# ashiq24/UNO

Hardware: AMD Instinct MI355X
Metric: UNO training samples/s (421^2 Darcy) (higher is better)
Workload: dtype f32; 1 GPU; Darcy 2D 421x421, UNO_9(3,64,pad=5) 64ch, batch 16/GPU, train step (fwd+loss+bwd+allreduce+Adam); global_batch=16, parallelism=dp1

## Files before the change

include/uno_spectral.h:

```cpp
#ifndef UNO_SPECTRAL_H
#define UNO_SPECTRAL_H

#ifdef __cplusplus
extern "C" {
#endif

#define UNO_SPECTRAL_ABI_VERSION 14

int uno_abi_version(void);
void* uno_upload_table(const void* host, long long bytes);

const char* uno_last_error(void);

long long uno_spectral_conv2d_fwd_ws_bytes(int B, int Ci, int Co, int m1, int m2);
long long uno_spectral_conv2d_bwd_ws_bytes(int B, int Ci, int Co, int m1, int m2);

int uno_spectral_conv2d_forward(const float* x, const float* w1, const float* w2, float* y,
                                float* xtrunc, void* ws, int B, int Ci, int Co, int H, int W,
                                int Ho, int Wo, int m1, int m2, void* stream);

int uno_spectral_conv2d_backward(const float* gy, const float* xtrunc, const float* w1,
                                 const float* w2, float* gx, float* gw1, float* gw2, void* ws,
                                 int B, int Ci, int Co, int H, int W, int Ho, int Wo, int m1,
                                 int m2, void* stream);
// ... 36 lines not shown
long long uno_spectral_conv3d_bwd_ws_bytes(int B, int Ci, int Co, int H, int Ho, int m1, int m2, int m3);
int uno_spectral_conv3d_forward(const float* x, const float* const* w, float* y, float* xtrunc, void* ws,
                                int B, int Ci, int Co, int H, int W, int T, int Ho, int Wo, int To,
                                int m1, int m2, int m3, void* stream);
int uno_spectral_conv3d_backward(const float* gy, const float* xtrunc, const float* const* w, float* gx,
                                 float* const* gw, void* ws, int B, int Ci, int Co, int H, int W, int T,
                                 int Ho, int Wo, int To, int m1, int m2, int m3, void* stream);

long long uno_dft3d_ws_bytes(int n_vol, int D1, int m2, int m3);
int uno_dft3d_forward_grouped(const float* x, float* spec, void* ws, int n_vol, int D1, int D2, int D3, int m1, int m2, int m3,
                              float scale, int adjoint, int group, int stride, int offset, void* stream);
int uno_dft3d_inverse_grouped(const float* spec, float* y, void* ws, int n_vol, int D1, int D2, int D3, int m1, int m2, int m3,
                              float scale, int weighted, int group, int stride, int offset, void* stream);

int uno_spectral_conv3d_forward2(const float* x1, const float* x2, int C1, const float* const* w, float* y, float* xtrunc, void* ws,
                                 int B, int Ci, int Co, int H, int W, int T, int Ho, int Wo, int To, int m1, int m2, int m3,
                                 void* stream);
int uno_spectral_conv3d_backward2(const float* gy, const float* xtrunc, const float* const* w, float* gx1, float* gx2, int C1,
                                  float* const* gw, void* ws, int B, int Ci, int Co, int H, int W, int T, int Ho, int Wo, int To,
                                  int m1, int m2, int m3, void* stream);

int uno_cdft_axis(const float* in, float* out, int inverse, int n_img, int H, int m1, int m2, int m3,
                  float scale, int mask_overlap, void* stream);


int uno_dft2d_forward(const float* images, float* spec, int n_img, int H, int W, int m1, int m2,
                      float scale, int hermitian_cols, int mask_overlap, void* stream);

int uno_dft2d_inverse(const float* spec, float* images, int n_img, int H, int W, int m1, int m2,
                      float scale, int hermitian_cols, int mask_overlap, void* stream);

int uno_reserve_cus(int n);

int uno_sweep_alternation(int enable);

int uno_dft2d_inverse_add_applies(int n_img, int H, int W, int m1, int m2, int Hs, int Ws);
int uno_dft2d_inverse_add(const float* spec, float* images, int n_img, int H, int W, int m1, int m2, float scale, int hermitian_cols,
                          int mask_overlap, const float* addend, int Hs, int Ws, const int* tile_p0, const float* row_op,
                          const int* col_v0, const float* col_op, void* stream);

int uno_dft2d_forward_resample_applies(int n_img, int H, int W, int m1, int m2, int Ho, int Wo, int KW);
int uno_dft2d_forward_resample(const float* images, float* spec, int n_img, int H, int W, int m1, int m2, float scale, int hermitian_cols,
                               int mask_overlap, int group, int stride, int offset, float* resampled, int Ho, int Wo, const int* col_start,
                               const float* col_wt, int KW, const int* row_tiles, const float* row_op, void* stream);

int uno_spectrum_crop(const float* src, float* dst, int n_img, int M1, int M2, int m1, int m2, int src_group, int src_stride, int src_offset,
                      int dst_group, int dst_stride, int dst_offset, void* stream);

int uno_dft2d_forward_bf16(const void* images, float* spec, int n_img, int H, int W, int m1, int m2,
                           float scale, int hermitian_cols, int mask_overlap, void* stream);
int uno_dft2d_inverse_bf16(const float* spec, void* images, int n_img, int H, int W, int m1, int m2,
                           float scale, int hermitian_cols, int mask_overlap, void* stream);

int uno_dft2d_forward_grouped(const float* images, float* spec, int n_img, int H, int W, int m1, int m2, float scale,
                              int hermitian_cols, int mask_overlap, int group, int stride, int offset, void* stream);
int uno_dft2d_inverse_grouped(const float* spec, float* images, int n_img, int H, int W, int m1, int m2, float scale,
                              int hermitian_cols, int mask_overlap, int group, int stride, int offset, void* stream);

int uno_mode_mix(const float* in, const float* const* w, float* out, int op, int B, int Ci, int Co,
                 int ncorner, int modes_per_corner, void* stream);

int uno_mode_wgrad(const float* xtrunc, const float* go, float* const* gw, int B, int Ci, int Co,
                   int ncorner, int modes_per_corner, void* stream);
int uno_mode_backward(const float* xtrunc, const float* go, const float* const* w, float* gx_spec, float* const* gw, int B, int Ci,
                      int Co, int ncorner, int modes_per_corner, int accumulate, void* stream);
int uno_mode_wgrad_acc(const float* xtrunc, const float* go, float* const* gw, int B, int Ci, int Co, int ncorner,
                       int modes_per_corner, int accumulate, void* stream);
int uno_spectral_conv2d_backward_acc(const void* gy, const float* xtrunc, const void* w1, const void* w2, void* gx,
                                     float* gw1, float* gw2, void* ws, int B, int Ci, int Co, int H, int W, int Ho, int Wo,
                                     int m1, int m2, int io_format, int accumulate_gw, void* stream);

int uno_resample2d(const float* in, float* out, float* tmp, int n_img, int H, int W, int Ho, int Wo,
                   const int* startH, const float* wtH, int KH, const int* startW, const float* wtW, int KW,
                   const int* tile_p0, const float* tile_w, int NP, int accumulate, void* stream);

int uno_channel_mix(const float* x, const float* w, const float* bias, float* y, int B, int Ci, int Co,
                    long long P, int transpose_w, int accumulate, int act_in, const float* dgelu_of, void* stream);

long long uno_channel_wgrad_ws_bytes(int B, int Ci, int Co, long long P);
int uno_channel_wgrad(const float* gy, const float* x, float* gw, float* gb, void* ws, int B, int Ci, int Co,
                      long long P, int act_x, void* stream);

int uno_channel_mix2(const float* x1, const float* x2, int C1, const float* w, const float* bias, float* y1, float* y2, int Co1,
                     float* y_act, int B, int Ci, int Co, long long P, int transpose_w, int accumulate, int act_in,
                     const float* dgelu_of, const float* proj_w, const float* proj_b, float* proj_out, void* stream);
int uno_channel_wgrad2(const float* gy, const float* x1, const float* x2, int C1, float* gw, float* gb, void* ws, int B, int Ci,
                       int Co, long long P, int act_x, int accumulate, void* stream);
int uno_channel_wgrad_finish(const void* parts, float* gw, float* gb, int Ci, int Co, long long nparts, int accumulate, void* stream);

int uno_gelu_project_forward(const float* pre, const float* w, const float* bias, float* out, int B, int C, long long P,
                             void* stream);
long long uno_gelu_project_bwd_ws_bytes(int B, int C, long long P);
int uno_gelu_project_backward(const float* pre, const float* w, const float* gout, float* gpre, float* gw, float* gb,
                              void* ws, int B, int C, long long P, void* stream);

int uno_gelu_project2_forward(const float* pre, const float* s, const float* w, const float* bias, float* out, int B, int C1, int C2,
                              long long P, int act2, void* stream);
long long uno_gelu_project2_bwd_ws_bytes(int B, int C1, int C2, long long P);
int uno_gelu_project2_backward(const float* pre, const float* s, const float* w, const float* gout, float* gpre, float* gs, float* gw,
                               float* gb, void* ws, int B, int C1, int C2, long long P, int act2, void* stream);

long long uno_rel_l2_steps_ws_bytes(int B, long long P, int T);
int uno_rel_l2_steps(const float* pred, const float* target, float* sums, float* rel, float* totals, void* ws, int B, long long P, int T,
                     void* stream);

long long uno_rel_l2_ws_bytes(int B, long long N);
int uno_rel_l2_forward(const float* x, long long x_row, long long x_elem, const float* y, long long y_row, long long y_elem, float* sums,
                       float* ratio, float* total, void* ws, int B, long long N, void* stream);
int uno_rel_l2_backward(const float* x, long long x_row, long long x_elem, const float* y, long long y_row, long long y_elem,
                        const float* sums, const float* g, int g_per_row, float scale, float* gx, int B, long long N, void* stream);

long long uno_rollout_ws_bytes(int B, long long P, int T);
int uno_rollout_advance(float* window, const float* frame, const float* target, float* pred, void* ws, int B, int C, int T_in, long long P,
                        int T, int t, int shift, void* stream);
int uno_rollout_finish(const void* ws, float* sums, float* rel, float* totals, int B, long long P, int T, void* stream);

int uno_rollout_lift(const float* given, const float* pred, const float* feat, const float* w, const float* bias, float* h, int B, int T_in,
                     int F, int Cm, long long P, int T, int t, void* stream);
long long uno_rollout_lift_bwd_ws_bytes(int B, int T_in, int F, int Cm, long long P, int T);
int uno_rollout_lift_backward(const float* gh, const float* given, const float* pred, const float* target, const float* feat, const float* w,
                              const float* sums, const float* gL, float* gpred, float* gframe, void* parts, int B, int T_in, int F, int Cm,
                              long long P, int T, int t, void* stream);
int uno_rollout_loss_seed(const float* pred, const float* target, const float* sums, const float* gL, float* gframe, int B, long long P, int T,
                          void* stream);

int uno_channel_mix2_win(const float* x1, const float* x2, int C1, const float* w, const float* bias, float* y1, float* y2, int Co1,
                         float* y_act, int B, int Ci, int Co, int rows, int cols, int pitch, long long plane, int transpose_w,
                         int accumulate, int act_in, const float* dgelu_of, const float* proj_w, const float* proj_b, float* proj_out,
                         void* stream);
int uno_channel_wgrad2_win(const float* gy, const float* x1, const float* x2, int C1, float* gw, float* gb, void* ws, int B, int Ci,
                           int Co, int rows, int cols, int pitch, long long plane, int act_x, int accumulate, void* stream);
int uno_gelu_project_backward_win(const float* pre, const float* w, const float* gout, float* gpre, float* gw, float* gb, void* ws,
                                  int B, int C, int rows, int cols, int pitch, long long plane, void* stream);
int uno_project_backward_applies(int B, int C1, int Ci, int Co, int rows, int cols, int pitch, long long plane);
long long uno_project_backward_ws_bytes(int B, int Ci, int Co, long long P);
int uno_project_backward(const float* x1, const float* x2, int C1, const float* w, const float* pre, const float* w2, const float* gout,
                         float* g1, float* g2, float* gw, float* gb, float* gw2, float* gb2, void* ws, int B, int Ci, int Co, int rows,
                         int cols, int pitch, long long plane, int act_in, int accumulate_w, void* stream);
int uno_clear_border(float* t, long long n_planes, int Hp, int Wp, int rows, int cols, void* stream);
int uno_channel_mix_act_padded(const float* x, const float* w, const float* bias, float* y, float* y_act, int B, int Ci, int Co, int H,
                               int W, int Hp, int Wp, int act_in, void* stream);
int uno_channel_mix_dgelu_padded(const float* x, const float* w, const float* bias, const float* g_padded, float* gz, int B, int Ci,
                                 int Co, int H, int W, int Hp, int Wp, int act_in, void* stream);
int uno_lift_forward(const float* x, const float* w1, const float* b1, const float* w0, const float* b0, float* act, int B, int Cin,
                     int Cm, int Co, int H, int W, int Hp, int Wp, void* stream);
long long uno_lift_bwd_ws_bytes(int B, int Cin, int Cm, int Co, int H, int W);
int uno_lift_backward(const float* x, const float* w1, const float* b1, const float* w0, const float* b0, const float* g_act, float* gw1,
                      float* gb1, float* gw0, float* gb0, void* ws, int B, int Cin, int Cm, int Co, int H, int W, int Hp, int Wp,
                      void* stream);
int uno_lift_backward_takes_second(int B, int Cin, int Cm, int Co, int H, int W, int Hp, int Wp);
int uno_lift_backward2(const float* x, const float* w1, const float* b1, const float* w0, const float* b0, const float* g_act,
                       const float* g_act2, float* gw1, float* gb1, float* gw0, float* gb0, void* ws, int B, int Cin, int Cm, int Co,
                       int H, int W, int Hp, int Wp, void* stream);

int uno_gelu_pad(const float* s, const float* gy, float* out, int n_img, int H, int W, int Hp, int Wp, int backward,
                 void* stream);

int uno_instnorm_forward(const float* x, const float* gamma, const float* beta, float* y, float* mean, float* rstd, long long rows,
                         int C, long long N, float eps, int gelu, void* stream);
int uno_instnorm_backward(const float* x, const float* gy, const float* gamma, const float* beta, const float* mean,
                          const float* rstd, float* gx, float* s1, float* s2, long long rows, int C, long long N, int gelu,
                          void* stream);

int uno_adam_step(float* p, const float* g, float* m, float* v, long long n, int is_complex, double lr, double beta1,
                  double beta2, double eps, double weight_decay, int step, void* stream);

int uno_adam_step_multi(int n_tensors, float* const* p, const float* const* g, float* const* m, float* const* v,
                        const long long* n, const int* is_complex, double lr, double beta1, double beta2, double eps,
                        double weight_decay, int step, void* stream);

int uno_adam_step_multi_dev(int n_tensors, float* const* p, const float* const* g, float* const* m, float* const* v,
                            const long long* n, const int* is_complex, double lr, double beta1, double beta2, double eps,
                            double weight_decay, int* step_counter, float* scalars, const double* hyper, void* stream);

int uno_spectral_conv2d_forward_mixed(const void* x_bf16, const void* w1_f16, const void* w2_f16, void* y_bf16,
                                      float* xtrunc, void* ws, int B, int Ci, int Co, int H, int W, int Ho, int Wo,
                                      int modes1, int modes2, void* stream);
int uno_spectral_conv2d_backward_mixed(const void* gy_bf16, const float* xtrunc, const void* w1_f16, const void* w2_f16,
                                       void* gx_bf16, float* gw1, float* gw2, void* ws, int B, int Ci, int Co, int H, int W,
                                       int Ho, int Wo, int modes1, int modes2, void* stream);
int uno_mode_mix_f16w(const float* in, const void* const* w_f16, float* out, int op, int B, int Ci, int Co, int ncorner,
                      int modes_per_corner, void* stream);
int uno_dft2d_forward_grouped_bf16(const void* images, float* spec, int n_img, int H, int W, int m1, int m2, float scale,
                                   int hermitian_cols, int mask_overlap, int group, int stride, int offset, void* stream);
int uno_dft2d_inverse_grouped_bf16(const float* spec, void* images, int n_img, int H, int W, int m1, int m2, float scale,
                                   int hermitian_cols, int mask_overlap, int group, int stride, int offset, void* stream);
int uno_resample2d_bf16(const void* in, void* out, float* tmp, int n_img, int H, int W, int Ho, int Wo, const int* startH,
                        const float* wtH, int KH, const int* startW, const float* wtW, int KW, const int* tile_p0,
                        const float* tile_w, int NP, int accumulate, void* stream);
int uno_channel_mix_bf16(const void* x, const float* w, const float* bias, void* y, int B, int Ci, int Co, long long P,
                         int transpose_w, int accumulate, int act_in, const void* dgelu_of, void* stream);
int uno_channel_wgrad_bf16(const void* gy, const void* x, float* gw, float* gb, void* ws, int B, int Ci, int Co, long long P,
                           int act_x, void* stream);
int uno_channel_mix2_bf16(const void* x1, const void* x2, int C1, const float* w, const float* bias, void* y1, void* y2, int Co1,
                          void* y_act, int B, int Ci, int Co, long long P, int transpose_w, int accumulate, int act_in,
                          const void* dgelu_of, const float* proj_w, const float* proj_b, void* proj_out, void* stream);
int uno_channel_wgrad2_bf16(const void* gy, const void* x1, const void* x2, int C1, float* gw, float* gb, void* ws, int B, int Ci,
                            int Co, long long P, int act_x, int accumulate, void* stream);
int uno_gelu_project_forward_bf16(const void* pre, const float* w, const float* bias, void* out, int B, int C, long long P,
                                  void* stream);
int uno_gelu_project_backward_bf16(const void* pre, const float* w, const void* gout, void* gpre, float* gw, float* gb,
                                   void* ws, int B, int C, long long P, void* stream);
int uno_gelu_pad_bf16(const void* s, const void* gy, void* out, int n_img, int H, int W, int Hp, int Wp, int backward,
                      void* stream);
int uno_instnorm_forward_bf16(const void* x, const float* gamma, const float* beta, void* y, float* mean, float* rstd,
                              long long rows, int C, long long N, float eps, int gelu, void* stream);
int uno_instnorm_backward_bf16(const void* x, const void* gy, const float* gamma, const float* beta, const float* mean,
                               const float* rstd, void* gx, float* s1, float* s2, long long rows, int C, long long N,
                               int gelu, void* stream);

long long uno_dft2d_any_ws_bytes(int n_img, int H, int W, int m1, int m2);
int uno_scratch_provide(void* ptr, long long bytes);
long long uno_channel_mix_ws_bytes(int Ci, int Co, long long P, int bf16);

int uno_transpose_batched(const float* in, float* out, int B, long long R, int C, long long ld_in, long long sb_in,
                          long long ld_out, long long sb_out, void* stream);

int uno_channel_mix2_rows(const float* x1, const float* x2, int C1, const float* w, const float* bias, float* y, int B, int Ci, int Co,
                          int rows, int cols, int pitch, int col0, long long plane, int act_in, void* stream);
int uno_channel_mix2_rows_grad(const float* gy, const float* w, int C1, const float* dgelu_of, float* g1, float* g2, int B, int Ci,
                               int Co, int rows, int cols, int pitch, int col0, long long plane, void* stream);
int uno_channel_wgrad2_rows(const float* gy, const float* x1, const float* x2, int C1, float* gw, float* gb, void* ws, int B, int Ci,
                            int Co, int rows, int cols, int pitch, int col0, long long plane, int act_x, int accumulate, void* stream);
int uno_channel_mix_act_padded_rows(const float* x, const float* w, const float* bias, float* y, float* y_act, int B, int Ci, int Co,
                                    int rows, int cols, int pitch, int col0, int act_in, void* stream);
int uno_dgelu_rows(const float* pre, const float* g_padded, float* gz, long long n_planes, int rows, int cols, int pitch, int col0,
                   long long plane, void* stream);

long long uno_ns2d_ws_bytes(int B, int N);
int uno_ns2d_forward(const float* w, float* w_h, void* ws, int B, int N, void* stream);
int uno_ns2d_inverse(const float* w_h, float* w, void* ws, int B, int N, void* stream);
int uno_ns2d_steps(float* w_h, const float* f_h, int f_batched, void* ws, int B, int N, long long n_steps, double visc, double delta_t,
                   void* stream);

int uno_profile_begin(int max_records);
int uno_profile_end(void);
int uno_profile_get(int index, char* name, int name_len, double* ms, double* bytes);

#ifdef __cplusplus
}
#endif
#endif
```

uno_amd/_native.py:

```python
from __future__ import annotations

import contextlib
import ctypes as C
import os
import threading

import torch

_HERE = os.path.dirname(os.path.abspath(__file__))
LIB_PATH = os.path.join(_HERE, "lib", "libuno_spectral.so")
ABI_VERSION = 14

_lib = None
_lock = threading.Lock()

_fp = C.c_void_p
_i = C.c_int
_SIGNATURES = {
    "uno_abi_version": (C.c_int, []),
    "uno_last_error": (C.c_char_p, []),
    "uno_dft2d_any_ws_bytes": (C.c_longlong, [_i] * 5),
    "uno_scratch_provide": (C.c_int, [_fp, C.c_longlong]),
    "uno_spectral_conv2d_fwd_ws_bytes": (C.c_longlong, [_i] * 5),
    "uno_spectral_conv2d_bwd_ws_bytes": (C.c_longlong, [_i] * 5),
    "uno_spectral_conv2d_forward": (C.c_int, [_fp] * 6 + [_i] * 9 + [_fp]),
    "uno_spectral_conv2d_backward": (C.c_int, [_fp] * 8 + [_i] * 9 + [_fp]),
    "uno_spectral_conv2d_forward_bf16": (C.c_int, [_fp] * 6 + [_i] * 9 + [_fp]),
    "uno_spectral_conv2d_backward_bf16": (C.c_int, [_fp] * 8 + [_i] * 9 + [_fp]),
    "uno_fft_resample3d_ws_bytes": (C.c_longlong, [_i] * 6),
    "uno_fft_resample3d": (C.c_int, [_fp] * 3 + [_i] * 8 + [_fp, _fp, _i, _fp, _fp, _i, C.c_float, _i, _i, _fp]),
    "uno_fft_resample3d_acc": (C.c_int, [_fp] * 4 + [_i] * 8 + [_fp, _fp, _i, _fp, _fp, _i, C.c_float, _i, _i, _fp]),
    "uno_fft_resample3d_any_ws_bytes": (C.c_longlong, [_i] * 6),
    "uno_fft_resample3d_any": (C.c_int, [_fp] * 3 + [_i] * 8 + [_fp, _fp, _i, _fp, _fp, _i, C.c_float, _i, _i, _fp]),
    "uno_fft_resample3d_any_acc": (C.c_int, [_fp] * 4 + [_i] * 8 + [_fp, _fp, _i, _fp, _fp, _i, C.c_float, _i, _i, _fp]),
    "uno_fft_resample3d_wide_ws_bytes": (C.c_longlong, [_i] * 6),
    "uno_fft_resample3d_wide": (C.c_int, [_fp] * 3 + [_i] * 8 + [_fp, _fp, _i, _fp, _fp, _i, C.c_float, _i, _i, _fp]),
    "uno_fft_resample3d_wide_acc": (C.c_int, [_fp] * 4 + [_i] * 8 + [_fp, _fp, _i, _fp, _fp, _i, C.c_float, _i, _i, _fp]),
    "uno_dft2d_forward": (C.c_int, [_fp, _fp] + [_i] * 5 + [C.c_float, _i, _i, _fp]),
    "uno_dft2d_forward_bf16": (C.c_int, [_fp, _fp] + [_i] * 5 + [C.c_float, _i, _i, _fp]),
    "uno_dft2d_inverse_bf16": (C.c_int, [_fp, _fp] + [_i] * 5 + [C.c_float, _i, _i, _fp]),
    "uno_dft2d_inverse": (C.c_int, [_fp, _fp] + [_i] * 5 + [C.c_float, _i, _i, _fp]),
    "uno_reserve_cus": (C.c_int, [_i]),
    "uno_sweep_alternation": (C.c_int, [_i]),
    "uno_dft2d_inverse_add_applies": (C.c_int, [_i] * 7),
    "uno_dft2d_forward_resample_applies": (C.c_int, [_i] * 8),
    "uno_dft2d_forward_resample": (C.c_int, [_fp, _fp] + [_i] * 5 + [C.c_float] + [_i] * 5 + [_fp, _i, _i, _fp, _fp, _i, _fp, _fp, _fp]),
    "uno_dft2d_inverse_add": (C.c_int, [_fp, _fp] + [_i] * 5 + [C.c_float, _i, _i, _fp, _i, _i, _fp, _fp, _fp, _fp, _fp]),
    "uno_dft2d_forward_grouped": (C.c_int, [_fp, _fp] + [_i] * 5 + [C.c_float] + [_i] * 5 + [_fp]),
    "uno_dft2d_inverse_grouped": (C.c_int, [_fp, _fp] + [_i] * 5 + [C.c_float] + [_i] * 5 + [_fp]),
    "uno_spectrum_crop": (C.c_int, [_fp, _fp] + [_i] * 11 + [_fp]),
    "uno_mode_mix": (C.c_int, [_fp, C.POINTER(_fp), _fp] + [_i] * 6 + [_fp]),
    "uno_mode_wgrad": (C.c_int, [_fp, _fp, C.POINTER(_fp)] + [_i] * 5 + [_fp]),
    "uno_mode_backward": (C.c_int, [_fp, _fp, C.POINTER(_fp), _fp, C.POINTER(_fp)] + [_i] * 6 + [_fp]),
    "uno_spectral_conv3d_fwd_ws_bytes": (C.c_longlong, [_i] * 8),
    "uno_spectral_conv3d_bwd_ws_bytes": (C.c_longlong, [_i] * 8),
    "uno_spectral_conv3d_forward": (C.c_int, [_fp, C.POINTER(_fp), _fp, _fp, _fp] + [_i] * 12 + [_fp]),
    "uno_spectral_conv3d_backward": (C.c_int, [_fp, _fp, C.POINTER(_fp), _fp, C.POINTER(_fp), _fp] + [_i] * 12 + [_fp]),
    "uno_cdft_axis": (C.c_int, [_fp, _fp] + [_i] * 6 + [C.c_float, _i, _fp]),
    "uno_dft3d_ws_bytes": (C.c_longlong, [_i] * 4),
    "uno_dft3d_forward_grouped": (C.c_int, [_fp, _fp, _fp] + [_i] * 7 + [C.c_float] + [_i] * 4 + [_fp]),
    "uno_dft3d_inverse_grouped": (C.c_int, [_fp, _fp, _fp] + [_i] * 7 + [C.c_float] + [_i] * 4 + [_fp]),
    "uno_spectral_conv3d_forward2": (C.c_int, [_fp, _fp, _i, C.POINTER(_fp), _fp, _fp, _fp] + [_i] * 12 + [_fp]),
    "uno_spectral_conv3d_backward2": (C.c_int, [_fp, _fp, C.POINTER(_fp), _fp, _fp, _i, C.POINTER(_fp), _fp] + [_i] * 12 + [_fp]),
    "uno_resample2d": (C.c_int, [_fp, _fp, _fp] + [_i] * 5 + [_fp, _fp, _i, _fp, _fp, _i, _fp, _fp, _i, _i, _fp]),
    "uno_channel_mix": (C.c_int, [_fp, _fp, _fp, _fp, _i, _i, _i, C.c_longlong, _i, _i, _i, _fp, _fp]),
    "uno_channel_wgrad_ws_bytes": (C.c_longlong, [_i, _i, _i, C.c_longlong]),
    "uno_channel_wgrad": (C.c_int, [_fp, _fp, _fp, _fp, _fp, _i, _i, _i, C.c_longlong, _i, _fp]),
    "uno_channel_mix2": (C.c_int, [_fp, _fp, _i, _fp, _fp, _fp, _fp, _i, _fp, _i, _i, _i, C.c_longlong, _i, _i, _i, _fp, _fp, _fp, _fp, _fp]),
    "uno_channel_wgrad2": (C.c_int, [_fp, _fp, _fp, _i, _fp, _fp, _fp, _i, _i, _i, C.c_longlong, _i, _i, _fp]),
    "uno_channel_mix2_win": (C.c_int, [_fp, _fp, _i, _fp, _fp, _fp, _fp, _i, _fp, _i, _i, _i, _i, _i, _i, C.c_longlong, _i, _i, _i, _fp, _fp, _fp, _fp, _fp]),
    "uno_channel_mix_ws_bytes": (C.c_longlong, [_i, _i, C.c_longlong, _i]),
    "uno_clear_border": (C.c_int, [_fp, C.c_longlong, _i, _i, _i, _i, _fp]),
    "uno_channel_mix_act_padded": (C.c_int, [_fp, _fp, _fp, _fp, _fp, _i, _i, _i, _i, _i, _i, _i, _i, _fp]),
    "uno_lift_forward": (C.c_int, [_fp] * 6 + [_i] * 8 + [_fp]),
    "uno_lift_bwd_ws_bytes": (C.c_longlong, [_i] * 6),
    "uno_lift_backward": (C.c_int, [_fp] * 11 + [_i] * 8 + [_fp]),
    "uno_lift_backward2": (C.c_int, [_fp] * 12 + [_i] * 8 + [_fp]),
    "uno_lift_backward_takes_second": (C.c_int, [_i] * 8),
    "uno_channel_mix_dgelu_padded": (C.c_int, [_fp, _fp, _fp, _fp, _fp, _i, _i, _i, _i, _i, _i, _i, _i, _fp]),
    "uno_channel_wgrad2_win": (C.c_int, [_fp, _fp, _fp, _i, _fp, _fp, _fp, _i, _i, _i, _i, _i, _i, C.c_longlong, _i, _i, _fp]),
    "uno_gelu_project_backward_win": (C.c_int, [_fp] * 7 + [_i, _i, _i, _i, _i, C.c_longlong, _fp]),
    "uno_channel_wgrad_finish": (C.c_int, [_fp, _fp, _fp, _i, _i, C.c_longlong, _i, _fp]),
    "uno_mode_wgrad_acc": (C.c_int, [_fp, _fp, C.POINTER(_fp)] + [_i] * 6 + [_fp]),
    "uno_spectral_conv2d_backward_acc": (C.c_int, [_fp] * 8 + [_i] * 11 + [_fp]),
    "uno_upload_table": (C.c_void_p, [_fp, C.c_longlong]),
    "uno_project_backward_applies": (C.c_int, [_i] * 7 + [C.c_longlong]),
    "uno_project_backward_ws_bytes": (C.c_longlong, [_i, _i, _i, C.c_longlong]),
    "uno_project_backward": (C.c_int, [_fp, _fp, _i] + [_fp] * 11 + [_i] * 6 + [C.c_longlong, _i, _i, _fp]),
    "uno_gelu_project_forward": (C.c_int, [_fp, _fp, _fp, _fp, _i, _i, C.c_longlong, _fp]),
    "uno_gelu_project_bwd_ws_bytes": (C.c_longlong, [_i, _i, C.c_longlong]),
    "uno_gelu_project_backward": (C.c_int, [_fp] * 7 + [_i, _i, C.c_longlong, _fp]),
    "uno_gelu_project2_forward": (C.c_int, [_fp] * 5 + [_i, _i, _i, C.c_longlong, _i, _fp]),
    "uno_gelu_project2_bwd_ws_bytes": (C.c_longlong, [_i, _i, _i, C.c_longlong]),
    "uno_gelu_project2_backward": (C.c_int, [_fp] * 9 + [_i, _i, _i, C.c_longlong, _i, _fp]),
    "uno_rel_l2_steps_ws_bytes": (C.c_longlong, [_i, C.c_longlong, _i]),
    "uno_rel_l2_steps": (C.c_int, [_fp] * 6 + [_i, C.c_longlong, _i, _fp]),
    "uno_rel_l2_ws_bytes": (C.c_longlong, [_i, C.c_longlong]),
    "uno_rel_l2_forward": (C.c_int, [_fp, C.c_longlong, C.c_longlong] * 2 + [_fp] * 4 + [_i, C.c_longlong, _fp]),
    "uno_rel_l2_backward": (C.c_int, [_fp, C.c_longlong, C.c_longlong] * 2 + [_fp, _fp, _i, C.c_float, _fp, _i, C.c_longlong, _fp]),
    "uno_rollout_ws_bytes": (C.c_longlong, [_i, C.c_longlong, _i]),
    "uno_rollout_advance": (C.c_int, [_fp] * 5 + [_i, _i, _i, C.c_longlong, _i, _i, _i, _fp]),
    "uno_rollout_finish": (C.c_int, [_fp] * 4 + [_i, C.c_longlong, _i, _fp]),
    "uno_rollout_lift": (C.c_int, [_fp] * 6 + [_i, _i, _i, _i, C.c_longlong, _i, _i, _fp]),
    "uno_rollout_lift_bwd_ws_bytes": (C.c_longlong, [_i, _i, _i, _i, C.c_longlong, _i]),
    "uno_rollout_lift_backward": (C.c_int, [_fp] * 11 + [_i, _i, _i, _i, C.c_longlong, _i, _i, _fp]),
    "uno_rollout_loss_seed": (C.c_int, [_fp] * 5 + [_i, C.c_longlong, _i, _fp]),
    "uno_gelu_pad": (C.c_int, [_fp, _fp, _fp] + [_i] * 6 + [_fp]),
    "uno_transpose_batched": (C.c_int, [_fp, _fp, _i, C.c_longlong, _i] + [C.c_longlong] * 4 + [_fp]),
    "uno_instnorm_forward": (C.c_int, [_fp] * 6 + [C.c_longlong, _i, C.c_longlong, C.c_float, _i, _fp]),
    "uno_instnorm_backward": (C.c_int, [_fp] * 9 + [C.c_longlong, _i, C.c_longlong, _i, _fp]),
    "uno_adam_step": (C.c_int, [_fp, _fp, _fp, _fp, C.c_longlong, _i] + [C.c_double] * 5 + [_i, _fp]),
    "uno_adam_step_multi": (C.c_int, [_i, C.POINTER(_fp), C.POINTER(_fp), C.POINTER(_fp), C.POINTER(_fp), C.POINTER(C.c_longlong),
                                      C.POINTER(_i)] + [C.c_double] * 5 + [_i, _fp]),
    "uno_adam_step_multi_dev": (C.c_int, [_i, C.POINTER(_fp), C.POINTER(_fp), C.POINTER(_fp), C.POINTER(_fp), C.POINTER(C.c_longlong),
                                          C.POINTER(_i)] + [C.c_double] * 5 + [_fp, _fp, _fp, _fp]),
    "uno_spectral_conv2d_forward_mixed": (C.c_int, [_fp] * 6 + [_i] * 9 + [_fp]),
    "uno_spectral_conv2d_backward_mixed": (C.c_int, [_fp] * 8 + [_i] * 9 + [_fp]),
    "uno_mode_mix_f16w": (C.c_int, [_fp, C.POINTER(_fp), _fp] + [_i] * 6 + [_fp]),
    "uno_dft2d_forward_grouped_bf16": (C.c_int, [_fp, _fp] + [_i] * 5 + [C.c_float] + [_i] * 5 + [_fp]),
    "uno_dft2d_inverse_grouped_bf16": (C.c_int, [_fp, _fp] + [_i] * 5 + [C.c_float] + [_i] * 5 + [_fp]),
    "uno_resample2d_bf16": (C.c_int, [_fp, _fp, _fp] + [_i] * 5 + [_fp, _fp, _i, _fp, _fp, _i, _fp, _fp, _i, _i, _fp]),
    "uno_channel_mix_bf16": (C.c_int, [_fp, _fp, _fp, _fp, _i, _i, _i, C.c_longlong, _i, _i, _i, _fp, _fp]),
    "uno_channel_wgrad_bf16": (C.c_int, [_fp, _fp, _fp, _fp, _fp, _i, _i, _i, C.c_longlong, _i, _fp]),
    "uno_channel_mix2_bf16": (C.c_int, [_fp, _fp, _i, _fp, _fp, _fp, _fp, _i, _fp, _i, _i, _i, C.c_longlong, _i, _i, _i, _fp, _fp, _fp, _fp, _fp]),
    "uno_channel_wgrad2_bf16": (C.c_int, [_fp, _fp, _fp, _i, _fp, _fp, _fp, _i, _i, _i, C.c_longlong, _i, _i, _fp]),
    "uno_gelu_project_forward_bf16": (C.c_int, [_fp, _fp, _fp, _fp, _i, _i, C.c_longlong, _fp]),
    "uno_gelu_project_backward_bf16": (C.c_int, [_fp] * 7 + [_i, _i, C.c_longlong, _fp]),
    "uno_gelu_pad_bf16": (C.c_int, [_fp, _fp, _fp] + [_i] * 6 + [_fp]),
    "uno_instnorm_forward_bf16": (C.c_int, [_fp] * 6 + [C.c_longlong, _i, C.c_longlong, C.c_float, _i, _fp]),
    "uno_instnorm_backward_bf16": (C.c_int, [_fp] * 9 + [C.c_longlong, _i, C.c_longlong, _i, _fp]),
    "uno_channel_mix2_rows": (C.c_int, [_fp, _fp, _i, _fp, _fp, _fp] + [_i] * 7 + [C.c_longlong, _i, _fp]),
    "uno_channel_mix2_rows_grad": (C.c_int, [_fp, _fp, _i, _fp, _fp, _fp] + [_i] * 7 + [C.c_longlong, _fp]),
    "uno_channel_wgrad2_rows": (C.c_int, [_fp, _fp, _fp, _i, _fp, _fp, _fp] + [_i] * 7 + [C.c_longlong, _i, _i, _fp]),
    "uno_channel_mix_act_padded_rows": (C.c_int, [_fp] * 5 + [_i] * 8 + [_fp]),
    "uno_dgelu_rows": (C.c_int, [_fp, _fp, _fp, C.c_longlong, _i, _i, _i, _i, C.c_longlong, _fp]),
    "uno_ns2d_ws_bytes": (C.c_longlong, [_i, _i]),
    "uno_ns2d_forward": (C.c_int, [_fp, _fp, _fp, _i, _i, _fp]),
    "uno_ns2d_inverse": (C.c_int, [_fp, _fp, _fp, _i, _i, _fp]),
    "uno_ns2d_steps": (C.c_int, [_fp, _fp, _i, _fp, _i, _i, C.c_longlong, C.c_double, C.c_double, _fp]),
    "uno_profile_begin": (C.c_int, [_i]),
    "uno_profile_end": (C.c_int, []),
    "uno_profile_get": (C.c_int, [_i, C.c_char_p, _i, C.POINTER(C.c_double), C.POINTER(C.c_double)]),
}
EXPORTED_SYMBOLS = tuple(_SIGNATURES)


def lib():
    global _lib
    if _lib is None:
        with _lock:
            if _lib is None:
                if not os.path.exists(LIB_PATH):
                    raise RuntimeError(
                        f"uno_amd: native library {LIB_PATH} is missing - build it with "
                        "`python -m uno_amd.build` (hipcc, gfx950); there is no CPU fallback")
                h = C.CDLL(LIB_PATH)
                for name, (res, args) in _SIGNATURES.items():
                    fn = getattr(h, name)
                    fn.restype = res
                    fn.argtypes = args
                if h.uno_abi_version() != ABI_VERSION:
                    raise RuntimeError(f"uno_amd: ABI mismatch, library {h.uno_abi_version()} != binding {ABI_VERSION}")
                _lib = h
    return _lib


def _check(rc: int, what: str):
    if rc != 0:
        msg = lib().uno_last_error().decode(errors="replace")
        raise RuntimeError(f"{what} failed (code {rc}): {msg}")


def _ptr(t: torch.Tensor):
    return C.c_void_p(t.data_ptr())


def _opt(t):
    return _ptr(t) if t is not None else C.c_void_p(0)


def _count(lead) -> int:
    n = 1
    for d in lead:
        n *= d
    return n


def _stream(t: torch.Tensor):
    return C.c_void_p(torch.cuda.current_stream(t.device).cuda_stream)


class _scratch:

    def __init__(self, device, nbytes):
        self.bytes, self.device, self.buf = nbytes, device, None

    def __enter__(self):
        if self.bytes > 0:
            self.buf = torch.empty(self.bytes, dtype=torch.uint8, device=self.device)
            _check(lib().uno_scratch_provide(_ptr(self.buf), self.bytes), "uno_scratch_provide")
        return self

    def __exit__(self, *exc):
        if self.bytes > 0:
            lib().uno_scratch_provide(None, 0)
        return False


class _any_mode_scratch(_scratch):

    def __init__(self, device, *needs):
        L = lib()
        _scratch.__init__(self, device, max((int(L.uno_dft2d_any_ws_bytes(*[int(v) for v in n])) for n in needs), default=0))


class _mix_scratch(_scratch):

    def __init__(self, device, Ci, Co, P, bf16):
        _scratch.__init__(self, device, int(lib().uno_channel_mix_ws_bytes(int(Ci), int(Co), int(P), 1 if bf16 else 0)))


def _require(t: torch.Tensor, dtype, name: str, dense: bool = True):
    if not t.is_cuda:
        raise RuntimeError(f"uno_amd: {name} must live on a HIP device (got {t.device})"
                           + ("; the spectral convolution runs only on the MI355X kernels" if dense else ""))
    if t.dtype != dtype:
        raise RuntimeError(f"uno_amd: {name} must be {dtype} (got {t.dtype})")
    if dense and not t.is_contiguous():
        raise RuntimeError(f"uno_amd: {name} must be contiguous")


# ... 497 lines not shown
    sW, wW = tabW
    accumulate = out is not None
    if accumulate:
        _require(out, x.dtype, "out")
        if tuple(out.shape) != (*lead, Ho, Wo):
            raise RuntimeError(f"uno_amd: out has shape {tuple(out.shape)}, expected {(*lead, Ho, Wo)}")
    else:
        out = torch.empty((*lead, Ho, Wo), dtype=x.dtype, device=x.device)
    with torch.cuda.device(x.device):
        tmp = torch.empty(max(1, n * min(Ho * W, H * Wo)), dtype=torch.float32, device=x.device)
        if tilesH is not None:
            tp0, tw = tilesH
            targs = (_ptr(tp0), _ptr(tw), tw.shape[1])
        else:
            targs = (C.c_void_p(0), C.c_void_p(0), 0)
        fn = _entry("uno_resample2d", bf16)
        rc = fn(_ptr(x), _ptr(out), _ptr(tmp), n, H, W, Ho, Wo, _ptr(sH), _ptr(wH), wH.shape[1],
                _ptr(sW), _ptr(wW), wW.shape[1], *targs, 1 if accumulate else 0, _stream(x))
    _check(rc, "uno_resample2d")
    return out


def _window_fits(rows: int, cols: int, pitch: int, plane: int) -> bool:
    return not (rows < 1 or cols % 4 or cols < 260 or pitch < cols or (rows - 1) * pitch + cols > plane or rows * cols >= 1 << 24)


def _window_args(window, plane: int, bf16: bool):
    rows, cols, pitch = (int(v) for v in window)
    if bf16:
        raise RuntimeError("uno_amd: pixel windows are float32 only")
    if not _window_fits(rows, cols, pitch, plane):
        raise RuntimeError(f"uno_amd: window rows={rows} cols={cols} pitch={pitch} does not fit a plane of {plane} elements "
                           "(cols: a multiple of 4, 260 <= cols <= pitch; rows * cols < 2^24)")
    return rows, cols, pitch


def channel_mix(x, w, bias=None, transpose_w: bool = False, out=None, act_in: bool = False, dgelu_of=None, dgelu_total: bool = False,
                window=None):
    if window is not None:
        return channel_mix2(x, None, w, bias, transpose_w=transpose_w, out=out, act_in=act_in, dgelu_of=dgelu_of,
                            accumulate=(2 if (dgelu_total and dgelu_of is not None) else 1) if out is not None else 0, window=window)
    bf16 = _act_dtype(x, "x")
    _require(w, torch.float32, "weight")
    if bias is not None:
        _require(bias, torch.float32, "bias")
    B, Ci, P = x.shape
    Co = w.shape[1] if transpose_w else w.shape[0]
    if (w.shape[0] if transpose_w else w.shape[1]) != Ci:
        raise RuntimeError(f"uno_amd: weight {tuple(w.shape)} does not match {Ci} input channels")
    accumulate = out is not None
    if accumulate:
        _require(out, x.dtype, "out")
        if tuple(out.shape) != (B, Co, P):
            raise RuntimeError(f"uno_amd: out has shape {tuple(out.shape)}, expected {(B, Co, P)}")
        y = out
    else:
        y = torch.empty((B, Co, P), dtype=x.dtype, device=x.device)
    with torch.cuda.device(x.device), _mix_scratch(x.device, Ci, Co, P, bf16):
        if dgelu_of is not None:
            _require(dgelu_of, x.dtype, "dgelu_of")
            if tuple(dgelu_of.shape) != (B, Co, P):
                raise RuntimeError(f"uno_amd: dgelu_of has shape {tuple(dgelu_of.shape)}, expected {(B, Co, P)}")
        rc = _entry("uno_channel_mix", bf16)(_ptr(x), _ptr(w), _opt(bias), _ptr(y), B, Ci, Co, P, 1 if transpose_w else 0,
                                             (2 if (dgelu_total and dgelu_of is not None) else 1) if accumulate else 0,
                                             1 if act_in else 0, _opt(dgelu_of), _stream(x))
    _check(rc, "uno_channel_mix")
    return y


def clear_border(t, rows: int, cols: int):
    _require(t, torch.float32, "tensor")
    Hp, Wp = t.shape[-2:]
    n = t.numel() // max(1, Hp * Wp)
    with torch.cuda.device(t.device):
        rc = lib().uno_clear_border(_ptr(t), n, Hp, Wp, int(rows), int(cols), _stream(t))
    _check(rc, "uno_clear_border")
    return t


def channel_mix_act_padded_ok(x, Hp: int, Wp: int) -> bool:
    H, W = x.shape[-2:]
    return x.dtype == torch.float32 and 260 <= W <= Wp and H <= Hp and H * W < (1 << 24)


def channel_mix_act_padded(x, w, bias, Hp: int, Wp: int, act_in: bool = False, keep_y: bool = True):
    _require(x, torch.float32, "x")
    _require(w, torch.float32, "weight")
    if bias is not None:
        _require(bias, torch.float32, "bias")
    B, Ci, H, W = x.shape
    Co = w.shape[0]
    if w.shape[1] != Ci:
        raise RuntimeError(f"uno_amd: weight {tuple(w.shape)} does not match {Ci} input channels")
    y = torch.empty((B, Co, H, W), dtype=x.dtype, device=x.device) if keep_y else None
    act = torch.empty((B, Co, Hp, Wp), dtype=x.dtype, device=x.device)
    with torch.cuda.device(x.device):
        rc = lib().uno_channel_mix_act_padded(_ptr(x), _ptr(w), _opt(bias), _opt(y), _ptr(act),
                                              B, Ci, Co, H, W, int(Hp), int(Wp), 1 if act_in else 0, _stream(x))
    _check(rc, "uno_channel_mix_act_padded")
    return y, act


def lift_ok(x, w1, w0, Hp: int, Wp: int) -> bool:
    if x.dim() != 4 or x.dtype != torch.float32:
        return False
    H, W = x.shape[-2:]
    return (1 <= x.shape[1] <= 3 and w1.shape[0] in (16, 32) and w1.shape[1] == x.shape[1] and w0.shape[1] == w1.shape[0]
            and 260 <= W <= Wp and H <= Hp and H * W < (1 << 24))


def lift_forward(x, w1, b1, w0, b0, Hp: int, Wp: int):
    for t, n in ((x, "x"), (w1, "weight 1"), (w0, "weight 0")) + tuple((t, "bias") for t in (b1, b0) if t is not None):
        _require(t, torch.float32, n)
    B, Cin, H, W = x.shape
    Cm, Co = w1.shape[0], w0.shape[0]
    act = torch.empty((B, Co, Hp, Wp), dtype=x.dtype, device=x.device)
    with torch.cuda.device(x.device):
        rc = lib().uno_lift_forward(_ptr(x), _ptr(w1), _opt(b1), _ptr(w0), _opt(b0),
                                    _ptr(act), B, Cin, Cm, Co, H, W, int(Hp), int(Wp), _stream(x))
    _check(rc, "uno_lift_forward")
    return act


def lift_backward_takes_second(x, w1, w0, Hp: int, Wp: int) -> bool:
    B, Cin, H, W = x.shape
    return bool(lib().uno_lift_backward_takes_second(B, Cin, w1.shape[0], w0.shape[0], H, W, int(Hp), int(Wp)))


def lift_backward(x, w1, b1, w0, b0, g_act, g_act2=None):
    _require(g_act, torch.float32, "grad_output")
    B, Cin, H, W = x.shape
    Cm, Co = w1.shape[0], w0.shape[0]
    Hp, Wp = g_act.shape[-2:]
    if tuple(g_act.shape[:2]) != (B, Co):
        raise RuntimeError("uno_amd: grad_output does not match the lift")
    if g_act2 is not None:
        _require(g_act2, torch.float32, "second grad_output")
        if tuple(g_act2.shape) != tuple(g_act.shape):
            raise RuntimeError("uno_amd: the two gradients of the lift's output disagree in shape")
    dev = x.device
    gw1 = torch.empty((Cm, Cin), dtype=torch.float32, device=dev)
    gw0 = torch.empty((Co, Cm), dtype=torch.float32, device=dev)
    gb1 = torch.empty((Cm,), dtype=torch.float32, device=dev) if b1 is not None else None
    gb0 = torch.empty((Co,), dtype=torch.float32, device=dev) if b0 is not None else None
    with torch.cuda.device(dev):
        ws = torch.empty(max(1, lib().uno_lift_bwd_ws_bytes(B, Cin, Cm, Co, H, W)), dtype=torch.uint8, device=dev)
        rc = lib().uno_lift_backward2(_ptr(x), _ptr(w1), _opt(b1), _ptr(w0), _opt(b0),
                                     _ptr(g_act), _opt(g_act2), _ptr(gw1), _opt(gb1), _ptr(gw0),
                                     _opt(gb0), _ptr(ws), B, Cin, Cm, Co, H, W, int(Hp), int(Wp), _stream(x))
    _check(rc, "uno_lift_backward")
    return gw1, gb1, gw0, gb0


def channel_mix_dgelu_padded(x, w, bias, g_padded, act_in: bool = False):
    _require(x, torch.float32, "x")
    _require(w, torch.float32, "weight")
    _require(g_padded, torch.float32, "grad_output")
    if bias is not None:
        _require(bias, torch.float32, "bias")
    B, Ci, H, W = x.shape
    Co = w.shape[0]
    if w.shape[1] != Ci or g_padded.dim() != 4 or g_padded.shape[:2] != (B, Co) or g_padded.shape[2] < H or g_padded.shape[3] < W:
        raise RuntimeError("uno_amd: weight / grad_output do not match the layer")
    Hp, Wp = g_padded.shape[2:]
    gz = torch.empty((B, Co, H, W), dtype=x.dtype, device=x.device)
    with torch.cuda.device(x.device):
        rc = lib().uno_channel_mix_dgelu_padded(_ptr(x), _ptr(w), _opt(bias), _ptr(g_padded), _ptr(gz),
                                                B, Ci, Co, H, W, int(Hp), int(Wp), 1 if act_in else 0, _stream(x))
    _check(rc, "uno_channel_mix_dgelu_padded")
    return gz


def channel_mix2_ok(C1: int, Co1, Co: int, P: int) -> bool:
    if C1 is not None and (C1 < 16 or C1 % 16):
        return False
    if Co1 is not None and (Co1 < 64 or Co1 % 64):
        return False
    return True


def channel_mix2(x1, x2, w, bias=None, transpose_w: bool = False, out=None, out2=None, split_out: int | None = None,
                 act_in: bool = False, dgelu_of=None, y_act: bool = False, accumulate: bool = False, project=None, window=None):
    bf16 = _act_dtype(x1, "x1")
    _require(w, torch.float32, "weight")
    if x2 is not None:
        _require(x2, x1.dtype, "x2")
        if x2.shape[0] != x1.shape[0] or x2.shape[2] != x1.shape[2]:
            raise RuntimeError("uno_amd: the two sources disagree in batch / pixel count")
    if bias is not None:
        _require(bias, torch.float32, "bias")
    B, C1, P = x1.shape
    Ci = C1 + (x2.shape[1] if x2 is not None else 0)
    Co = w.shape[1] if transpose_w else w.shape[0]
    if (w.shape[0] if transpose_w else w.shape[1]) != Ci:
        raise RuntimeError(f"uno_amd: weight {tuple(w.shape)} does not match {Ci} input channels")
    Co1 = Co if split_out is None else int(split_out)
    if out is None:
        y1 = torch.empty((B, Co1, P), dtype=x1.dtype, device=x1.device)
        y2 = torch.empty((B, Co - Co1, P), dtype=x1.dtype, device=x1.device) if split_out is not None else None
    else:
        y1, y2 = out, out2
        _require(y1, x1.dtype, "out")
        if tuple(y1.shape) != (B, Co1, P) or (split_out is not None and (y2 is None or tuple(y2.shape) != (B, Co - Co1, P))):
            raise RuntimeError("uno_amd: output tensors do not match (B, Co1, P) / (B, Co - Co1, P)")
        if y2 is not None:
            _require(y2, x1.dtype, "out2")
    act = torch.empty((B, Co, P), dtype=x1.dtype, device=x1.device) if y_act else None
    if dgelu_of is not None:
        _require(dgelu_of, x1.dtype, "dgelu_of")
        if tuple(dgelu_of.shape) != (B, Co1, P):
            raise RuntimeError(f"uno_amd: dgelu_of has shape {tuple(dgelu_of.shape)}, expected {(B, Co1, P)}")
    proj = pw = pb = None
    if project is not None:
        pw, pb = project
        _require(pw, torch.float32, "projection weight")
        if pw.numel() != Co:
            raise RuntimeError(f"uno_amd: projection weight has {pw.numel()} entries for {Co} channels")
        if pb is not None:
            _require(pb, torch.float32, "projection bias")
        proj = torch.empty((B, P), dtype=x1.dtype, device=x1.device)
    acc_flag = int(accumulate) if out is not None else 0
    if acc_flag == 2 and (dgelu_of is None or window is None):
        raise RuntimeError("uno_amd: accumulate = 2 goes with dgelu_of (windowed one-destination calls)")
    with torch.cuda.device(x1.device), _mix_scratch(x1.device, Ci, Co, P if window is None else window[0] * window[1], bf16):
        if window is not None:
            fn, size = lib().uno_channel_mix2_win, (*_window_args(window, P, bf16), P)
        else:
            fn, size = _entry("uno_channel_mix2", bf16), (P,)
        rc = fn(_ptr(x1), _opt(x2), C1, _ptr(w), _opt(bias), _ptr(y1), _opt(y2), Co1, _opt(act),
                B, Ci, Co, *size, 1 if transpose_w else 0, acc_flag, 1 if act_in else 0,
                _opt(dgelu_of), _opt(pw), _opt(pb), _opt(proj), _stream(x1))
    _check(rc, "uno_channel_mix2")
    if split_out is not None:
        return y1, y2
    if project is not None:
        return y1, proj
    return (y1, act) if y_act else y1


def channel_wgrad_partial_floats(B: int, Ci: int, Co: int, P: int) -> int:
    return int(lib().uno_channel_wgrad_ws_bytes(B, Ci, Co, P)) // 4


def channel_wgrad_finish(parts, Ci: int, Co: int, need_bias: bool, out_w=None, out_b=None, accumulate: bool = False):
    _require(parts, torch.float32, "partial sums")
    blk = Co * (Ci + 1)
    if parts.numel() == 0 or parts.numel() % blk:
        raise RuntimeError("uno_amd: the partial sums are not a whole number of (Co, Ci + 1) blocks")
    gw, gb, accumulate = _real_grad_buffers(out_w, out_b, Ci, Co, need_bias, parts.device, accumulate)
    with torch.cuda.device(parts.device):
        rc = lib().uno_channel_wgrad_finish(_ptr(parts), _ptr(gw), _opt(gb), Ci, Co,
                                            parts.numel() // blk, 1 if accumulate else 0, _stream(parts))
    _check(rc, "uno_channel_wgrad_finish")
    return gw, gb


def channel_wgrad2(gy, x1, x2, need_bias: bool = True, act_x: bool = False, out_w=None, out_b=None, accumulate: bool = False,
                   partials_out=None, window=None):
    bf16 = _act_dtype(gy, "grad_output")
    _require(x1, gy.dtype, "x1")
    B, Co, P = gy.shape
    if window is not None:
        if partials_out is not None:
            raise RuntimeError("uno_amd: windowed weight gradients run both stages")
        win = _window_args(window, P, bf16)
    C1 = x1.shape[1]
    C2 = 0
    if x2 is not None:
        _require(x2, gy.dtype, "x2")
        C2 = x2.shape[1]
        if x2.shape[0] != B or x2.shape[2] != P:
            raise RuntimeError("uno_amd: grad_output and the sources disagree in batch / pixel count")
    if x1.shape[0] != B or x1.shape[2] != P:
        raise RuntimeError("uno_amd: grad_output and the sources disagree in batch / pixel count")
    Ci = C1 + C2
    L = lib()
    if partials_out is not None:
        _require(partials_out, torch.float32, "partial-sum buffer")
        if partials_out.numel() != channel_wgrad_partial_floats(B, Ci, Co, P):
            raise RuntimeError("uno_amd: partial-sum buffer has the wrong size")
        with torch.cuda.device(gy.device):
            rc = _entry("uno_channel_wgrad2", bf16)(_ptr(gy), _ptr(x1), _opt(x2), C1, C.c_void_p(0), C.c_void_p(0),
                                                    _ptr(partials_out), B, Ci, Co, P, 1 if act_x else 0, 3, _stream(gy))
        _check(rc, "uno_channel_wgrad2")
        return None, None
    gw, gb, accumulate = _real_grad_buffers(out_w, out_b, Ci, Co, need_bias, gy.device, accumulate)
    with torch.cuda.device(gy.device):
        if window is not None:
            fn, size, Pl = L.uno_channel_wgrad2_win, (*win, P), win[0] * win[1]
        else:
            fn, size, Pl = _entry("uno_channel_wgrad2", bf16), (P,), P
        ws = torch.empty(max(1, L.uno_channel_wgrad_ws_bytes(B, Ci, Co, Pl)), dtype=torch.uint8, device=gy.device)
        rc = fn(_ptr(gy), _ptr(x1), _opt(x2), C1, _ptr(gw), _opt(gb),
                _ptr(ws), B, Ci, Co, *size, 1 if act_x else 0, 1 if accumulate else 0, _stream(gy))
    _check(rc, "uno_channel_wgrad2")
    return gw, gb


def rows_window_ok(rows: int, cols: int, pitch: int, col0: int, plane: int, Ci: int = 1, Co: int = 1) -> bool:
    return (rows >= 0 and cols >= 1 and col0 >= 0 and col0 + cols <= pitch <= 256 and rows * pitch < (1 << 24) and plane >= rows * pitch
            and 1 <= Ci <= 1024 and Co >= 1)


def _rows_args(window, plane: int):
    rows, cols, pitch, col0 = (int(v) for v in window)
    return rows, cols, pitch, col0, int(plane)
# ... 713 lines not shown
```

uno_amd/csrc/capi_pointwise.hip:

```cpp
#include "../../include/uno_spectral.h"
#include "uno_common.h"

using namespace uno;

extern "C" {

static int resample2d_impl(const void* in, void* out, float* tmp, int n_img, int H, int W, int Ho, int Wo, const int* startH,
                           const float* wtH, int KH, const int* startW, const float* wtW, int KW, const int* tile_p0,
                           const float* tile_w, int NP, int accumulate, int bf16, void* stream) {
    if (n_img < 0 || H < 1 || W < 1 || Ho < 1 || Wo < 1) { set_error("uno_resample2d: bad sizes"); return -1; }
    if (n_img == 0) return 0;
    if (!in || !out || !tmp || !startH || !wtH || !startW || !wtW) { set_error("uno_resample2d: null pointer"); return -1; }
    return launch_resample2d(in, out, tmp, n_img, H, W, Ho, Wo, startH, wtH, KH, startW, wtW, KW, tile_p0, tile_w, NP, accumulate, bf16, (hipStream_t)stream);
}

int uno_resample2d(const float* in, float* out, float* tmp, int n_img, int H, int W, int Ho, int Wo, const int* startH,
                   const float* wtH, int KH, const int* startW, const float* wtW, int KW, const int* tile_p0,
                   const float* tile_w, int NP, int accumulate, void* stream) {
    return resample2d_impl(in, out, tmp, n_img, H, W, Ho, Wo, startH, wtH, KH, startW, wtW, KW, tile_p0, tile_w, NP, accumulate, 0, stream);
}

int uno_resample2d_bf16(const void* in, void* out, float* tmp, int n_img, int H, int W, int Ho, int Wo, const int* startH,
                        const float* wtH, int KH, const int* startW, const float* wtW, int KW, const int* tile_p0,
                        const float* tile_w, int NP, int accumulate, void* stream) {
// ... 123 lines not shown
        ChannelMixArgs a{};
        a.x = pre; a.w = w; a.y = g1; a.y2 = x2 ? g2 : nullptr; a.dgelu_of = act_in ? x1 : nullptr;
        a.B = B; a.Ci = Co; a.Co = Ci; a.C1 = Co; a.Co1 = x2 ? C1 : Ci; a.P = P; a.transpose_w = 1;
        a.win = win; a.pb_w2 = w2; a.pb_g = gout;
        if (int rc = launch_channel_mix2(a, s)) return rc;
    }
    WgradProjectedBack pb;
    pb.w2 = w2; pb.g = gout; pb.gw2 = gw2; pb.gb2 = gb2;
    return launch_channel_wgrad2(pre, x1, x2, C1, gw, gb, (float*)ws, B, Ci, Co, P, act_in, accumulate_w, 0, s, win, pb);
}

int uno_clear_border(float* t, long long n_planes, int Hp, int Wp, int rows, int cols, void* stream) {
    if (n_planes < 0 || Hp < 1 || Wp < 1 || rows < 0 || rows > Hp || cols < 0 || cols > Wp) {
        set_error("uno_clear_border: bad sizes planes=%lld (%d, %d) keep (%d, %d)", n_planes, Hp, Wp, rows, cols);
        return -1;
    }
    if (n_planes == 0) return 0;
    if (!t) { set_error("uno_clear_border: null pointer"); return -1; }
    return launch_clear_border(t, n_planes, Hp, Wp, rows, cols, (hipStream_t)stream);
}

static int lift_padded(const char* who, const float* x, const float* w, const float* bias, float* y, float* y_act, const float* gmul, int B,
                       int Ci, int Co, int H, int W, int Hp, int Wp, int act_in, void* stream) {
    if (B < 0 || Ci < 1 || Co < 1 || H < 1 || W < 1 || Hp < H || Wp < W) {
        set_error("%s: bad sizes B=%d Ci=%d Co=%d (%d, %d) -> (%d, %d)", who, B, Ci, Co, H, W, Hp, Wp);
        return -1;
    }
    if (B == 0) return 0;
    if (!x || !w || (!y && !y_act) || (gmul && !y)) { set_error("%s: null pointer", who); return -1; }
    ChannelMixArgs a{};
    a.x = x; a.w = w; a.bias = bias; a.y = y; a.y_act = y_act; a.gmul = gmul;
    a.B = B; a.Ci = Ci; a.Co = Co; a.C1 = Ci; a.Co1 = Co; a.P = (long long)H * W; a.act_in = act_in;
    a.act_cols = W; a.act_pitch = Wp; a.act_plane = (long long)Hp * Wp;
    if (int rc = launch_channel_mix2(a, (hipStream_t)stream)) return rc;
    return y_act ? launch_clear_border(y_act, (long long)B * Co, Hp, Wp, H, W, (hipStream_t)stream) : 0;
}

int uno_channel_mix_act_padded(const float* x, const float* w, const float* bias, float* y, float* y_act, int B, int Ci, int Co, int H, int W,
                               int Hp, int Wp, int act_in, void* stream) {
    if (!y_act) { set_error("uno_channel_mix_act_padded: null pointer"); return -1; }
    return lift_padded("uno_channel_mix_act_padded", x, w, bias, y, y_act, nullptr, B, Ci, Co, H, W, Hp, Wp, act_in, stream);
}

int uno_channel_mix_dgelu_padded(const float* x, const float* w, const float* bias, const float* g_padded, float* gz, int B, int Ci, int Co,
                                 int H, int W, int Hp, int Wp, int act_in, void* stream) {
    if (!g_padded || !gz) { set_error("uno_channel_mix_dgelu_padded: null pointer"); return -1; }
    return lift_padded("uno_channel_mix_dgelu_padded", x, w, bias, gz, nullptr, g_padded, B, Ci, Co, H, W, Hp, Wp, act_in, stream);
}

static int lift_check(const char* who, int B, int Cin, int Cm, int Co, int H, int W, int Hp, int Wp) {
    if (B < 0 || Cin < 1 || Cin > 3 || Cm < 5 || Cm > 32 || Cm % 16 || Co < 1 || H < 1 || W < 260 || Hp < H || Wp < W || (long long)H * W >= (1LL << 24)) {
        set_error("%s: needs 1 .. 3 input channels, 16 or 32 middle channels, 260 <= W <= Wp, H <= Hp, H * W < 2^24 (got B=%d %d -> %d -> %d, (%d, %d) -> (%d, %d))",
                  who, B, Cin, Cm, Co, H, W, Hp, Wp);
        return -1;
    }
    return 0;
}

static bool lift_fused_fits(int B, int H, int Hp, int Wp, int Co) {
    return (long long)Hp * Wp * Co < (1LL << 31) && B <= 65535 && (long long)H * Wp < (1LL << 24);
}

int uno_lift_forward(const float* x, const float* w1, const float* b1, const float* w0, const float* b0, float* act, int B, int Cin, int Cm,
                     int Co, int H, int W, int Hp, int Wp, void* stream) {
    if (int rc = lift_check("uno_lift_forward", B, Cin, Cm, Co, H, W, Hp, Wp)) return rc;
    if (B == 0) return 0;
    if (!x || !w1 || !w0 || !act) { set_error("uno_lift_forward: null pointer"); return -1; }
    if (lift_bwd_fused_applies(Cin, Cm, Co, W, (long long)H * W) && lift_fused_fits(B, H, Hp, Wp, Co) && (Wp & ~3) >= 260 && (Wp & ~3) >= W) {
        if (int rc = launch_lift_forward_fused(x, w1, b1, w0, b0, act, B, Cin, H, W, Hp, Wp, (hipStream_t)stream)) return rc;
        return launch_clear_border(act, (long long)B * Co, Hp, Wp, H, Wp, (hipStream_t)stream);
    }
    ChannelMixArgs a{};
    a.x = x; a.w = w0; a.bias = b0; a.y = nullptr; a.y_act = act;
    a.B = B; a.Ci = Cm; a.Co = Co; a.C1 = Cm; a.Co1 = Co; a.P = (long long)H * W; a.act_in = 1;
    a.act_cols = W; a.act_pitch = Wp; a.act_plane = (long long)Hp * Wp;
    a.vh_x = x; a.vh_w = w1; a.vh_b = b1; a.vh_ci = Cin; a.vh_mode = 1;
    if (int rc = launch_channel_mix2(a, (hipStream_t)stream)) return rc;
    return launch_clear_border(act, (long long)B * Co, Hp, Wp, H, W, (hipStream_t)stream);
}

static long long lift_wgrad_ws(int B, int Cin, int Cm, int Co, long long P) {
    const long long a = 4LL * channel_wgrad_ws_floats(B, Cm, Co, P, nullptr), b = 4LL * channel_wgrad_ws_floats(B, Cin, Cm, P, nullptr);
    return a > b ? a : b;
}
long long uno_lift_bwd_ws_bytes(int B, int Cin, int Cm, int Co, int H, int W) {
    if (B < 1 || Cin < 1 || Cm < 1 || Co < 1 || H < 1 || W < 1) return 0;
    const long long P = (long long)H * W;
    return 4LL * B * P * (Co + Cm) + lift_wgrad_ws(B, Cin, Cm, Co, P);
}

int uno_lift_backward_takes_second(int B, int Cin, int Cm, int Co, int H, int W, int Hp, int Wp) {
    if (B < 1 || Cin < 1 || Cin > 3 || Cm < 5 || Cm > 32 || Cm % 16 || Co < 1 || H < 1 || W < 260 || Hp < H || Wp < W) return 0;
    return (lift_bwd_fused_applies(Cin, Cm, Co, W, (long long)H * W) && lift_fused_fits(B, H, Hp, Wp, Co)) ? 1 : 0;
}

int uno_lift_backward2(const float* x, const float* w1, const float* b1, const float* w0, const float* b0_, const float* g_act, const float* g_act2,
                       float* gw1, float* gb1, float* gw0, float* gb0, void* ws, int B, int Cin, int Cm, int Co, int H, int W, int Hp, int Wp,
                       void* stream);

int uno_lift_backward(const float* x, const float* w1, const float* b1, const float* w0, const float* b0_, const float* g_act, float* gw1,
                      float* gb1, float* gw0, float* gb0, void* ws, int B, int Cin, int Cm, int Co, int H, int W, int Hp, int Wp, void* stream) {
    return uno_lift_backward2(x, w1, b1, w0, b0_, g_act, nullptr, gw1, gb1, gw0, gb0, ws, B, Cin, Cm, Co, H, W, Hp, Wp, stream);
}

int uno_lift_backward2(const float* x, const float* w1, const float* b1, const float* w0, const float* b0_, const float* g_act, const float* g_act2,
                       float* gw1, float* gb1, float* gw0, float* gb0, void* ws, int B, int Cin, int Cm, int Co, int H, int W, int Hp, int Wp,
                       void* stream) {
    if (int rc = lift_check("uno_lift_backward", B, Cin, Cm, Co, H, W, Hp, Wp)) return rc;
    if (g_act2 && !uno_lift_backward_takes_second(B, Cin, Cm, Co, H, W, Hp, Wp) && B > 0) {
        set_error("uno_lift_backward2: a second gradient tensor goes with the fused kernel only (query uno_lift_backward_takes_second)");
        return -3;
    }
    if (!gw1 || !gw0) { set_error("uno_lift_backward: null pointer"); return -1; }
    hipStream_t s = (hipStream_t)stream;
    if (B == 0) {
        if (hipMemsetAsync(gw1, 0, sizeof(float) * Cm * Cin, s) != hipSuccess || hipMemsetAsync(gw0, 0, sizeof(float) * Co * Cm, s) != hipSuccess ||
            (gb1 && hipMemsetAsync(gb1, 0, sizeof(float) * Cm, s) != hipSuccess) || (gb0 && hipMemsetAsync(gb0, 0, sizeof(float) * Co, s) != hipSuccess)) {
            set_error("uno_lift_backward: memset failed");
            return -5;
        }
        return 0;
    }
    if (!x || !w1 || !w0 || !g_act || !ws) { set_error("uno_lift_backward: null pointer"); return -1; }
    const long long P = (long long)H * W;
    if (lift_bwd_fused_applies(Cin, Cm, Co, W, P) && lift_fused_fits(B, H, Hp, Wp, Co)) {
        float* part = static_cast<float*>(ws);
        const long long nparts = lift_bwd_fused_parts(B, H, W);
        float* part1 = part + (size_t)nparts * Co * (Cm + 1);
        if (int rc = launch_lift_backward_fused(x, w1, b1, w0, b0_, g_act, part, part1, B, Cin, H, W, Hp, Wp, s, g_act2)) return rc;
        if (int rc = launch_channel_wgrad_finish(part, gw0, gb0, Cm, Co, nparts, 0, s)) return rc;
        return launch_channel_wgrad_finish(part1, gw1, gb1, Cin, Cm, nparts, 0, s);
    }
    float* gz = static_cast<float*>(ws);
    float* gh = gz + (size_t)B * Co * P;
    float* wws = gh + (size_t)B * Cm * P;
    {
        ChannelMixArgs a{};
        a.x = x; a.w = w0; a.bias = b0_; a.y = gz; a.gmul = g_act;
        a.B = B; a.Ci = Cm; a.Co = Co; a.C1 = Cm; a.Co1 = Co; a.P = P; a.act_in = 1;
        a.act_cols = W; a.act_pitch = Wp; a.act_plane = (long long)Hp * Wp;
        a.vh_x = x; a.vh_w = w1; a.vh_b = b1; a.vh_ci = Cin; a.vh_mode = 1;
        if (int rc = launch_channel_mix2(a, s)) return rc;
    }
    {
        ChannelMixArgs a{};
        a.x = gz; a.w = w0; a.y = gh; a.B = B; a.Ci = Co; a.Co = Cm; a.C1 = Co; a.Co1 = Cm; a.P = P; a.transpose_w = 1;
        a.vh_x = x; a.vh_w = w1; a.vh_b = b1; a.vh_ci = Cin; a.vh_mode = 2;
        if (int rc = launch_channel_mix2(a, s)) return rc;
    }
    if (int rc = launch_channel_wgrad_vh(gz, x, w1, b1, Cin, gw0, gb0, wws, B, Cm, Co, P, 1, s, 0)) return rc;
    return launch_channel_wgrad2(gh, x, nullptr, Cin, gw1, gb1, wws, B, Cin, Cm, P, 0, 0, 0, s);
}

long long uno_channel_wgrad_ws_bytes(int B, int Ci, int Co, long long P) {
    if (B < 1 || Ci < 1 || Co < 1 || P < 1) return 0;
    return 4LL * channel_wgrad_ws_floats(B, Ci, Co, P, nullptr);
}

static int channel_wgrad_impl(const void* gy, const void* x, float* gw, float* gb, void* ws, int B, int Ci, int Co, long long P,
                              int act_x, int bf16, void* stream) {
    if (B < 0 || Ci < 1 || Co < 1 || P < 0) { set_error("uno_channel_wgrad: bad sizes B=%d Ci=%d Co=%d P=%lld", B, Ci, Co, P); return -1; }
    if (!gw) { set_error("uno_channel_wgrad: null pointer"); return -1; }
    if (B == 0 || P == 0) {
        if (hipMemsetAsync(gw, 0, sizeof(float) * Co * Ci, (hipStream_t)stream) != hipSuccess ||
            (gb && hipMemsetAsync(gb, 0, sizeof(float) * Co, (hipStream_t)stream) != hipSuccess)) { set_error("uno_channel_wgrad: memset failed"); return -5; }
        return 0;
    }
    if (!gy || !x || !ws) { set_error("uno_channel_wgrad: null pointer"); return -1; }
    return launch_channel_wgrad(gy, x, gw, gb, (float*)ws, B, Ci, Co, P, act_x, bf16, (hipStream_t)stream);
}

int uno_channel_wgrad(const float* gy, const float* x, float* gw, float* gb, void* ws, int B, int Ci, int Co, long long P,
                      int act_x, void* stream) {
    return channel_wgrad_impl(gy, x, gw, gb, ws, B, Ci, Co, P, act_x, 0, stream);
}

int uno_channel_wgrad_bf16(const void* gy, const void* x, float* gw, float* gb, void* ws, int B, int Ci, int Co, long long P,
                           int act_x, void* stream) {
    return channel_wgrad_impl(gy, x, gw, gb, ws, B, Ci, Co, P, act_x, 1, stream);
}

static int channel_wgrad2_impl(const void* gy, const void* x1, const void* x2, int C1, float* gw, float* gb, void* ws, int B, int Ci,
                               int Co, long long P, int act_x, int accumulate, int bf16, void* stream, const PixelWindow& win = PixelWindow()) {
    if (B < 0 || Ci < 1 || Co < 1 || P < 0) { set_error("uno_channel_wgrad2: bad sizes B=%d Ci=%d Co=%d P=%lld", B, Ci, Co, P); return -1; }
    if (accumulate < 0 || accumulate > 3 || accumulate == 2) { set_error("uno_channel_wgrad2: accumulate is 0, 1 or 3 (got %d)", accumulate); return -1; }
    if (!gw && accumulate != 3) { set_error("uno_channel_wgrad2: null pointer"); return -1; }
    if (B == 0 || P == 0) {
        if (accumulate == 3) {
            if (!ws) { set_error("uno_channel_wgrad2: null pointer"); return -1; }
            if (hipMemsetAsync(ws, 0, uno_channel_wgrad_ws_bytes(B, Ci, Co, P), (hipStream_t)stream) != hipSuccess) { set_error("uno_channel_wgrad2: memset failed"); return -5; }
            return 0;
        }
        if (accumulate) return 0;
        if (hipMemsetAsync(gw, 0, sizeof(float) * Co * Ci, (hipStream_t)stream) != hipSuccess ||
            (gb && hipMemsetAsync(gb, 0, sizeof(float) * Co, (hipStream_t)stream) != hipSuccess)) { set_error("uno_channel_wgrad2: memset failed"); return -5; }
        return 0;
    }
    if (!gy || !x1 || !ws) { set_error("uno_channel_wgrad2: null pointer"); return -1; }
    return launch_channel_wgrad2(gy, x1, x2, x2 ? C1 : Ci, gw, gb, (float*)ws, B, Ci, Co, P, act_x, accumulate, bf16, (hipStream_t)stream, win);
}

int uno_channel_wgrad2_win(const float* gy, const float* x1, const float* x2, int C1, float* gw, float* gb, void* ws, int B, int Ci, int Co,
                           int rows, int cols, int pitch, long long plane, int act_x, int accumulate, void* stream) {
    PixelWindow win; long long P;
    if (!make_window("uno_channel_wgrad2_win", rows, cols, pitch, plane, &win, &P)) return -1;
    return channel_wgrad2_impl(gy, x1, x2, C1, gw, gb, ws, B, Ci, Co, P, act_x, accumulate, 0, stream, win);
}

int uno_channel_wgrad2(const float* gy, const float* x1, const float* x2, int C1, float* gw, float* gb, void* ws, int B, int Ci, int Co,
                       long long P, int act_x, int accumulate, void* stream) {
    return channel_wgrad2_impl(gy, x1, x2, C1, gw, gb, ws, B, Ci, Co, P, act_x, accumulate, 0, stream);
}

int uno_channel_wgrad2_bf16(const void* gy, const void* x1, const void* x2, int C1, float* gw, float* gb, void* ws, int B, int Ci, int Co,
                            long long P, int act_x, int accumulate, void* stream) {
    return channel_wgrad2_impl(gy, x1, x2, C1, gw, gb, ws, B, Ci, Co, P, act_x, accumulate, 1, stream);
}

int uno_channel_wgrad_finish(const void* parts, float* gw, float* gb, int Ci, int Co, long long nparts, int accumulate, void* stream) {
    if (Ci < 1 || Co < 1 || nparts < 1) { set_error("uno_channel_wgrad_finish: bad sizes Ci=%d Co=%d blocks=%lld", Ci, Co, nparts); return -1; }
    if (!parts || !gw) { set_error("uno_channel_wgrad_finish: null pointer"); return -1; }
    return launch_channel_wgrad_finish((const float*)parts, gw, gb, Ci, Co, nparts, accumulate, (hipStream_t)stream);
}

int uno_adam_step(float* p, const float* g, float* m, float* v, long long n, int is_complex, double lr, double beta1, double beta2,
                  double eps, double weight_decay, int step, void* stream) {
    if (n < 0 || step < 1 || !(beta1 >= 0.f && beta1 < 1.f) || !(beta2 >= 0.f && beta2 < 1.f)) {
        set_error("uno_adam_step: bad arguments n=%lld step=%d betas=(%g, %g)", n, step, beta1, beta2);
        return -1;
    }
    if (n == 0) return 0;
    if (!p || !g || !m || !v) { set_error("uno_adam_step: null pointer"); return -1; }
    return launch_adam(p, g, m, v, n, is_complex, lr, beta1, beta2, eps, weight_decay, step, (hipStream_t)stream);
}

int uno_adam_step_multi(int n_tensors, float* const* p, const float* const* g, float* const* m, float* const* v,
                        const long long* n, const int* is_complex, double lr, double beta1, double beta2, double eps,
                        double weight_decay, int step, void* stream) {
    if (n_tensors < 0 || (n_tensors > 0 && (!p || !g || !m || !v || !n || !is_complex))) {
        set_error("uno_adam_step_multi: bad arguments");
        return -1;
    }
    if (step < 1 || !(beta1 >= 0.f && beta1 < 1.f) || !(beta2 >= 0.f && beta2 < 1.f)) {
        set_error("uno_adam_step_multi: bad arguments step=%d betas=(%g, %g)", step, beta1, beta2);
        return -1;
    }
    for (int t = 0; t < n_tensors; ++t) {
        if (n[t] < 0) { set_error("uno_adam_step_multi: tensor %d has n=%lld", t, n[t]); return -1; }
        if (n[t] > 0 && (!p[t] || !g[t] || !m[t] || !v[t])) { set_error("uno_adam_step_multi: null pointer (tensor %d)", t); return -1; }
    }
    return launch_adam_multi(n_tensors, p, g, m, v, n, is_complex, lr, beta1, beta2, eps, weight_decay, step, (hipStream_t)stream);
}

int uno_adam_step_multi_dev(int n_tensors, float* const* p, const float* const* g, float* const* m, float* const* v,
                            const long long* n, const int* is_complex, double lr, double beta1, double beta2, double eps,
                            double weight_decay, int* step_counter, float* scalars, const double* hyper, void* stream) {
    if (n_tensors < 0 || (n_tensors > 0 && (!p || !g || !m || !v || !n || !is_complex)) || !step_counter || !scalars) {
        set_error("uno_adam_step_multi_dev: bad arguments");
        return -1;
    }
    if (!(beta1 >= 0.f && beta1 < 1.f) || !(beta2 >= 0.f && beta2 < 1.f)) { set_error("uno_adam_step_multi_dev: bad betas (%g, %g)", beta1, beta2); return -1; }
    for (int t = 0; t < n_tensors; ++t) {
        if (n[t] < 0) { set_error("uno_adam_step_multi_dev: tensor %d has n=%lld", t, n[t]); return -1; }
        if (n[t] > 0 && (!p[t] || !g[t] || !m[t] || !v[t])) { set_error("uno_adam_step_multi_dev: null pointer (tensor %d)", t); return -1; }
    }
    if (int rc = launch_adam_advance(step_counter, scalars, hyper, lr, eps, weight_decay, beta1, beta2, (hipStream_t)stream)) return rc;
    return launch_adam_multi(n_tensors, p, g, m, v, n, is_complex, lr, beta1, beta2, eps, weight_decay, 1, (hipStream_t)stream, scalars);
}

static int gelu_project_forward_impl(const void* pre, const float* w, const float* bias, void* out, int B, int C, long long P, int bf16, void* stream) {
    if (B < 0 || C < 1 || P < 0) { set_error("uno_gelu_project_forward: bad sizes B=%d C=%d P=%lld", B, C, P); return -1; }
    if (B == 0 || P == 0) return 0;
    if (!pre || !w || !out) { set_error("uno_gelu_project_forward: null pointer"); return -1; }
    return launch_gelu_project_fwd(pre, w, bias, out, B, C, P, bf16, (hipStream_t)stream);
}

int uno_gelu_project_forward(const float* pre, const float* w, const float* bias, float* out, int B, int C, long long P, void* stream) {
    return gelu_project_forward_impl(pre, w, bias, out, B, C, P, 0, stream);
}

int uno_gelu_project_forward_bf16(const void* pre, const float* w, const float* bias, void* out, int B, int C, long long P, void* stream) {
    return gelu_project_forward_impl(pre, w, bias, out, B, C, P, 1, stream);
}

long long uno_gelu_project_bwd_ws_bytes(int B, int C, long long P) {
    if (B < 1 || C < 1 || P < 1) return 0;
    return 4LL * gelu_project_ws_floats(B, C, P);
}

static int gelu_project_backward_impl(const void* pre, const float* w, const void* gout, void* gpre, float* gw, float* gb, void* ws, int B,
                                      int C, long long P, int bf16, void* stream, const PixelWindow& win = PixelWindow()) {
    if (B < 0 || C < 1 || P < 0) { set_error("uno_gelu_project_backward: bad sizes B=%d C=%d P=%lld", B, C, P); return -1; }
    if (!gw) { set_error("uno_gelu_project_backward: null pointer"); return -1; }
    if (B == 0 || P == 0) {
        if (hipMemsetAsync(gw, 0, sizeof(float) * C, (hipStream_t)stream) != hipSuccess ||
            (gb && hipMemsetAsync(gb, 0, sizeof(float), (hipStream_t)stream) != hipSuccess)) { set_error("uno_gelu_project_backward: memset failed"); return -5; }
        return 0;
    }
    if (!pre || !w || !gout || !gpre || !ws) { set_error("uno_gelu_project_backward: null pointer"); return -1; }
    return launch_gelu_project_bwd(pre, w, gout, gpre, gw, gb, (float*)ws, B, C, P, bf16, (hipStream_t)stream, win);
}

int uno_gelu_project_backward_win(const float* pre, const float* w, const float* gout, float* gpre, float* gw, float* gb, void* ws, int B,
                                  int C, int rows, int cols, int pitch, long long plane, void* stream) {
    PixelWindow win; long long P;
    if (!make_window("uno_gelu_project_backward_win", rows, cols, pitch, plane, &win, &P)) return -1;
// ... 240 lines not shown
```

uno_amd/csrc/lift_bwd.hip:

```cpp
#include "uno_common.h"
#include <cstdlib>

namespace uno {

constexpr int LB_PT = 128;
constexpr int LB_TS = 148;
constexpr int LB_CM = 32, LB_CO = 64;
constexpr int LB_WS = 80, LB_WTS = 48;
#ifndef UNO_LB_TPW
#define UNO_LB_TPW 8
#endif
constexpr int LB_TPW = UNO_LB_TPW;

struct LiftGeom {
    int H, W, W4, nslot, npt;
    int skip_d, skip_p;
    int Pd, Pp;
    unsigned magic;
};
static LiftGeom lift_geom(int H, int W, int Hp, int Wp, int slots_per_row = 0) {
    LiftGeom g;
    g.H = H; g.W = W; g.W4 = slots_per_row ? slots_per_row : ((W + 3) & ~3); g.nslot = H * g.W4; g.npt = (g.nslot + 127) / 128;
    g.skip_d = W - g.W4; g.skip_p = Wp - g.W4; g.Pd = H * W; g.Pp = Hp * Wp;
    g.magic = (unsigned)(((1ULL << 40) + g.W4 - 1) / (unsigned long long)g.W4);
    return g;
}
__device__ __forceinline__ int lift_clamped(int off, int plane_len) { return max(min(off, plane_len - 4), 0); }
struct LiftQuad { int nv, od, op, row_ok, last, shd, shp; };
__device__ __forceinline__ LiftQuad lift_quad(const LiftGeom& g, int s0, int s) {
    const int r0 = (int)(((unsigned long long)(unsigned)s0 * g.magic) >> 40);
    const int r = r0 + (s >= (r0 + 1) * g.W4 ? 1 : 0);
    const int col = s - r * g.W4;
    const int od = s + r * g.skip_d, op = s + r * g.skip_p, odc = lift_clamped(od, g.Pd), opc = lift_clamped(op, g.Pp);
    return LiftQuad{r < g.H ? min(max(g.W - col, 0), 4) : 0, odc, opc, r < g.H ? 1 : 0, col == g.W4 - 4 ? 1 : 0, od - odc, op - opc};
}
__device__ __forceinline__ float4 lift_fix(const float4& v, int sh) {
    float t0 = v.x, t1 = v.y, t2 = v.z, t3 = v.w;
    if (sh & 1) { t0 = t1; t1 = t2; t2 = t3; }
    if (sh & 2) { t0 = t2; t1 = t3; }
    return make_float4(t0, t1, t2, t3);
}
__device__ __forceinline__ float4 lift_mask(const float4& v, int nv) {
    return make_float4(nv > 0 ? v.x : 0.f, nv > 1 ? v.y : 0.f, nv > 2 ? v.z : 0.f, nv > 3 ? v.w : 0.f);
}

struct LiftBwdParams {
    const float* x;
    const float* w1;
    const float* b1;
    const float* w0;
    const float* b0;
    const float* g;
    const float* g2;
    float* part;
    float* part1;
    int B, Cin;
    LiftGeom geo;
    unsigned long long* stamps;
    int rev;
};

__device__ __forceinline__ float4 lb_vh(const float4& t, const float4* q) {
    return make_float4(fmaf(t.z, q[2].x, fmaf(t.y, q[1].x, fmaf(t.x, q[0].x, t.w))), fmaf(t.z, q[2].y, fmaf(t.y, q[1].y, fmaf(t.x, q[0].y, t.w))),
                       fmaf(t.z, q[2].z, fmaf(t.y, q[1].z, fmaf(t.x, q[0].z, t.w))), fmaf(t.z, q[2].w, fmaf(t.y, q[1].w, fmaf(t.x, q[0].w, t.w))));
}

__device__ __forceinline__ void lb_gelu_both(float x, float& g, float& d) {
    const float cdf = 0.5f * (1.f + uno_erf(x * 0.70710678118654752440f));
    g = x * cdf;
    d = fmaf(x, 0.39894228040143267794f * __expf(-0.5f * x * x), cdf);
}

__global__ __launch_bounds__(256, 2) void lift_backward_kernel(LiftBwdParams p) {
    extern __shared__ __attribute__((aligned(16))) float lb_smem[];
    float* sA = lb_smem;
    float* sZ = sA + LB_CM * LB_TS;
    float* sW = sZ + LB_CO * LB_TS;
    float* sWT = sW + LB_CM * LB_WS;
    float4* sVH = reinterpret_cast<float4*>(sWT + LB_CO * LB_WTS);
    const int tid = threadIdx.x, lane = tid & 63, r16 = lane & 15, kk = lane >> 4;
    const int wave = __builtin_amdgcn_readfirstlane(tid >> 6);
    const int b = sweep_y(p.rev), bxs = sweep_x(p.rev);
    const LiftGeom& G = p.geo;

#pragma unroll
    for (int u = 0; u < 8; ++u) {
        const int e = tid + 256 * u, o = e >> 5, m = e & 31;
        const float v = p.w0[e];
        sW[m * LB_WS + o] = v;
        sWT[o * LB_WTS + m] = v;
    }
    if (tid < LB_CM) {
        const float* wr = p.w1 + tid * p.Cin;
        sVH[tid] = make_float4(wr[0], p.Cin > 1 ? wr[1] : 0.f, p.Cin > 2 ? wr[2] : 0.f, p.b1 ? p.b1[tid] : 0.f);
    }
    const float b0v = p.b0 ? p.b0[16 * wave + r16] : 0.f;
    const float* xb = p.x + (size_t)b * p.Cin * G.Pd;
    const float* gb = p.g + (size_t)b * LB_CO * G.Pp;
    const float* gb2 = p.g2 ? p.g2 + (size_t)b * LB_CO * G.Pp : nullptr;

    f32x4 acc3[2] = {f32x4{0, 0, 0, 0}, f32x4{0, 0, 0, 0}};
    float bsum = 0.f;

#ifdef UNO_LB_DEV
    unsigned long long tph[8] = {0, 0, 0, 0, 0, 0, 0, 0}, t_prev = __builtin_readcyclecounter();
#define LB_STAMP(i) do { asm volatile("s_waitcnt lgkmcnt(0)" ::: "memory"); const unsigned long long t_ = __builtin_readcyclecounter(); tph[i] += t_ - t_prev; t_prev = t_; } while (0)
#else
#define LB_STAMP(i) do { } while (0)
#endif
    const int t_begin = bxs * LB_TPW, t_end = min(t_begin + LB_TPW, G.npt);
    float4 xq[3], gq[8];
    float4 xc[3];
    float g1[4][4];
#pragma unroll
    for (int u = 0; u < 4; ++u)
#pragma unroll
        for (int k = 0; k < 4; ++k) g1[u][k] = 0.f;
    LiftQuad cur = {0, 0, 0, 0, 0, 0, 0}, nxt = {0, 0, 0, 0, 0, 0, 0};
    auto load_tile = [&](int tile) {
        const int s0 = tile * LB_PT;
        nxt = lift_quad(G, s0, s0 + (tid & 31) * 4);
#pragma unroll
        for (int k = 0; k < 3; ++k) xq[k] = io_ld4(xb + (size_t)min(k, p.Cin - 1) * G.Pd + nxt.od);
#pragma unroll
        for (int u = 0; u < 8; ++u) gq[u] = io_ld4(gb + (size_t)((tid >> 5) + 8 * u) * G.Pp + nxt.op);
    };
    if (t_begin < t_end) load_tile(t_begin);
    __syncthreads();
    for (int tile = t_begin; tile < t_end; ++tile) {
        cur = nxt;
#pragma unroll
        for (int k = 0; k < 3; ++k) { xq[k] = lift_fix(xq[k], cur.shd); xc[k] = lift_mask(xq[k], cur.nv); }
        float4 dh[4];
        {
            const int q4 = (tid & 31) * 4;
            const float vm0 = cur.nv > 0 ? 1.f : 0.f, vm1 = cur.nv > 1 ? 1.f : 0.f, vm2 = cur.nv > 2 ? 1.f : 0.f, vm3 = cur.nv > 3 ? 1.f : 0.f;
#pragma unroll
            for (int u = 0; u < 4; ++u) {
                const int m = (tid >> 5) + 8 * u;
                const float4 h = lb_vh(sVH[m], xq);
                float4 a4;
                lb_gelu_both(h.x, a4.x, dh[u].x); lb_gelu_both(h.y, a4.y, dh[u].y); lb_gelu_both(h.z, a4.z, dh[u].z); lb_gelu_both(h.w, a4.w, dh[u].w);
                *reinterpret_cast<float4*>(sA + m * LB_TS + q4) = make_float4(a4.x * vm0, a4.y * vm1, a4.z * vm2, a4.w * vm3);
            }
#pragma unroll
            for (int u = 0; u < 8; ++u) *reinterpret_cast<float4*>(sZ + ((tid >> 5) + 8 * u) * LB_TS + q4) = lift_mask(lift_fix(gq[u], cur.shp), cur.nv);
        }
        if (gb2) {
#pragma unroll
            for (int u = 0; u < 8; ++u) gq[u] = io_ld4(gb2 + (size_t)((tid >> 5) + 8 * u) * G.Pp + cur.op);
        } else if (tile + 1 < t_end) load_tile(tile + 1);
        LB_STAMP(0);
        __syncthreads();
        LB_STAMP(1);
        f32x4 acc1[8];
#pragma unroll
        for (int mt = 0; mt < 8; ++mt) acc1[mt] = f32x4{0, 0, 0, 0};
        float wv[LB_CM / 4];
#pragma unroll
        for (int ks = 0; ks < LB_CM / 4; ++ks) wv[ks] = sW[(4 * ks + kk) * LB_WS + 16 * wave + r16];
#pragma unroll
        for (int ks = 0; ks < LB_CM / 4; ++ks) {
            const float* arow = sA + (4 * ks + kk) * LB_TS + r16;
#pragma unroll
            for (int mt = 0; mt < 4; ++mt) acc1[mt] = mfma16(arow[16 * mt], wv[ks], acc1[mt]);
        }
        LB_STAMP(2);
        if (gb2) {
            const int q4 = (tid & 31) * 4;
#pragma unroll
            for (int u = 0; u < 8; ++u) {
                float4* dst = reinterpret_cast<float4*>(sZ + ((tid >> 5) + 8 * u) * LB_TS + q4);
                const float4 a = *dst, b2 = lift_mask(lift_fix(gq[u], cur.shp), cur.nv);
                *dst = make_float4(a.x + b2.x, a.y + b2.y, a.z + b2.z, a.w + b2.w);
            }
            if (tile + 1 < t_end) load_tile(tile + 1);
            __syncthreads();
        }
        float* const zrow = sZ + (16 * wave + r16) * LB_TS + 4 * kk;
        auto gz_tile = [&](int mt) {
            const float4 g4 = *reinterpret_cast<const float4*>(zrow + 16 * mt);
            const float4 gz = make_float4(uno_dgelu(acc1[mt][0] + b0v) * g4.x, uno_dgelu(acc1[mt][1] + b0v) * g4.y,
                                          uno_dgelu(acc1[mt][2] + b0v) * g4.z, uno_dgelu(acc1[mt][3] + b0v) * g4.w);
            *reinterpret_cast<float4*>(zrow + 16 * mt) = gz;
            bsum += (gz.x + gz.y) + (gz.z + gz.w);
        };
        __builtin_amdgcn_sched_barrier(0);
#pragma unroll
        for (int ks = 0; ks < LB_CM / 4; ++ks) {
            const float* arow = sA + (4 * ks + kk) * LB_TS + r16;
#pragma unroll
            for (int mt = 4; mt < 8; ++mt) acc1[mt] = mfma16(arow[16 * mt], wv[ks], acc1[mt]);
        }
#pragma unroll
        for (int mt = 0; mt < 4; ++mt) gz_tile(mt);
        __builtin_amdgcn_sched_group_barrier(0x100, 36, 0);
#pragma unroll
        for (int i = 0; i < 32; ++i) {
            __builtin_amdgcn_sched_group_barrier(0x008, 1, 0);
            __builtin_amdgcn_sched_group_barrier(0x002, 11, 0);
        }
        __builtin_amdgcn_sched_barrier(0);
#pragma unroll
        for (int mt = 4; mt < 8; ++mt) gz_tile(mt);
        LB_STAMP(3);
        __syncthreads();
        LB_STAMP(1);
        const int wp = wave >> 1, wm = wave & 1;
        f32x4 acc2[4];
#pragma unroll
        for (int mt = 0; mt < 4; ++mt) acc2[mt] = f32x4{0, 0, 0, 0};
#pragma unroll 4
        for (int ks = 0; ks < LB_CO / 4; ++ks) {
            const float wv = sWT[(4 * ks + kk) * LB_WTS + 16 * wm + r16];
            const float* zrow = sZ + (4 * ks + kk) * LB_TS + 64 * wp + r16;
#pragma unroll
            for (int mt = 0; mt < 4; ++mt) acc2[mt] = mfma16(zrow[16 * mt], wv, acc2[mt]);
        }
        LB_STAMP(4);
        {
            const float* zr = sZ + (16 * wave + r16) * LB_TS + kk;
            const float* a0 = sA + r16 * LB_TS + kk;
            const float* a1 = sA + (16 + r16) * LB_TS + kk;
#pragma unroll 8
            for (int ks = 0; ks < LB_PT / 4; ++ks) {
                const float zv = zr[4 * ks];
                acc3[0] = mfma16(zv, a0[4 * ks], acc3[0]);
                acc3[1] = mfma16(zv, a1[4 * ks], acc3[1]);
            }
        }
        LB_STAMP(5);
        __syncthreads();
        LB_STAMP(1);
#pragma unroll
        for (int mt = 0; mt < 4; ++mt)
            *reinterpret_cast<float4*>(sA + (16 * wm + r16) * LB_TS + 64 * wp + 16 * mt + 4 * kk) = make_float4(acc2[mt][0], acc2[mt][1], acc2[mt][2], acc2[mt][3]);
        LB_STAMP(6);
        __syncthreads();
        LB_STAMP(1);
        {
            const int q4 = (tid & 31) * 4;
#pragma unroll
            for (int u = 0; u < 4; ++u) {
                const int m = (tid >> 5) + 8 * u;
                float4 v = *reinterpret_cast<const float4*>(sA + m * LB_TS + q4);
                v = lift_mask(make_float4(v.x * dh[u].x, v.y * dh[u].y, v.z * dh[u].z, v.w * dh[u].w), cur.nv);
#pragma unroll
                for (int k = 0; k < 3; ++k) g1[u][k] = fmaf(v.x, xc[k].x, fmaf(v.y, xc[k].y, fmaf(v.z, xc[k].z, fmaf(v.w, xc[k].w, g1[u][k]))));
                g1[u][3] += (v.x + v.y) + (v.z + v.w);
            }
        }
        LB_STAMP(7);
        __syncthreads();
        LB_STAMP(1);
    }
#ifdef UNO_LB_DEV
    if (p.stamps && lane == 0) {
        unsigned long long* o_ = p.stamps + (((size_t)b * gridDim.x + blockIdx.x) * 4 + wave) * 8;
        for (int i = 0; i < 8; ++i) o_[i] = tph[i];
    }
#endif
    float* part = p.part + ((size_t)b * gridDim.x + bxs) * (LB_CO * (LB_CM + 1));
#pragma unroll
    for (int t = 0; t < 2; ++t)
#pragma unroll
        for (int r = 0; r < 4; ++r) part[(16 * wave + 4 * kk + r) * (LB_CM + 1) + 16 * t + r16] = acc3[t][r];
    bsum += __shfl_xor(bsum, 16);
    bsum += __shfl_xor(bsum, 32);
    if (kk == 0) part[(16 * wave + r16) * (LB_CM + 1) + LB_CM] = bsum;
    float* part1 = p.part1 + ((size_t)b * gridDim.x + bxs) * (LB_CM * (p.Cin + 1));
#pragma unroll
    for (int u = 0; u < 4; ++u)
#pragma unroll
        for (int k = 0; k < 4; ++k) {
            float v = g1[u][k];
            v += __shfl_xor(v, 1); v += __shfl_xor(v, 2); v += __shfl_xor(v, 4); v += __shfl_xor(v, 8); v += __shfl_xor(v, 16);
            if ((tid & 31) == 0) {
                const int m = (tid >> 5) + 8 * u;
                if (k < p.Cin) part1[m * (p.Cin + 1) + k] = v;
                else if (k == 3) part1[m * (p.Cin + 1) + p.Cin] = v;
            }
        }
}

struct LiftFwdParams {
    const float* x; const float* w1; const float* b1; const float* w0; const float* b0;
    float* act;
    int B, Cin, tail;
    LiftGeom geo;
    unsigned long long* stamps;
    int rev;
};

__global__ __launch_bounds__(256, 2) void lift_forward_kernel(LiftFwdParams p) {
    extern __shared__ __attribute__((aligned(16))) float lb_smem[];
    float* sA = lb_smem;
    float* sO = sA + LB_CM * LB_TS;
    float* sW = sO + LB_CO * LB_TS;
    float4* sVH = reinterpret_cast<float4*>(sW + LB_CM * LB_WS);
    const int tid = threadIdx.x, lane = tid & 63, r16 = lane & 15, kk = lane >> 4;
    const int wave = __builtin_amdgcn_readfirstlane(tid >> 6);
    const int b = sweep_y(p.rev), bxs = sweep_x(p.rev);
    const LiftGeom& G = p.geo;
#pragma unroll
    for (int u = 0; u < 8; ++u) {
        const int e = tid + 256 * u;
        sW[(e & 31) * LB_WS + (e >> 5)] = p.w0[e];
    }
    if (tid < LB_CM) {
        const float* wr = p.w1 + tid * p.Cin;
        sVH[tid] = make_float4(wr[0], p.Cin > 1 ? wr[1] : 0.f, p.Cin > 2 ? wr[2] : 0.f, p.b1 ? p.b1[tid] : 0.f);
    }
    const float b0v = p.b0 ? p.b0[16 * wave + r16] : 0.f;
    const float* xb = p.x + (size_t)b * p.Cin * G.Pd;
    float* ab = p.act + (size_t)b * LB_CO * G.Pp;
    float4 xqA[3], xqB[3];
    LiftQuad qdA = {0, 0, 0, 0, 0, 0, 0}, qdB = {0, 0, 0, 0, 0, 0, 0};
    auto load_x = [&](int tile, float4* xq, LiftQuad& qd) {
        const int s0 = tile * LB_PT;
        qd = lift_quad(G, s0, s0 + (tid & 31) * 4);
#pragma unroll
        for (int k = 0; k < 3; ++k) xq[k] = io_ld4(xb + (size_t)min(k, p.Cin - 1) * G.Pd + qd.od);
    };
#ifdef UNO_LB_DEV
    unsigned long long tph[8] = {0, 0, 0, 0, 0, 0, 0, 0}, t_prev = __builtin_readcyclecounter();
#endif
    const int t_begin = bxs * LB_TPW, t_end = min(t_begin + LB_TPW, G.npt);
    if (t_begin < t_end) load_x(t_begin, xqA, qdA);
    if (t_begin + 1 < t_end) load_x(t_begin + 1, xqB, qdB);
    __syncthreads();
    auto do_tile = [&](int tile, float4* xq, LiftQuad& qd) {
        const LiftQuad cur = qd;
        {
            const int q4 = (tid & 31) * 4;
            const float4 q[3] = {lift_mask(lift_fix(xq[0], cur.shd), cur.nv), lift_mask(lift_fix(xq[1], cur.shd), cur.nv), lift_mask(lift_fix(xq[2], cur.shd), cur.nv)};
#pragma unroll
            for (int u = 0; u < 4; ++u) {
                const int m = (tid >> 5) + 8 * u;
                const float4 h = lb_vh(sVH[m], q);
                *reinterpret_cast<float4*>(sA + m * LB_TS + q4) = make_float4(uno_gelu(h.x), uno_gelu(h.y), uno_gelu(h.z), uno_gelu(h.w));
            }
        }
        if (tile + 2 < t_end) load_x(tile + 2, xq, qd);
        LB_STAMP(0);
        __syncthreads();
        LB_STAMP(1);
        f32x4 acc1[8];
#pragma unroll
        for (int mt = 0; mt < 8; ++mt) acc1[mt] = f32x4{0, 0, 0, 0};
        float wv[LB_CM / 4];
#pragma unroll
        for (int ks = 0; ks < LB_CM / 4; ++ks) wv[ks] = sW[(4 * ks + kk) * LB_WS + 16 * wave + r16];
#pragma unroll
        for (int ks = 0; ks < LB_CM / 4; ++ks) {
            const float* arow = sA + (4 * ks + kk) * LB_TS + r16;
#pragma unroll
            for (int mt = 0; mt < 4; ++mt) acc1[mt] = mfma16(arow[16 * mt], wv[ks], acc1[mt]);
        }
        LB_STAMP(2);
        float* const orow = sO + (16 * wave + r16) * LB_TS + 4 * kk;
        auto out_tile = [&](int mt) {
            *reinterpret_cast<float4*>(orow + 16 * mt) = make_float4(uno_gelu(acc1[mt][0] + b0v), uno_gelu(acc1[mt][1] + b0v),
                                                                     uno_gelu(acc1[mt][2] + b0v), uno_gelu(acc1[mt][3] + b0v));
        };
        __builtin_amdgcn_sched_barrier(0);
#pragma unroll
        for (int ks = 0; ks < LB_CM / 4; ++ks) {
            const float* arow = sA + (4 * ks + kk) * LB_TS + r16;
#pragma unroll
            for (int mt = 4; mt < 8; ++mt) acc1[mt] = mfma16(arow[16 * mt], wv[ks], acc1[mt]);
        }
#pragma unroll
        for (int mt = 0; mt < 4; ++mt) out_tile(mt);
        __builtin_amdgcn_sched_group_barrier(0x100, 32, 0);
#pragma unroll
        for (int i = 0; i < 32; ++i) {
            __builtin_amdgcn_sched_group_barrier(0x008, 1, 0);
            __builtin_amdgcn_sched_group_barrier(0x002, 7, 0);
        }
        __builtin_amdgcn_sched_barrier(0);
#pragma unroll
        for (int mt = 4; mt < 8; ++mt) out_tile(mt);
        LB_STAMP(3);
        __syncthreads();
        LB_STAMP(1);
        if (cur.row_ok) {
            const int q4 = (tid & 31) * 4;
#pragma unroll
            for (int u = 0; u < 8; ++u) {
                const int o = (tid >> 5) + 8 * u;
                const float4 v = lift_mask(*reinterpret_cast<const float4*>(sO + o * LB_TS + q4), cur.nv);
                float* dst = ab + (size_t)o * G.Pp + cur.op;
                io_store4(dst, v.x, v.y, v.z, v.w);
                if (cur.last) {
                    if (p.tail > 0) dst[4] = 0.f;
                    if (p.tail > 1) dst[5] = 0.f;
                    if (p.tail > 2) dst[6] = 0.f;
                }
            }
        }
        LB_STAMP(7);
        __syncthreads();
        LB_STAMP(1);
    };
    for (int tile = t_begin; tile < t_end; tile += 2) {
        do_tile(tile, xqA, qdA);
        if (tile + 1 < t_end) do_tile(tile + 1, xqB, qdB);
    }
#ifdef UNO_LB_DEV
    if (p.stamps && lane == 0) {
        unsigned long long* o_ = p.stamps + (((size_t)b * gridDim.x + blockIdx.x) * 4 + wave) * 8;
        for (int i = 0; i < 8; ++i) o_[i] = tph[i];
    }
#endif
}

int launch_lift_forward_fused(const float* x, const float* w1, const float* b1, const float* w0, const float* b0, float* act, int B, int Cin,
                              int H, int W, int Hp, int Wp, hipStream_t s) {
    LiftFwdParams p;
    p.x = x; p.w1 = w1; p.b1 = b1; p.w0 = w0; p.b0 = b0; p.act = act;
    p.B = B; p.Cin = Cin; p.geo = lift_geom(H, W, Hp, Wp, Wp & ~3); p.tail = Wp & 3;
    p.stamps = nullptr;
    p.rev = next_sweep_reversed(SWEEP_LIFT);
#ifdef UNO_LB_DEV
    if (getenv("UNO_LF_STAMPS")) p.stamps = reinterpret_cast<unsigned long long*>((uintptr_t)strtoull(getenv("UNO_LF_STAMPS"), nullptr, 0));
#endif
    if ((long long)Hp * Wp * LB_CO >= (1LL << 31) || B > 65535 || (long long)H * Wp >= (1LL << 24)) { set_error("lift_forward: tensor too large"); return -2; }
    static int lds_slot[64];
    const size_t lds = sizeof(float) * (LB_CM * LB_TS + LB_CO * LB_TS + LB_CM * LB_WS) + sizeof(float4) * LB_CM;
    if (!ensure_dynamic_lds(reinterpret_cast<const void*>(lift_forward_kernel), lds, lds_slot)) { set_error("lift_forward: cannot raise dynamic LDS to %zu", lds); return -4; }
    {
        ProfScope prof("uno::lift_forward_kernel", 4.0 * B * ((double)H * W * Cin + (double)H * Wp * LB_CO), s);
        hipLaunchKernelGGL(lift_forward_kernel, dim3((unsigned)((p.geo.npt + LB_TPW - 1) / LB_TPW), (unsigned)B), dim3(256), lds, s, p);
    }
    const hipError_t e = hipGetLastError();
    if (e != hipSuccess) { set_error("lift_forward launch: %s", hipGetErrorString(e)); return -5; }
    return 0;
}

static size_t lift_bwd_lds() { return sizeof(float) * (LB_CM * LB_TS + LB_CO * LB_TS + LB_CM * LB_WS + LB_CO * LB_WTS) + sizeof(float4) * LB_CM; }

bool lift_bwd_fused_applies(int Cin, int Cm, int Co, int W, long long P) {
    return Cin >= 1 && Cin <= 3 && Cm == LB_CM && Co == LB_CO && W >= 260 && P >= LB_PT && P < (1LL << 24) - (1 << 16);
}

long long lift_bwd_fused_parts(int B, int H, int W) {
    const long long npt = ((long long)H * ((W + 3) & ~3) + LB_PT - 1) / LB_PT;
    return (long long)B * ((npt + LB_TPW - 1) / LB_TPW);
}

int launch_lift_backward_fused(const float* x, const float* w1, const float* b1, const float* w0, const float* b0, const float* g, float* part,
                               float* part1, int B, int Cin, int H, int W, int Hp, int Wp, hipStream_t s, const float* g2) {
    LiftBwdParams p;
    p.x = x; p.w1 = w1; p.b1 = b1; p.w0 = w0; p.b0 = b0; p.g = g; p.g2 = g2; p.part = part; p.part1 = part1;
    p.B = B; p.Cin = Cin; p.geo = lift_geom(H, W, Hp, Wp);
    p.stamps = nullptr;
    p.rev = next_sweep_reversed(SWEEP_LIFT);
#ifdef UNO_LB_DEV
    if (getenv("UNO_LB_STAMPS")) p.stamps = reinterpret_cast<unsigned long long*>((uintptr_t)strtoull(getenv("UNO_LB_STAMPS"), nullptr, 0));
#endif
    if ((long long)Hp * Wp * LB_CO >= (1LL << 31) || B > 65535) { set_error("lift_backward: tensor too large"); return -2; }
    static int lds_slot[64];
    const size_t lds = lift_bwd_lds();
    if (!ensure_dynamic_lds(reinterpret_cast<const void*>(lift_backward_kernel), lds, lds_slot)) { set_error("lift_backward: cannot raise dynamic LDS to %zu", lds); return -4; }
    {
        ProfScope prof("uno::lift_backward_kernel", 4.0 * B * (double)H * W * (Cin + LB_CO * (g2 ? 2 : 1)), s);
        hipLaunchKernelGGL(lift_backward_kernel, dim3((unsigned)((p.geo.npt + LB_TPW - 1) / LB_TPW), (unsigned)B), dim3(256), lds, s, p);
    }
    const hipError_t e = hipGetLastError();
    if (e != hipSuccess) { set_error("lift_backward launch: %s", hipGetErrorString(e)); return -5; }
    return 0;
}

}
```

uno_amd/csrc/uno_common.h:

```cpp
#pragma once
#include <hip/hip_runtime.h>
#include <stdint.h>

namespace uno {

typedef float f32x4 __attribute__((ext_vector_type(4)));

__device__ __forceinline__ f32x4 mfma16(float a, float b, f32x4 c) {
    return __builtin_amdgcn_mfma_f32_16x16x4f32(a, b, c, 0, 0, 0);
}

__device__ __forceinline__ float uno_erf(float x) {
    x = __builtin_fminf(__builtin_fmaxf(x, -4.f), 4.f);
    const float t = x * x;
    float p = -2.72614225801306e-10f;
    p = fmaf(p, t, 2.77068142495902e-08f);
    p = fmaf(p, t, -2.10102402082508e-06f);
    p = fmaf(p, t, -5.69250639462346e-05f);
    p = fmaf(p, t, -7.34990630326855e-04f);
    p = fmaf(p, t, -2.95459980854025e-03f);
    p = fmaf(p, t, -1.60960333262415e-02f);
    p *= x;
    float q = -1.45660718464996e-05f;
    q = fmaf(q, t, -2.13374055278905e-04f);
// ... 159 lines not shown
    int accumulate;
};

struct CdftParams {
    const float* in = nullptr;
    float* out = nullptr;
    const float2* tw = nullptr;
    int n_img = 0, H = 0, C = 0, m1 = 0, m2 = 0, m3 = 0;
    float scale = 1.f;
    int mask = 0;
    const int* rowfreq = nullptr;
    int sp_group = 0, sp_stride = 0, sp_offset = 0;
};

__host__ __device__ __forceinline__ size_t grouped_volume(int vol, int group, int stride, int offset) {
    if (group <= 0) return (size_t)vol;
    return (size_t)(vol / group) * (size_t)stride + (size_t)offset + (size_t)(vol % group);
}

struct Vol3dParams {
    const float* in = nullptr;
    float* out = nullptr;
    const float2* tw1 = nullptr;
    const float2* tw2 = nullptr;
    const float2* tw3 = nullptr;
    int n_vol = 0, D1 = 0, D2 = 0, D3 = 0, m1 = 0, m2 = 0, m3 = 0;
    float scale = 1.f;
    int herm = 0;
    const float* ctab = nullptr;
    int sp_group = 0, sp_stride = 0, sp_offset = 0;
};

const float2* twiddle_table(int N);
void* upload_table(const void* host, size_t bytes);
float2 twiddle_value(long long n, int N);

inline bool ensure_dynamic_lds(const void* kernel, size_t bytes, int* slot) {
    if (bytes <= 64 * 1024) return true;
    int dev = 0;
    if (hipGetDevice(&dev) != hipSuccess || dev < 0 || dev >= 64) dev = 0;
    if ((size_t)__atomic_load_n(&slot[dev], __ATOMIC_RELAXED) >= bytes) return true;
    const int want = 160 * 1024;
    if (hipFuncSetAttribute(kernel, hipFuncAttributeMaxDynamicSharedMemorySize, want) != hipSuccess) return false;
    __atomic_store_n(&slot[dev], want, __ATOMIC_RELAXED);
    return true;
}
void set_error(const char* fmt, ...);
struct Scratch { void* ptr; size_t bytes; };
const Scratch& thread_scratch();
int reserved_cus();
int next_sweep_reversed(int family);
enum { SWEEP_K1 = 1, SWEEP_K3 = 2, SWEEP_K7 = 4, SWEEP_K8 = 8, SWEEP_K9 = 16, SWEEP_NORM = 32, SWEEP_PROJ = 64, SWEEP_LIFT = 128 };
inline int usable_cus(int device_cus) { const int r = reserved_cus(); return device_cus - r >= 8 ? device_cus - r : (device_cus < 8 ? device_cus : 8); }

struct ProfScope {
    int slot;
    hipStream_t stream;
    ProfScope(const char* name, double bytes, hipStream_t s);
    ~ProfScope();
};

int launch_dft2d_fwd(const Dft2dParams& p, hipStream_t s);
int launch_dft2d_inv(const Dft2dParams& p, hipStream_t s);
bool dft2d_inv_add_applies(const Dft2dParams& p);
int launch_dft2d_inv_add(const Dft2dParams& p, hipStream_t s);
bool dft2d_fwd_fd_applies(const Dft2dParams& p);
int launch_dft2d_fwd_fd(const Dft2dParams& p, hipStream_t s);
int launch_spectrum_crop(const float* src, float* dst, int n_img, int M1, int M2, int m1, int m2, int s_group, int s_stride, int s_offset,
                         int d_group, int d_stride, int d_offset, hipStream_t s);
bool dft2d_fwd_plane_applies(const Dft2dParams& p);
bool dft2d_inv_plane_applies(const Dft2dParams& p);
bool dft2d_b16_applies(const Dft2dParams& p);
int launch_dft2d_fwd_b16(const Dft2dParams& p, hipStream_t s);
int launch_dft2d_inv_b16(const Dft2dParams& p, hipStream_t s);
int launch_dft2d_fwd_plane(const Dft2dParams& p, hipStream_t s);
int launch_dft2d_inv_plane(const Dft2dParams& p, hipStream_t s);
bool vol3d_fwd_applies(int n_vol, int D1, int D2, int D3, int m1, int m2, int m3);
bool vol3d_inv_applies(int n_vol, int D1, int D2, int D3, int m1, int m2, int m3);
int launch_dft3d_fwd_volume(const Vol3dParams& p, hipStream_t s);
int launch_dft3d_inv_volume(const Vol3dParams& p, hipStream_t s);
int launch_mode_gemm(const ModeGemmParams& p, hipStream_t s);
int launch_mode_gemm_pair(const ModeGemmParams& input_grad, const ModeGemmParams& weight_grad, hipStream_t s);
int launch_cdft(const CdftParams& p, bool inverse, hipStream_t s);
int launch_dft2d_generic(const Dft2dParams& p, bool inverse, void* ws, size_t ws_bytes, hipStream_t s);
int launch_cdft_generic(const CdftParams& p, bool inverse, hipStream_t s);
void resample3d_any_lds_bytes(int D1, int D2, int D3, int M1, int M2, int M3, int J1, int J2, int m3, size_t out[3]);
void resample3d_wide_lds_bytes(int D1, int D2, int D3, int M1, int M2, int M3, int J1, int J2, int m3, size_t out[3]);
int launch_resample3d_any(const float* x, float* y, float* y_act, int accumulate, void* ws, int n_vol, int D1, int D2, int D3, int M1, int M2, int M3, int J1,
                          const int* f1_in, const int* f1_out, int J2, const int* f2_in, const int* f2_out, int m3, float scale,
                          int herm_in, int herm_out, hipStream_t s);
int launch_resample3d_wide(const float* x, float* y, float* y_act, int accumulate, void* ws, int n_vol, int D1, int D2, int D3, int M1, int M2, int M3,
                           int J1, const int* f1_in, const int* f1_out, int J2, const int* f2_in, const int* f2_out, int m3, float scale,
                           int herm_in, int herm_out, hipStream_t s);
long long ns2d_ws_bytes(int B, int N);
int launch_ns2d_forward(const float* w, float* w_h, void* ws, int B, int N, hipStream_t s);
int launch_ns2d_inverse(const float* w_h, float* w, void* ws, int B, int N, hipStream_t s);
int launch_ns2d_steps(float* w_h, const float* f_h, int f_batched, void* ws, int B, int N, long long n_steps, double visc, double delta_t,
                      hipStream_t s);
int launch_resample2d(const void* in, void* out, float* tmp, int n_img, int H, int W, int Ho, int Wo, const int* startH,
                      const float* wtH, int KH, const int* startW, const float* wtW, int KW, const int* tile_p0,
                      const float* tile_w, int NP, int accumulate, int bf16, hipStream_t s);
struct ChannelMixArgs {
    const void* x; const void* x2; const float* w; const float* bias; void* y; void* y2; void* y_act; const void* dgelu_of;
    const float* proj_w; const float* proj_b; void* proj_out;
    int B, Ci, Co, C1, Co1; long long P; int transpose_w, accumulate, act_in, bf16;
    PixelWindow win;
    void* ws = nullptr; size_t ws_bytes = 0;
    const float* vh_x = nullptr; const float* vh_w = nullptr; const float* vh_b = nullptr; int vh_ci = 0, vh_mode = 0;
    const void* gmul = nullptr;
    const float* pb_w2 = nullptr; const float* pb_g = nullptr;
    int act_cols = 0, act_pitch = 0; long long act_plane = 0;
};
int launch_clear_border(float* t, long long n_planes, int Hp, int Wp, int rows, int cols, hipStream_t s);
int launch_channel_mix2(const ChannelMixArgs& a, hipStream_t s);
int launch_channel_mix(const void* x, const float* w, const float* bias, void* y, int B, int Ci, int Co, long long P,
                       int transpose_w, int accumulate, int act_in, const void* dgelu_of, int bf16, hipStream_t s, void* ws = nullptr,
                       size_t ws_bytes = 0);
long long channel_mix_ws_bytes(int Ci, int Co, long long P, int bf16);
int launch_adam_multi(int n_tensors, float* const* p, const float* const* g, float* const* m, float* const* v, const long long* n,
                      const int* is_complex, double lr, double beta1, double beta2, double eps, double wd, int step, hipStream_t s,
                      const float* dev_scalars = nullptr);
int launch_adam_advance(int* step, float* scalars, const double* hyper, double lr, double eps, double wd, double beta1, double beta2,
                        hipStream_t s);
int launch_adam(float* p, const float* g, float* m, float* v, long long n, int is_complex, double lr, double beta1, double beta2,
                double eps, double wd, int step, hipStream_t s);
struct GeluProjectSecond { const void* s = nullptr; void* gs = nullptr; int C1 = 0, act = 0; };
int launch_gelu_project_fwd(const void* pre, const float* w, const float* bias, void* out, int B, int C, long long P, int bf16, hipStream_t s,
                            const GeluProjectSecond* two = nullptr);
long long gelu_project_ws_floats(int B, int C, long long P);
int launch_gelu_project_bwd(const void* pre, const float* w, const void* gout, void* gpre, float* gw, float* gb, float* ws, int B,
                            int C, long long P, int bf16, hipStream_t s, const PixelWindow& win = PixelWindow(),
                            const GeluProjectSecond* two = nullptr);
int launch_gelu_pad(const void* s, const void* gy, void* out, int n_img, int H, int W, int Hp, int Wp, int backward, int bf16, hipStream_t st);
int launch_transpose_batched(const float* in, float* out, int B, long long R, int C, long long ld_in, long long sb_in, long long ld_out,
                             long long sb_out, hipStream_t st);
int launch_instnorm_fwd(const void* x, const float* gamma, const float* beta, void* y, float* mean, float* rstd, long long rows, int C,
                        long long N, float eps, int gelu, int bf16, hipStream_t s);
int launch_instnorm_bwd(const void* x, const void* gy, const float* gamma, const float* beta, const float* mean, const float* rstd,
                        void* gx, float* s1, float* s2, long long rows, int C, long long N, int gelu, int bf16, hipStream_t s);
long long channel_wgrad_ws_floats(int B, int Ci, int Co, long long P, int* nsplit_out);
int launch_channel_wgrad(const void* gy, const void* x, float* gw, float* gb, float* ws, int B, int Ci, int Co, long long P,
                         int act_x, int bf16, hipStream_t s);
struct WgradProjectedBack { const float* w2 = nullptr; const float* g = nullptr; float* gw2 = nullptr; float* gb2 = nullptr; };
bool channel_wgrad_pb_applies(int B, int Ci, int Co, int C1, long long P);
long long channel_wgrad_pb_ws_floats(int B, int Ci, int Co, long long P);
int launch_channel_wgrad2(const void* gy, const void* x, const void* x2, int C1, float* gw, float* gb, float* ws, int B, int Ci, int Co,
                          long long P, int act_x, int accumulate, int bf16, hipStream_t s, const PixelWindow& win = PixelWindow(),
                          const WgradProjectedBack& pb = WgradProjectedBack());
int launch_channel_wgrad_vh(const void* gy, const float* vh_x, const float* vh_w, const float* vh_b, int vh_ci, float* gw, float* gb, float* ws,
                            int B, int Ci, int Co, long long P, int act_x, hipStream_t s, int accumulate = 0);
bool lift_bwd_fused_applies(int Cin, int Cm, int Co, int W, long long P);
long long lift_bwd_fused_parts(int B, int H, int W);
int launch_lift_forward_fused(const float* x, const float* w1, const float* b1, const float* w0, const float* b0, float* act, int B, int Cin,
                              int H, int W, int Hp, int Wp, hipStream_t s);
int launch_lift_backward_fused(const float* x, const float* w1, const float* b1, const float* w0, const float* b0, const float* g, float* part,
                               float* part1, int B, int Cin, int H, int W, int Hp, int Wp, hipStream_t s, const float* g2 = nullptr);
int launch_channel_wgrad_finish(const float* parts, float* gw, float* gb, int Ci, int Co, long long nparts, int accumulate, hipStream_t s);
long long rel_l2_steps_chunks(long long P, int T, long long* chunk_pixels);
long long rel_l2_steps_ws_floats(int B, long long P, int T);
int launch_rel_l2_steps(const float* pred, const float* target, float* sums, float* rel, float* totals, float* ws, int B, long long P, int T,
                        hipStream_t s);
int launch_rel_l2_steps_finish(const float* ws, float* sums, float* rel, float* totals, int B, int T, long long nc, hipStream_t s);
long long rollout_chunks(long long P, long long* chunk_pixels);
long long rollout_ws_floats(int B, long long P, int T);
int launch_rollout_advance(float* window, const float* frame, const float* target, float* pred, float* ws, int B, int C, int T_in, long long P,
                           int T, int t, int shift, hipStream_t s);
long long rollout_lift_bwd_ws_floats(int B, int C, int Cm, long long P, int T);
int launch_rollout_lift(const float* given, const float* pred, const float* feat, const float* w, const float* bias, float* h, int B, int T_in,
                        int F, int Cm, long long P, int T, int t, hipStream_t s);
int launch_rollout_lift_backward(const float* gh, const float* given, const float* pred, const float* target, const float* feat, const float* w,
                                 const float* sums, const float* gL, float* gpred, float* gframe, float* parts, int B, int T_in, int F, int Cm,
                                 long long P, int T, int t, hipStream_t s);
int launch_rollout_loss_seed(const float* pred, const float* target, const float* sums, const float* gL, float* gframe, int B, long long P, int T,
                             hipStream_t s);
long long rel_l2_chunks(long long N, long long* chunk_elems);
long long rel_l2_ws_floats(int B, long long N);
int launch_rel_l2_forward(const float* x, long long xrs, long long xes, const float* y, long long yrs, long long yes, float* sums, float* ratio,
                          float* total, float* ws, int B, long long N, hipStream_t s);
int launch_rel_l2_backward(const float* x, long long xrs, long long xes, const float* y, long long yrs, long long yes, const float* sums,
                           const float* g, int per_row, float scale, float* gx, int B, long long N, hipStream_t s);

}
```

uno_amd/harness/__init__.py:

```python
from .models import UNO, UNO_9, UNO_P, UNO_S256, Uno3D_T9, Uno3D_T10, Uno3D_T20, Uno3D_T40
from .optim import ComplexAdam
from .losses import LpLoss, RolloutErrors, StepErrors, lp_loss_rel_sum, rel_l2, step_errors
from .mixed import MixedDarcyTrainer
from .train import DarcyTrainer, GraphedRollout, GraphedStep, ns2d_evaluate, ns2d_rollout_errors, ns2d_rollout_loss, ns3d_evaluate, ns3d_loss, ns3d_step_error, synthetic_darcy_batch
from .datagen import GaussianRF, generate_ns_dataset, navier_stokes_2d
from . import workloads
```

uno_amd/harness/losses.py:

```python
from typing import NamedTuple, Optional

import torch


def lp_loss_rel_sum(pred: torch.Tensor, target: torch.Tensor) -> torch.Tensor:
    n = pred.shape[0]
    diff = torch.linalg.vector_norm(pred.reshape(n, -1) - target.reshape(n, -1), ord=2, dim=1)
    return (diff / torch.linalg.vector_norm(target.reshape(n, -1), ord=2, dim=1)).sum()


def _rows(t: torch.Tensor) -> Optional[torch.Tensor]:
    if t.dim() < 1 or t.shape[0] == 0 or t.numel() == 0:
        return None
    try:
        return t.view(t.shape[0], -1)
    except RuntimeError:
        return None


def _native_rows(x: torch.Tensor, y: torch.Tensor):
    if not (x.is_cuda and y.is_cuda and x.device == y.device and x.dtype == torch.float32 and y.dtype == torch.float32
            and x.shape == y.shape and not (y.requires_grad and torch.is_grad_enabled())):
        return None
    xr, yr = _rows(x), _rows(y)
    return None if xr is None or yr is None else (xr, yr)


class _RelL2Fn(torch.autograd.Function):

    @staticmethod
    def forward(ctx, x, y, reduce):
        from .. import _native
        record = _native.rel_l2_forward(x, y)
        ctx.save_for_backward(x, y, record)
        ctx.reduce = reduce
        B = x.shape[0]
        if reduce == 0:
            return record[2 * B:3 * B]
        return record[3 * B] if reduce == 1 else record[3 * B] / B

    @staticmethod
    @torch.autograd.function.once_differentiable
    def backward(ctx, g):
        from .. import _native
        if not ctx.needs_input_grad[0]:
            return None, None, None
        x, y, record = ctx.saved_tensors
        if g.dtype != torch.float32:
            g = g.to(torch.float32)
        if g.dim() == 1 and g.shape[0] > 1 and g.stride(0) == 0:
            g = g[:1]
        elif not g.is_contiguous():
            g = g.contiguous()
        return _native.rel_l2_backward(x, y, record, g, 1.0 / x.shape[0] if ctx.reduce == 2 else 1.0), None, None


def rel_l2(x: torch.Tensor, y: torch.Tensor) -> torch.Tensor:
    rows = _native_rows(x, y)
    if rows is None:
        n = x.shape[0]
        diff = torch.linalg.vector_norm(x.reshape(n, -1) - y.reshape(n, -1), ord=2, dim=1)
        return diff / torch.linalg.vector_norm(y.reshape(n, -1), ord=2, dim=1)
    return _RelL2Fn.apply(rows[0], rows[1], 0)


class LpLoss(object):

    def __init__(self, d=2, p=2, size_average=True, reduction=True):
        super(LpLoss, self).__init__()
        assert d > 0 and p > 0
        self.d = d
        self.p = p
        self.reduction = reduction
        self.size_average = size_average

    def rel(self, x, y):
        rows = _native_rows(x, y) if self.p == 2 else None
        if rows is not None:
            return _RelL2Fn.apply(rows[0], rows[1], 0 if not self.reduction else (2 if self.size_average else 1))
        n = x.size()[0]
        ratio = torch.linalg.vector_norm(x.reshape(n, -1) - y.reshape(n, -1), ord=self.p, dim=1) \
            / torch.linalg.vector_norm(y.reshape(n, -1), ord=self.p, dim=1)
        if self.reduction:
            return torch.mean(ratio) if self.size_average else torch.sum(ratio)
        return ratio

    def __call__(self, x, y):
        return self.rel(x, y)


class StepErrors(NamedTuple):
    sums: torch.Tensor
    per_step: torch.Tensor
    full: torch.Tensor
    step_sum: torch.Tensor
    full_sum: torch.Tensor


class RolloutErrors(NamedTuple):
    errors: StepErrors
    pred: Optional[torch.Tensor]


NATIVE_STEP_ERRORS_MAX_T = 256


def _step_errors_stock(pred: torch.Tensor, target: torch.Tensor) -> StepErrors:
    B, T = pred.shape[0], pred.shape[-1]
    sums = torch.empty((B, T, 2), dtype=pred.dtype, device=pred.device)
    per_step = torch.empty((B, T), dtype=pred.dtype, device=pred.device)
    step_sum = torch.zeros((), dtype=pred.dtype, device=pred.device)
    for t in range(T):
        k, l = pred[..., t].reshape(B, -1), target[..., t].reshape(B, -1)
        d = k - l
        sums[:, t, 0], sums[:, t, 1] = (d * d).sum(dim=1), (l * l).sum(dim=1)
        per_step[:, t] = torch.linalg.vector_norm(d, ord=2, dim=1) / torch.linalg.vector_norm(l, ord=2, dim=1)
        step_sum = step_sum + per_step[:, t].sum()
    p, y = pred.reshape(B, -1), target.reshape(B, -1)
    full = torch.linalg.vector_norm(p - y, ord=2, dim=1) / torch.linalg.vector_norm(y, ord=2, dim=1)
    return StepErrors(sums, per_step, full, step_sum, full.sum())


def step_errors(pred: torch.Tensor, target: torch.Tensor) -> StepErrors:
    if pred.shape != target.shape or pred.dim() < 2:
        raise RuntimeError(f"step_errors: pred {tuple(pred.shape)} and target {tuple(target.shape)} must be equal (B, ..., T) shapes")
    pred, target = pred.detach(), target.detach()
    if not (pred.is_cuda and target.is_cuda and pred.dtype == torch.float32 and target.dtype == torch.float32
            and 1 <= pred.shape[-1] <= NATIVE_STEP_ERRORS_MAX_T and pred.shape[0] > 0 and pred[0].numel() > 0):
        return _step_errors_stock(pred, target)
    from .. import _native
    sums, rel, totals = _native.rel_l2_steps(pred.contiguous(), target.contiguous())
    T = pred.shape[-1]
    return StepErrors(sums, rel[:, :T], rel[:, T], totals[0], totals[1])
```

uno_amd/harness/mixed.py:

```python
from __future__ import annotations

import time

import torch

from ..integral_operators import enable_mixed_precision
from .losses import lp_loss_rel_sum
from .models import UNO_9
from .train import DarcyTrainer, synthetic_darcy_batch


class MixedDarcyTrainer(DarcyTrainer):

    def __init__(self, model, **kw):
        enable_mixed_precision(model)
        super().__init__(model, **kw)

    def step(self, a, u):
        B = a.shape[0]
        ab = a.to(torch.bfloat16)
        return self.step_with(lambda: lp_loss_rel_sum(self.model(ab).reshape(B, -1).float(), u.reshape(B, -1)))


def c5_mixed_model_bench(dev, B: int = 4, S: int = 1024, steps: int = 4, warmup: int = 2):
    torch.manual_seed(0)
    torch.cuda.synchronize(dev)
    torch.cuda.empty_cache()
    torch.cuda.reset_peak_memory_stats(dev)
    model = UNO_9(3, 64, pad=5).to(dev)
    tr = MixedDarcyTrainer(model, lr=1e-3, weight_decay=1e-3)
    a, u = synthetic_darcy_batch(B, S, 1234, dev)
    for _ in range(warmup):
        tr.step(a, u)
    torch.cuda.synchronize(dev)
    t0 = time.perf_counter()
    for _ in range(steps):
        loss = tr.step(a, u)
    torch.cuda.synchronize(dev)
    ms = (time.perf_counter() - t0) / steps * 1e3
    lv = float(loss)
    assert lv == lv, "mixed-precision training produced NaN"
    return {"config": f"C5 model: UNO_9(3,64,pad=5) at {S}^2, batch {B}, bf16 activations + fp16 spectral weights, f32 accumulation "
                      "and f32 master weights / Adam", "ms_per_step": ms, "samples_per_s": B / ms * 1e3,
            "peak_mem_GiB": torch.cuda.max_memory_allocated(dev) / 2 ** 30, "final_loss": lv}
```

uno_amd/harness/models.py:

```python
from __future__ import annotations

import math

import torch
import torch.nn as nn
import torch.nn.functional as F

from ..integral_operators import (GradJoin, SpectrumShare, OperatorBlock_2D, OperatorBlock_3D, channel_mix, channel_mix_cat, channel_mix_cat_project,
                                  enable_native_resample3d_any, enable_native_resample3d_wide, enable_one_buffer_any_grid, gelu_channel_mix, gelu_channel_mix_pad, gelu_pad2d, gelu_project, gelu_project2,
                                  lift_gelu_pad)
from ..pointwise import gelu_channel_mix_pad_last

NATIVE_ENDS_3D = False


def enable_native_ends_3d(model: nn.Module, enabled: bool = True) -> nn.Module:
    for m in model.modules():
        if isinstance(m, Uno3D_T20):
            m.native_ends = bool(enabled)
    return model


CAT_FREE_SKIPS_3D = False


def enable_cat_free_skips_3d(model: nn.Module, enabled: bool = True) -> nn.Module:
    for m in model.modules():
        if isinstance(m, Uno3D_T20):
            m.cat_free_skips = bool(enabled)
    return model


def _block_cat(block, xs, *dims):
    if hasattr(block, "forward_cat"):
        return block.forward_cat(xs, *dims)
    return block(torch.cat(list(xs), dim=1), *dims)


def _cached(cache: dict, key, build):
    grid = cache.get(key)
    if grid is None:
        grid = build()
        cache.clear()
        cache[key] = grid
    return grid


class UNO_9(nn.Module):

    def __init__(self, in_width, width, pad=5, factor=1, block_cls=OperatorBlock_2D):
        super().__init__()
        self.in_width = in_width
        self.width = width
        self.padding = pad
        w, f = width, factor
        self.fc_n1 = nn.Linear(in_width, w // 2)
        self.fc0 = nn.Linear(w // 2, w)
        self.conv0 = block_cls(w, 2 * f * w, 40, 40, 18, 18)
        self.conv1 = block_cls(2 * f * w, 4 * f * w, 20, 20, 8, 8, Normalize=True)
        self.conv2 = block_cls(4 * f * w, 4 * f * w, 20, 20, 8, 8)
        self.conv4 = block_cls(4 * f * w, 2 * f * w, 40, 40, 8, 8, Normalize=True)
        self.conv5 = block_cls(4 * f * w, w, 85, 85, 18, 18)
        self.fc1 = nn.Linear(2 * w, w)
        self.fc2 = nn.Linear(w, 1)
        self._grid_cache = {}

    def get_grid(self, shape, device):
        def build():
            b, sx, sy = shape[0], shape[1], shape[2]
            gx = torch.linspace(0, 1, sx, dtype=torch.float64).to(torch.float32).reshape(1, sx, 1, 1).expand(b, sx, sy, 1)
            gy = torch.linspace(0, 1, sy, dtype=torch.float64).to(torch.float32).reshape(1, 1, sy, 1).expand(b, sx, sy, 1)
            return torch.cat((gx, gy), dim=-1).contiguous().to(device)
        return _cached(self._grid_cache, (tuple(shape[:3]), str(device)), build)

    def forward(self, x):
        S1, S2 = x.shape[1], x.shape[2]
        x = torch.cat((x, self.get_grid(x.shape, x.device).to(x.dtype)), dim=-1).permute(0, 3, 1, 2).contiguous()
        scale = math.ceil(S2 / 85)
        margin = scale * self.padding
        product = hasattr(self.conv5, "forward_cat")
        fused = product and self.conv5.non_lin and not self.conv5.normalize
        jl = GradJoin() if fused else None
        lifted = lift_gelu_pad(x, self.fc_n1, self.fc0, margin, margin, grad_join=jl)
        d1, d2 = lifted.shape[-2], lifted.shape[-1]

        if fused:
            jc, j2 = GradJoin(), GradJoin()
            c0 = self.conv0(lifted, d1 // 2, d2 // 2, join=jl, out_join=jc)
            sc = SpectrumShare.for_block(self.conv5, self.conv4.conv.out_channels)
            c1 = self.conv1(c0, d1 // 4, d2 // 4, join=jc, share=sc)
            c2 = self.conv2(c1, d1 // 4, d2 // 4, out_join=j2)
            skip5 = [self.conv4(c2, d1 // 2, d2 // 2, join=j2), c0]
            out = channel_mix_cat_project([self.conv5.forward_cat(skip5, d1, d2, defer_gelu=True, defer_grad=jc, share=sc), lifted], self.fc1.weight,
                                          self.fc1.bias, self.fc2.weight, self.fc2.bias, gelu_first=True, defer_grad=jl, crop=(S1, S2))
            return out[:, :, :S1, :S2].permute(0, 2, 3, 1).contiguous()
        else:
            c0 = self.conv0(lifted, d1 // 2, d2 // 2)
            c1 = self.conv1(c0, d1 // 4, d2 // 4)
            c2 = self.conv2(c1, d1 // 4, d2 // 4)
            skip5 = [self.conv4(c2, d1 // 2, d2 // 2), c0]
            c5 = channel_mix_cat([_block_cat(self.conv5, skip5, d1, d2), lifted], self.fc1.weight, self.fc1.bias)
        out = gelu_project(c5, self.fc2.weight, self.fc2.bias)
        return out[:, :, :S1, :S2].permute(0, 2, 3, 1).contiguous()


class UNO(nn.Module):

    _BLOCKS = ((48, 48, 22, 22), (32, 32, 14, 14), (16, 16, 6, 6), (16, 16, 6, 6), (32, 32, 6, 6), (48, 48, 14, 14), (64, 64, 22, 22))
    _LIFT = None
    _FC1 = 4
    _TWO_SOURCE = False

    def __init__(self, in_width, width, pad=0, factor=3 / 4, block_cls=OperatorBlock_2D):
        super().__init__()
        self.in_width, self.width, self.factor, self.padding = in_width, width, factor, pad
        w, f = width, factor
        lift = w // 2 if self._LIFT is None else self._LIFT
        self.fc = nn.Linear(in_width, lift)
        self.fc0 = nn.Linear(lift, w)
        cin = (w, 2 * f * w, 4 * f * w, 8 * f * w, 8 * f * w, 8 * f * w, 4 * f * w)
        cout = (2 * f * w, 4 * f * w, 8 * f * w, 8 * f * w, 4 * f * w, 2 * f * w, w)
        for i, row in enumerate(self._BLOCKS):
            setattr(self, f"L{i}", block_cls(cin[i], cout[i], *row))
        self.fc1 = nn.Linear(2 * w, self._FC1 * w)
        self.fc2 = nn.Linear(self._FC1 * w + (lift if self._TWO_SOURCE else 0), 1)
        self._grid_cache = {}

    def get_grid(self, shape, device):
        def build():
            b, sx, sy = shape[0], shape[1], shape[2]
            gx = torch.linspace(0, 2 * math.pi, sx, dtype=torch.float64).to(torch.float32).reshape(1, sx, 1, 1).expand(b, sx, sy, 1)
            gy = torch.linspace(0, 2 * math.pi, sy, dtype=torch.float64).to(torch.float32).reshape(1, 1, sy, 1).expand(b, sx, sy, 1)
            return torch.cat((torch.sin(gx), torch.sin(gy), torch.cos(gx), torch.cos(gy)), dim=-1).contiguous().to(device)
        return _cached(self._grid_cache, (tuple(shape[:3]), str(device)), build)

    def _grids(self, d1, d2):
        a, b, c = (int(d1 * self.factor), int(d2 * self.factor)), (d1 // 2, d2 // 2), (d1 // 4, d2 // 4)
        return a, b, c, c, b, a, (d1, d2)

    def forward(self, x):
        z = torch.cat((x.permute(0, 3, 1, 2), self.get_grid(x.shape, x.device).permute(0, 3, 1, 2)), dim=1)
        return self.forward_cf(z).permute(0, 2, 3, 1).contiguous()

    def forward_cf(self, x):
        return self.body_cf(channel_mix(x, self.fc.weight, self.fc.bias))

    def body_cf(self, h):
        lifted = F.gelu(gelu_channel_mix(h, self.fc0.weight, self.fc0.bias))
        p = self.padding
        if p != 0:
            lifted = F.pad(lifted, [p, p, p, p])
        g = self._grids(lifted.shape[-2], lifted.shape[-1])
        c0 = self.L0(lifted, *g[0])
        c1 = self.L1(c0, *g[1])
        if hasattr(self.L6, "forward_cat") and all(b.non_lin and not b.normalize for b in (self.L2, self.L3)):
            j2, j3 = GradJoin(), GradJoin()
            c2 = self.L2(c1, *g[2], out_join=j2)
            c3 = self.L3(c2, *g[3], join=j2, out_join=j3)
            c4 = self.L4(c3, *g[4], join=j3)
        else:
            c4 = self.L4(self.L3(self.L2(c1, *g[2]), *g[3]), *g[4])
        c4 = torch.cat([c4, c1], dim=1)
        c5 = torch.cat([self.L5(c4, *g[5]), c0], dim=1)
        c6 = torch.cat([self.L6(c5, *g[6]), lifted], dim=1)
        if p != 0:
            c6 = c6[..., p:-p, p:-p] if self._TWO_SOURCE else c6[..., :-p, :-p]
        out = channel_mix(c6.contiguous(), self.fc1.weight, self.fc1.bias)
        if self._TWO_SOURCE:
            return gelu_project2(out, h, self.fc2.weight, self.fc2.bias, act2=True)
        return gelu_project(out, self.fc2.weight, self.fc2.bias)


class UNO_P(UNO):

    _BLOCKS = ((32, 32, 14, 14), (16, 16, 6, 6), (8, 8, 3, 3), (8, 8, 3, 3), (16, 16, 3, 3), (32, 32, 6, 6), (64, 64, 14, 14))
    _FC1, _TWO_SOURCE = 3, True
    _DIV = (2, 4, 8, 8, 4, 2, 1)

    def __init__(self, in_width, width, pad=0, factor=1, block_cls=OperatorBlock_2D):
        super().__init__(in_width, width, pad, factor, block_cls)

    def _grids(self, d1, d2):
        return [(d1 // k, d2 // k) for k in self._DIV]


class UNO_S256(UNO_P):

    _BLOCKS = ((64, 64, 32, 33), (16, 16, 8, 9), (8, 8, 4, 5), (8, 8, 4, 5), (16, 16, 4, 5), (64, 64, 8, 9), (256, 256, 32, 32))
    _LIFT = 16
    _DIV = (4, 16, 32, 32, 16, 4, 1)


def _grids3d(d1, d2, bottom, times):
    a, b, c = (int(3 * d1 / 4), int(3 * d2 / 4)), (d1 // 2, d2 // 2), (d1 // 4, d2 // 4)
    return [(*s, t) for s, t in zip((a, b, c, bottom, b, a, (d1, d2)), times)]


class Uno3D_T20(nn.Module):

    _NAMES = ("conv0", "conv1", "conv2", "conv3", "conv6", "conv7", "conv8")
    _NORMALIZED = ("conv0", "conv3", "conv7")
    _WIDTHS = (2, 4, 8, 16, 4, 2)
    _SKIPS = {"conv6": "conv1", "conv7": "conv0", "conv8": None}
    _BLOCKS = ((48, 48, 10, 22, 22, 5), (32, 32, 10, 14, 14, 5), (16, 16, 12, 6, 6, 5), (16, 16, 12, 6, 6, 6), (32, 32, 18, 6, 6, 6),
               (48, 48, 20, 14, 14, 8), (64, 64, 20, 22, 22, 8))

    @staticmethod
    def _lift_width(in_width, width):
        return in_width * 2

    @staticmethod
    def _plan(d1, d2, d3, padding):
        return _grids3d(d1, d2, (d1 // 4, d2 // 4), (d3, d3, int(d3 * 1.2), int(d3 * 1.2), int(d3 * 1.8), int(2.0 * d3), 2 * d3)), 2 * padding

    def __init__(self, in_width, width, pad=2, factor=1, pad_both=False, block_cls=OperatorBlock_3D):
        super().__init__()
        self.in_width, self.width, self.pad, self.pad_both = in_width, width, pad, pad_both
        w, f = width, factor
        lift = self._lift_width(in_width, w)
        self.fc = nn.Linear(in_width, lift)
        self.fc0 = nn.Linear(lift, w)
        cout = dict(zip(self._NAMES, [m * f * w for m in self._WIDTHS] + [2 * w]))
        cin = w
        for name, row in zip(self._NAMES, self._BLOCKS):
            setattr(self, name, block_cls(cin, cout[name], *row, Normalize=name in self._NORMALIZED))
            cin = cout[name] + (cout.get(self._SKIPS[name], w) if name in self._SKIPS else 0)
        self.fc1 = nn.Linear(3 * w, 4 * w)
        self.fc2 = nn.Linear(4 * w, 1)
        self._grid_cache = {}

    def get_grid(self, shape, device):
        def build():
            b, sx, sy, sz = shape[0], shape[1], shape[2], shape[3]
            lin = lambda hi, n: torch.linspace(0, hi, n, dtype=torch.float64).to(torch.float32)
            gx = lin(2 * math.pi, sx).reshape(1, sx, 1, 1, 1).expand(b, sx, sy, sz, 1)
            gy = lin(2 * math.pi, sy).reshape(1, 1, sy, 1, 1).expand(b, sx, sy, sz, 1)
# ... 135 lines not shown
```

uno_amd/harness/train.py:

```python
from __future__ import annotations

import time

import torch
import torch.distributed as dist
from torch.autograd.function import once_differentiable

from .losses import NATIVE_STEP_ERRORS_MAX_T, RolloutErrors, StepErrors, _step_errors_stock, lp_loss_rel_sum, step_errors
from .optim import ComplexAdam


def synthetic_darcy_batch(batch, S, seed, device, dtype=torch.float32):
    g = torch.Generator(device="cpu").manual_seed(seed)
    a = torch.rand(batch, S, S, 1, generator=g, dtype=dtype)
    u = torch.rand(batch, S, S, generator=g, dtype=dtype)
    return a.to(device), u.to(device)


class FlatGradients:

    def __init__(self, params, bucket_mb: float = 32.0, comm_dtype=None):
        self.comm_dtype = comm_dtype
        self.params = [p for p in params if p.requires_grad]
        sizes = [p.numel() * (2 if p.is_complex() else 1) for p in self.params]
        dev = self.params[0].device
        n_cplx = sum(1 for p in self.params if p.is_complex())
        self.flat = torch.zeros(sum(sizes) + n_cplx, dtype=torch.float32, device=dev)
        offsets = []
        self.views = []
        off = 0
        for p, n in zip(self.params, sizes):
            if p.is_complex() and off % 2:
                off += 1
            seg = self.flat[off:off + n]
            if p.is_complex():
                view = torch.view_as_complex(seg.view(*p.shape, 2))
            else:
                assert p.dtype == torch.float32
                view = seg.view(p.shape)
            p.grad = None
            p._uno_grad_buffer = view
            self.views.append(view)
            offsets.append(off)
            off += n
        limit = int(bucket_mb * (1 << 20) / 4)
        self.buckets = []
        self._bucket_of = {}
        end = off
        count = 0
        members = []
        for i in range(len(self.params) - 1, -1, -1):
            members.append(i)
            count += sizes[i]
            if count >= limit or i == 0:
                for j in members:
                    self._bucket_of[j] = len(self.buckets)
                self.buckets.append((offsets[i], end))
                end = offsets[i]
                count = 0
                members = []
        self._bucket_params = [sum(1 for b in self._bucket_of.values() if b == k) for k in range(len(self.buckets))]
        self._pending = list(self._bucket_params)
        self._next = 0
        self._works = []
        self._group = None
        self._armed = False
        self._hooks = []
        self.trace = None
        self._t_arm = 0.0

    def zero_(self):
        for p in self.params:
            p.grad = None

    def collect(self, only=None):
        pairs = zip(self.params, self.views) if only is None else ((self.params[only], self.views[only]),)
        for p, view in pairs:
            g = p.grad
            if g is None:
                if only is None:
                    view.zero_()
            elif g.data_ptr() != view.data_ptr():
                view.copy_(g)
                p.grad = view.view(view.shape)

    def arm(self, group=None, force=False):
        if self._works:
            self.abort()
        self._armed = bool(dist.is_available() and dist.is_initialized() and (force or dist.get_world_size(group) > 1))
        if not self._armed:
            return
        self._group = group
        self._t_arm = time.perf_counter()
        self._pending = list(self._bucket_params)
        self._next = 0
        self._works = []
        if not self._hooks:
            for i, p in enumerate(self.params):
                self._hooks.append(p.register_post_accumulate_grad_hook(self._make_hook(i)))

    def _make_hook(self, i):
        k = self._bucket_of[i]

        def hook(_param):
            if self._armed:
                self.collect(i)
                self._pending[k] -= 1
                self._issue_ready()
        return hook

    def _issue(self, k):
        a, b = self.buckets[k]
        if self.trace is not None:
            self.trace.append(time.perf_counter() - self._t_arm)
        if self.comm_dtype is None:
            self._works.append((dist.all_reduce(self.flat[a:b], op=dist.ReduceOp.SUM, group=self._group, async_op=True), None, a, b))
        else:
            low = self.flat[a:b].to(self.comm_dtype)
            self._works.append((dist.all_reduce(low, op=dist.ReduceOp.SUM, group=self._group, async_op=True), low, a, b))

    def _issue_ready(self):
        while self._next < len(self.buckets) and self._pending[self._next] <= 0:
            self._issue(self._next)
            self._next += 1

    def finish(self):
        self.collect()
        if not self._armed:
            return
        while self._next < len(self.buckets):
            self._issue(self._next)
            self._next += 1
        for w, low, a, b in self._works:
            w.wait()
            if low is not None:
                self.flat[a:b].copy_(low)
        self._works = []
        self._armed = False

    def abort(self):
        for w, low, a, b in self._works:
            try:
                w.wait()
            except Exception:
                pass
        self._works = []
        self._armed = False
        self._next = 0
        self._pending = list(self._bucket_params)

    def all_reduce_sum(self, group=None, force=False):
        self.collect()
        if dist.is_available() and dist.is_initialized() and (force or dist.get_world_size(group) > 1):
            dist.all_reduce(self.flat, op=dist.ReduceOp.SUM, group=group)


def ns2d_rollout_loss(model, xx, yy, T_f, step=1, native=False):
    if native:
        return _rollout_loss_native(model, xx, yy, T_f, step)
    loss = 0
    B = yy.shape[0]
# ... 242 lines not shown


def ns3d_step_error(out, y):
    return step_errors(out, y).step_sum


def ns3d_loss(model, x, y, with_step_error=False):
    B, S, T_f = x.shape[0], x.shape[1], y.shape[-1]
    out = model(x).view(B, S, S, T_f)
    loss = lp_loss_rel_sum(out.reshape(B, -1), y.reshape(B, -1))
    if not with_step_error:
        return loss
    with torch.no_grad():
        return loss, ns3d_step_error(out.detach(), y.reshape(B, S, S, T_f))


def ns3d_evaluate(model, batches):
    was_training = model.training
    model.eval()
    total = None
    try:
        with torch.no_grad():
            for x, y in batches:
                B, S, T_f = x.shape[0], x.shape[1], y.shape[-1]
                err = ns3d_step_error(model(x).view(B, S, S, T_f), y.reshape(B, S, S, T_f))
                total = err if total is None else total + err
    finally:
        model.train(was_training)
    return total


class GraphedStep:

    def __init__(self, model, opt, loss_fn, example_inputs, warmup: int = 2):
        if not torch.cuda.is_available():
            raise RuntimeError("GraphedStep needs the GPU (HIP graph capture)")
        self.model, self.opt, self.loss_fn = model, opt, loss_fn
        self.opt_in_graph = bool(getattr(opt, "capturable", False))
        if self.opt_in_graph:
            opt.init_state()
        self.static_in = tuple(t.clone() for t in example_inputs)
        side = torch.cuda.Stream()
        side.wait_stream(torch.cuda.current_stream())
        with torch.cuda.stream(side):
            for _ in range(warmup):
                opt.zero_grad(set_to_none=True)
                loss_fn(*self.static_in).backward()
        torch.cuda.current_stream().wait_stream(side)
        torch.cuda.synchronize()
        opt.zero_grad(set_to_none=True)
        self.graph = torch.cuda.CUDAGraph()
        with torch.cuda.graph(self.graph):
            self.static_loss = loss_fn(*self.static_in)
            self.static_loss.backward()
            if self.opt_in_graph:
                self.opt.step()
        self._params = [p for g in opt.param_groups for p in g["params"] if p.requires_grad]

    def step(self, *inputs):
        for dst, src in zip(self.static_in, inputs):
            dst.copy_(src, non_blocking=True)
        if self.opt_in_graph:
            self.opt.sync_hyper()
        self.graph.replay()
        if self.opt_in_graph:
            torch.autograd.graph.increment_version(self._params)
        else:
            self.opt.step()
        return self.static_loss.detach().clone()


class GraphedRollout:

    def __init__(self, model, T_f, example_inputs, return_pred=False, warmup: int = 1):
        if not torch.cuda.is_available():
            raise RuntimeError("GraphedRollout needs the GPU (HIP graph capture)")
        xx, yy = example_inputs
        if not _rollout_native_applies(model, xx, yy, T_f, 1):
            raise RuntimeError("GraphedRollout captures the native roll-out only: float32 device tensors (B, S, S, T), a model with "
                               f"forward_cf / get_grid, 1 <= T_f <= {NATIVE_STEP_ERRORS_MAX_T}, a non-empty batch")
        self.model, self.T_f, self.return_pred = model, T_f, return_pred
        self.static_in = (xx.clone(), yy.clone())
        side = torch.cuda.Stream()
        side.wait_stream(torch.cuda.current_stream())
        with torch.cuda.stream(side):
            for _ in range(max(1, warmup)):
                ns2d_rollout_errors(model, *self.static_in, T_f, return_pred=return_pred)
        torch.cuda.current_stream().wait_stream(side)
        torch.cuda.synchronize()
        self.graph = torch.cuda.CUDAGraph()
        with torch.cuda.graph(self.graph), torch.no_grad():
            self._record, self._pred = _rollout_native(model, *self.static_in, T_f, return_pred)

    def _replay(self, xx, yy):
        for dst, src in zip(self.static_in, (xx, yy)):
            if dst.shape != src.shape:
                raise RuntimeError(f"GraphedRollout: captured for {tuple(dst.shape)}, got {tuple(src.shape)}")
            if src.data_ptr() != dst.data_ptr():
                dst.copy_(src, non_blocking=True)
        self.graph.replay()

    def errors(self, xx, yy) -> RolloutErrors:
        self._replay(xx, yy)
        return _rollout_result(self._record.clone(), self._pred.clone() if self._pred is not None else None, xx.shape[0], self.T_f)

    def evaluate(self, batches):
        total = None
        for xx, yy in batches:
            self._replay(xx, yy)
            totals = self._record[-2:]
            total = totals.clone() if total is None else total + totals
        return total[0], total[1]


class DarcyTrainer:

    def __init__(self, model, lr=1e-3, weight_decay=1e-3, group=None, force_collectives=False, bucket_mb=32.0, comm_dtype=None,
                 comm_cus=None):
        self.model = model
        self.group = group
        self.force_collectives = force_collectives
        self.grads = FlatGradients(model.parameters(), bucket_mb=bucket_mb, comm_dtype=comm_dtype)
        self.comm_cus = 0
        if dist.is_available() and dist.is_initialized() and dist.get_world_size(group) > 1 and next(model.parameters()).is_cuda:
            import os
            from .. import _native
            self.comm_cus = int(os.environ.get("UNO_COMM_CUS", 16 if comm_cus is None else comm_cus))
            _native.reserve_cus(self.comm_cus)
        self.opt = ComplexAdam(model.parameters(), lr=lr, weight_decay=weight_decay)
        self.broadcast_parameters()

    def broadcast_parameters(self):
        if dist.is_available() and dist.is_initialized() and (self.force_collectives or dist.get_world_size(self.group) > 1):
            for t in list(self.model.parameters()) + list(self.model.buffers()):
                dist.broadcast(torch.view_as_real(t.data) if t.is_complex() else t.data, src=0, group=self.group)

    def step_with(self, loss_closure):
        self.grads.zero_()
        loss = loss_closure()
        self.grads.arm(self.group, self.force_collectives)
        try:
            loss.backward()
        except BaseException:
            self.grads.abort()
            from ..integral_operators import release_pass_state
            release_pass_state()
            raise
        self.grads.finish()
        self.opt.step()
        return loss.detach()

    def step(self, a, u):
        B, S = a.shape[0], a.shape[1]
        return self.step_with(lambda: lp_loss_rel_sum(self.model(a).reshape(B, -1), u.reshape(B, -1)))

    def step_blocking(self, a, u):
        B = a.shape[0]
        self.grads.zero_()
        loss = lp_loss_rel_sum(self.model(a).reshape(B, -1), u.reshape(B, -1))
        loss.backward()
        self.grads.all_reduce_sum(self.group, self.force_collectives)
        self.opt.step()
        return loss.detach()
```

uno_amd/pointwise.py:

```python
from __future__ import annotations

import torch
import torch.nn as nn
import torch.nn.functional as F
from torch.autograd.function import once_differentiable

from . import _native
from ._param_grads import _layer_grad_targets, _stack_pointwise


_ACT = (torch.float32, torch.bfloat16)


def _dev_act(x: torch.Tensor) -> bool:
    return x.is_cuda and x.dtype in _ACT


def _plain(t: torch.Tensor) -> torch.Tensor:
    if t.is_complex() and t.is_conj():
        t = t.resolve_conj()
    if t.is_neg():
        t = t.resolve_neg()
    if t.is_contiguous():
        return t
# ... 411 lines not shown
        return y.view(B, w.shape[0], *x1.shape[2:])
    xs = list(xs)
    if defer_grad is not None:
        defer_grad.void()
    if gelu_first:
        xs[0] = F.gelu(xs[0])
    return channel_mix(torch.cat(xs, dim=1), weight, bias)


class _GeluChannelMixFn(torch.autograd.Function):

    @staticmethod
    def forward(ctx, pre, w, bias, leaves=None):
        pre, w = _plain(pre), _plain(w)
        y = _native.channel_mix(pre, w, None if bias is None else _plain(bias), act_in=True)
        ctx.save_for_backward(pre, w)
        ctx.has_bias = bias is not None
        ctx.leaves = leaves
        return y

    @staticmethod
    @once_differentiable
    def backward(ctx, gy):
        pre, w = ctx.saved_tensors
        gy = _plain(gy)
        g_pre = _native.channel_mix(gy, w, None, transpose_w=True, dgelu_of=pre) if ctx.needs_input_grad[0] else None
        gw, gb = _wgrad_into(ctx.leaves, gy, pre, None, ctx.needs_input_grad[1], ctx.has_bias and ctx.needs_input_grad[2], act_x=True)
        return g_pre, gw, gb, None


def gelu_channel_mix(pre: torch.Tensor, weight: torch.Tensor, bias: torch.Tensor | None) -> torch.Tensor:
    B, Ci = pre.shape[0], pre.shape[1]
    w = weight.reshape(weight.shape[0], Ci)
    if _dev_act(pre) and w.dtype == torch.float32:
        y = _GeluChannelMixFn.apply(pre.reshape(B, Ci, -1), w, bias, (weight, bias))
        return y.view(B, w.shape[0], *pre.shape[2:])
    return channel_mix(F.gelu(pre), weight, bias)


class _GeluChannelMixPadFn(torch.autograd.Function):

    @staticmethod
    def forward(ctx, pre, w, bias, Hp, Wp, leaves=None):
        pre, w = _plain(pre), _plain(w)
        bias = None if bias is None else _plain(bias)
        _, act = _native.channel_mix_act_padded(pre, w, bias, Hp, Wp, act_in=True, keep_y=False)
        ctx.save_for_backward(pre, w, bias)
        ctx.has_bias = bias is not None
        ctx.leaves = leaves
        return act

    @staticmethod
    @once_differentiable
    def backward(ctx, gact):
        pre, w, bias = ctx.saved_tensors
        B, Ci, Co = pre.shape[0], pre.shape[1], w.shape[0]
        gz = _native.channel_mix_dgelu_padded(pre, w, bias, _plain(gact), act_in=True).view(B, Co, -1)
        pre3 = pre.view(B, Ci, -1)
        g_pre = _native.channel_mix(gz, w, None, transpose_w=True, dgelu_of=pre3).view(pre.shape) if ctx.needs_input_grad[0] else None
        gw, gb = _wgrad_into(ctx.leaves, gz, pre3, None, ctx.needs_input_grad[1], ctx.has_bias and ctx.needs_input_grad[2], act_x=True)
        return g_pre, gw, gb, None, None, None


def gelu_channel_mix_pad(pre: torch.Tensor, weight: torch.Tensor, bias: torch.Tensor | None, pad_h: int, pad_w: int) -> torch.Tensor:
    if pre.dim() == 4 and _dev_act(pre) and weight.dtype == torch.float32 and pad_h >= 0 and pad_w >= 0:
        Hp, Wp = pre.shape[2] + int(pad_h), pre.shape[3] + int(pad_w)
        if _native.channel_mix_act_padded_ok(pre, Hp, Wp):
            return _GeluChannelMixPadFn.apply(pre, weight.reshape(weight.shape[0], pre.shape[1]), bias, Hp, Wp, (weight, bias))
    return gelu_pad2d(gelu_channel_mix(pre, weight, bias), pad_h, pad_w)


class _GeluChannelMixPadLastFn(torch.autograd.Function):

    @staticmethod
    def forward(ctx, pre, w, bias, window, leaves=None):
        pre, w = _plain(pre), _plain(w)
        y, act = _native.channel_mix_act_padded_rows(pre, w, None if bias is None else _plain(bias), window, act_in=True, keep_y=True)
        ctx.save_for_backward(pre, w, y)
        ctx.has_bias, ctx.window, ctx.leaves = bias is not None, window, leaves
        return act

    @staticmethod
    @once_differentiable
    def backward(ctx, gact):
        pre, w, y = ctx.saved_tensors
        gz = _native.dgelu_rows(y, _plain(gact), ctx.window)
        g_pre = _native.channel_mix(gz, w, None, transpose_w=True, dgelu_of=pre) if ctx.needs_input_grad[0] else None
        gw, gb = _wgrad_into(ctx.leaves, gz, pre, None, ctx.needs_input_grad[1], ctx.has_bias and ctx.needs_input_grad[2], act_x=True)
        return g_pre, gw, gb, None, None


def gelu_channel_mix_pad_last(pre: torch.Tensor, weight: torch.Tensor, bias: torch.Tensor | None, pad_left: int, pad_right: int) -> torch.Tensor:
    pl, pr = int(pad_left), int(pad_right)
    if pre.dim() >= 3 and pre.is_cuda and pre.dtype == torch.float32 and weight.dtype == torch.float32 and pl >= 0 and pr >= 0 and pre.numel() > 0:
        B, Ci, T = pre.shape[0], pre.shape[1], pre.shape[-1]
        rows = pre.numel() // (B * Ci * T)
        pitch = T + pl + pr
        Co = weight.shape[0]
        if _native.rows_window_ok(rows, T, pitch, pl, rows * pitch, Ci, Co):
            act = _GeluChannelMixPadLastFn.apply(pre.reshape(B, Ci, -1), weight.reshape(Co, Ci), bias, (rows, T, pitch, pl), (weight, bias))
            return act.view(B, Co, *pre.shape[2:-1], pitch)
    return F.pad(F.gelu(gelu_channel_mix(pre, weight, bias)), [pl, pr] + [0, 0] * (pre.dim() - 3))


class _LiftFn(torch.autograd.Function):

    @staticmethod
    def forward(ctx, x, w1, b1, w0, b0, Hp, Wp, grad_join=None):
        x, w1, w0 = _plain(x), _plain(w1), _plain(w0)
        b1 = None if b1 is None else _plain(b1)
        b0 = None if b0 is None else _plain(b0)
        ctx.save_for_backward(x, w1, w0, *[t for t in (b1, b0) if t is not None])
        ctx.has = (b1 is not None, b0 is not None)
        ctx.join = None
        if grad_join is not None:
            grad_join.accepts_extra = bool(_native.lift_backward_takes_second(x, w1, w0, Hp, Wp))
            grad_join.extra = []
            ctx.join = grad_join
        return _native.lift_forward(x, w1, b1, w0, b0, Hp, Wp)

    @staticmethod
    @once_differentiable
    def backward(ctx, gact):
        x, w1, w0, *bs = ctx.saved_tensors
        b1 = bs.pop(0) if ctx.has[0] else None
        b0 = bs.pop(0) if ctx.has[1] else None
        gact = _plain(gact)
        g2 = None
        if ctx.join is not None:
            ctx.join.accepts_extra = False
            H, W = x.shape[-2:]
            for t, (rows, cols, pitch) in ctx.join.take_extra():
                t = t.view(gact.shape)
                if g2 is None and rows >= H and cols >= W and pitch == gact.shape[-1]:
                    g2 = t
                else:
                    gact = gact.clone()
                    gact[..., :rows, :cols] += t[..., :rows, :cols]
        gw1, gb1, gw0, gb0 = _native.lift_backward(x, w1, b1, w0, b0, gact, g2)
        return None, gw1, gb1, gw0, gb0, None, None, None


def lift_gelu_pad(x: torch.Tensor, fc_n1: nn.Module, fc0: nn.Module, pad_h: int, pad_w: int, grad_join=None) -> torch.Tensor:
    w1, w0 = fc_n1.weight, fc0.weight
    if x.dim() == 4 and _dev_act(x) and not x.requires_grad and w1.dtype == torch.float32 and w0.dtype == torch.float32 and pad_h >= 0 and pad_w >= 0:
        Hp, Wp = x.shape[2] + int(pad_h), x.shape[3] + int(pad_w)
        if _native.lift_ok(x, w1, w0, Hp, Wp):
            return _LiftFn.apply(x, w1, fc_n1.bias, w0, fc0.bias, Hp, Wp, grad_join)
    if grad_join is not None:
        grad_join.accepts_extra = False
    return gelu_channel_mix_pad(channel_mix(x, w1, fc_n1.bias), w0, fc0.bias, pad_h, pad_w)


class _GeluProjectFn(torch.autograd.Function):

    @staticmethod
    def forward(ctx, pre, w, bias):
        pre, w = _plain(pre), _plain(w)
        out = _native.gelu_project_forward(pre, w, None if bias is None else _plain(bias))
        ctx.save_for_backward(pre, w)
        ctx.has_bias = bias is not None
        return out

    @staticmethod
    @once_differentiable
    def backward(ctx, gout):
        pre, w = ctx.saved_tensors
        gpre, gw, gb = _native.gelu_project_backward(pre, w, _plain(gout), need_bias=ctx.has_bias)
        return gpre, gw, gb


def gelu_project(pre: torch.Tensor, weight: torch.Tensor, bias: torch.Tensor | None) -> torch.Tensor:
    if weight.shape[0] == 1 and _dev_act(pre) and weight.dtype == torch.float32 and pre.shape[1] <= 1024:
        B, C = pre.shape[0], pre.shape[1]
        out = _GeluProjectFn.apply(pre.reshape(B, C, -1), weight.reshape(C), bias)
        return out.view(B, 1, *pre.shape[2:])
    return channel_mix(F.gelu(pre), weight, bias)


class _GeluProject2Fn(torch.autograd.Function):

    @staticmethod
    def forward(ctx, pre, s, w, bias, act2):
        pre, s, w = _plain(pre), _plain(s), _plain(w)
        out = _native.gelu_project2_forward(pre, s, w, None if bias is None else _plain(bias), act2)
        ctx.save_for_backward(pre, s, w)
        ctx.has_bias, ctx.act2 = bias is not None, act2
        return out

    @staticmethod
    @once_differentiable
    def backward(ctx, gout):
        pre, s, w = ctx.saved_tensors
        gpre, gs, gw, gb = _native.gelu_project2_backward(pre, s, w, _plain(gout), ctx.act2, need_gs=ctx.needs_input_grad[1],
                                                          need_bias=ctx.has_bias)
        return gpre, gs, gw, gb, None


def gelu_project2(pre: torch.Tensor, s: torch.Tensor, weight: torch.Tensor, bias: torch.Tensor | None, act2: bool = False) -> torch.Tensor:
    C1, C2 = pre.shape[1], s.shape[1]
    if (weight.shape[0] == 1 and pre.is_cuda and s.is_cuda and pre.dtype == torch.float32 and s.dtype == torch.float32
            and weight.dtype == torch.float32 and C1 >= 1 and C2 >= 1 and C1 + C2 <= 1024):
        B = pre.shape[0]
        out = _GeluProject2Fn.apply(pre.reshape(B, C1, -1), s.reshape(B, C2, -1), weight.reshape(C1 + C2), bias, bool(act2))
        return out.view(B, 1, *pre.shape[2:])
    return channel_mix(torch.cat([F.gelu(pre), F.gelu(s) if act2 else s], 1), weight, bias)


class _GeluPadFn(torch.autograd.Function):

    @staticmethod
    def forward(ctx, s, Hp, Wp):
        s = _plain(s)
        ctx.save_for_backward(s)
        return _native.gelu_pad(s, Hp, Wp)

    @staticmethod
    @once_differentiable
    def backward(ctx, gy):
        (s,) = ctx.saved_tensors
        return _native.gelu_pad_backward(s, _plain(gy)), None, None


def gelu_pad2d(s: torch.Tensor, pad_h: int, pad_w: int) -> torch.Tensor:
    if _dev_act(s) and s.dim() >= 2 and pad_h >= 0 and pad_w >= 0:
        return _GeluPadFn.apply(s, s.shape[-2] + int(pad_h), s.shape[-1] + int(pad_w))
    return F.pad(F.gelu(s), [0, pad_w, 0, pad_h])


class _InstanceNormGeluFn(torch.autograd.Function):

    @staticmethod
    def forward(ctx, x, weight, bias, eps, gelu):
        x = _plain(x)
        w = None if weight is None else _plain(weight)
        b = None if bias is None else _plain(bias)
        y, mean, rstd = _native.instnorm_forward(x, w, b, eps, gelu)
        ctx.save_for_backward(x, w, b, mean, rstd)
        ctx.gelu = gelu
        return y

    @staticmethod
    @once_differentiable
    def backward(ctx, gy):
        x, w, b, mean, rstd = ctx.saved_tensors
        gx, s1, s2 = _native.instnorm_backward(x, _plain(gy), w, b, mean, rstd, ctx.gelu)
        gw = s2.sum(0) if w is not None and ctx.needs_input_grad[1] else None
        gb = s1.sum(0) if b is not None and ctx.needs_input_grad[2] else None
        return gx, gw, gb, None, None


def instance_norm_gelu(x: torch.Tensor, norm: nn.Module, gelu: bool) -> torch.Tensor:
    if (_dev_act(x) and isinstance(norm, (nn.InstanceNorm1d, nn.InstanceNorm2d, nn.InstanceNorm3d))
            and not norm.track_running_stats and x.dim() >= 3 and x.shape[1] == norm.num_features):
        if x.numel() // max(x.shape[0] * x.shape[1], 1) <= 1:
            raise ValueError(f"Expected more than 1 spatial element when training, got input size {x.size()}")
        return _InstanceNormGeluFn.apply(x, norm.weight, norm.bias, norm.eps, bool(gelu))
    out = norm(x)
    return F.gelu(out) if gelu else out
```

Measured before the change: 1515 samples/s.

## Generate grid coordinates inside lift kernels instead of concatenating grid input

The model's lift no longer concatenates the coordinate grid onto the input and permutes it to channels-first. The fused lift forward and backward kernels now read the single-channel input directly and look up x/y coordinates from small cached row and column tables. This removes the cat+permute+contiguous copy and cuts input reads from three planes to one. The training loss also switches from the stock relative-L2 to a native rel_l2_sum path.

```diff
diff --git a/include/uno_spectral.h b/include/uno_spectral.h
--- a/include/uno_spectral.h
+++ b/include/uno_spectral.h
@@ -212,6 +212,12 @@
 int uno_lift_backward2(const float* x, const float* w1, const float* b1, const float* w0, const float* b0, const float* g_act,
                        const float* g_act2, float* gw1, float* gb1, float* gw0, float* gb0, void* ws, int B, int Cin, int Cm, int Co,
                        int H, int W, int Hp, int Wp, void* stream);
+int uno_lift_grid_applies(int B, int Cm, int Co, int H, int W, int Hp, int Wp);
+int uno_lift_forward_grid(const float* a, const float* gx, const float* gy, const float* w1, const float* b1, const float* w0,
+                          const float* b0, float* act, int B, int Cm, int Co, int H, int W, int Hp, int Wp, void* stream);
+int uno_lift_backward_grid(const float* a, const float* gx, const float* gy, const float* w1, const float* b1, const float* w0,
+                           const float* b0, const float* g_act, const float* g_act2, float* gw1, float* gb1, float* gw0, float* gb0,
+                           void* ws, int B, int Cm, int Co, int H, int W, int Hp, int Wp, void* stream);
 
 int uno_gelu_pad(const float* s, const float* gy, float* out, int n_img, int H, int W, int Hp, int Wp, int backward,
                  void* stream);
diff --git a/uno_amd/_native.py b/uno_amd/_native.py
--- a/uno_amd/_native.py
+++ b/uno_amd/_native.py
@@ -77,6 +77,9 @@
     "uno_lift_backward": (C.c_int, [_fp] * 11 + [_i] * 8 + [_fp]),
     "uno_lift_backward2": (C.c_int, [_fp] * 12 + [_i] * 8 + [_fp]),
     "uno_lift_backward_takes_second": (C.c_int, [_i] * 8),
+    "uno_lift_grid_applies": (C.c_int, [_i] * 7),
+    "uno_lift_forward_grid": (C.c_int, [_fp] * 8 + [_i] * 7 + [_fp]),
+    "uno_lift_backward_grid": (C.c_int, [_fp] * 14 + [_i] * 7 + [_fp]),
     "uno_channel_mix_dgelu_padded": (C.c_int, [_fp, _fp, _fp, _fp, _fp, _i, _i, _i, _i, _i, _i, _i, _i, _fp]),
     "uno_channel_wgrad2_win": (C.c_int, [_fp, _fp, _fp, _i, _fp, _fp, _fp, _i, _i, _i, _i, _i, _i, C.c_longlong, _i, _i, _fp]),
     "uno_gelu_project_backward_win": (C.c_int, [_fp] * 7 + [_i, _i, _i, _i, _i, C.c_longlong, _fp]),
@@ -880,6 +883,67 @@
     return gw1, gb1, gw0, gb0
 
 
+def lift_grid_tables(H: int, W: int, device):
+    gx = torch.linspace(0, 1, H, dtype=torch.float64).to(torch.float32)
+    gy = torch.zeros((W + 3) // 4 * 4, dtype=torch.float32)
+    gy[:W] = torch.linspace(0, 1, W, dtype=torch.float64).to(torch.float32)
+    return gx.to(device), gy.to(device)
+
+
+def lift_grid_ok(a, w1, w0, Hp: int, Wp: int) -> bool:
+    if a.dim() != 3 or a.dtype != torch.float32 or not a.is_cuda or a.shape[0] < 1 or tuple(w1.shape[1:]) != (3,) or w0.shape[1] != w1.shape[0]:
+        return False
+    B, H, W = a.shape
+    return bool(lib().uno_lift_grid_applies(B, w1.shape[0], w0.shape[0], H, W, int(Hp), int(Wp)))
+
+
+def _lift_grid_operands(a, gx, gy):
+    for t, n in ((a, "a"), (gx, "row table"), (gy, "column table")):
+        _require(t, torch.float32, n)
+    B, H, W = a.shape
+    if gx.numel() != H or gy.numel() != (W + 3) // 4 * 4 or gx.device != a.device or gy.device != a.device:
+        raise RuntimeError(f"uno_amd: the grid tables hold {gx.numel()} and {gy.numel()} entries, a {tuple(a.shape)} input takes {H} and "
+                           f"{(W + 3) // 4 * 4} on its device (lift_grid_tables)")
+    return B, H, W
+
+
+def lift_forward_grid(a, gx, gy, w1, b1, w0, b0, Hp: int, Wp: int):
+    for t, n in ((w1, "weight 1"), (w0, "weight 0")) + tuple((t, "bias") for t in (b1, b0) if t is not None):
+        _require(t, torch.float32, n)
+    B, H, W = _lift_grid_operands(a, gx, gy)
+    Cm, Co = w1.shape[0], w0.shape[0]
+    act = torch.empty((B, Co, Hp, Wp), dtype=a.dtype, device=a.device)
+    with torch.cuda.device(a.device):
+        rc = lib().uno_lift_forward_grid(_ptr(a), _ptr(gx), _ptr(gy), _ptr(w1), _opt(b1), _ptr(w0), _opt(b0), _ptr(act), B, Cm, Co, H, W,
+                                         int(Hp), int(Wp), _stream(a))
+    _check(rc, "uno_lift_forward_grid")
+    return act
+
+
+def lift_backward_grid(a, gx, gy, w1, b1, w0, b0, g_act, g_act2=None):
+    _require(g_act, torch.float32, "grad_output")
+    B, H, W = _lift_grid_operands(a, gx, gy)
+    Cm, Co = w1.shape[0], w0.shape[0]
+    Hp, Wp = g_act.shape[-2:]
+    if tuple(g_act.shape[:2]) != (B, Co):
+        raise RuntimeError("uno_amd: grad_output does not match the lift")
+    if g_act2 is not None:
+        _require(g_act2, torch.float32, "second grad_output")
+        if tuple(g_act2.shape) != tuple(g_act.shape):
+            raise RuntimeError("uno_amd: the two gradients of the lift's output disagree in shape")
+    dev = a.device
+    gw1 = torch.empty((Cm, 3), dtype=torch.float32, device=dev)
+    gw0 = torch.empty((Co, Cm), dtype=torch.float32, device=dev)
+    gb1 = torch.empty((Cm,), dtype=torch.float32, device=dev) if b1 is not None else None
+    gb0 = torch.empty((Co,), dtype=torch.float32, device=dev) if b0 is not None else None
+    with torch.cuda.device(dev):
+        ws = torch.empty(max(1, lib().uno_lift_bwd_ws_bytes(B, 3, Cm, Co, H, W)), dtype=torch.uint8, device=dev)
+        rc = lib().uno_lift_backward_grid(_ptr(a), _ptr(gx), _ptr(gy), _ptr(w1), _opt(b1), _ptr(w0), _opt(b0), _ptr(g_act), _opt(g_act2),
+                                          _ptr(gw1), _opt(gb1), _ptr(gw0), _opt(gb0), _ptr(ws), B, Cm, Co, H, W, int(Hp), int(Wp), _stream(a))
+    _check(rc, "uno_lift_backward_grid")
+    return gw1, gb1, gw0, gb0
+
+
 def channel_mix_dgelu_padded(x, w, bias, g_padded, act_in: bool = False):
     _require(x, torch.float32, "x")
     _require(w, torch.float32, "weight")
diff --git a/uno_amd/csrc/capi_pointwise.hip b/uno_amd/csrc/capi_pointwise.hip
--- a/uno_amd/csrc/capi_pointwise.hip
+++ b/uno_amd/csrc/capi_pointwise.hip
@@ -299,6 +299,38 @@
     return launch_channel_wgrad2(gh, x, nullptr, Cin, gw1, gb1, wws, B, Cin, Cm, P, 0, 0, 0, s);
 }
 
+int uno_lift_grid_applies(int B, int Cm, int Co, int H, int W, int Hp, int Wp) {
+    if (B < 1 || H < 1 || W < 260 || Hp < H || Wp < W || (long long)H * W >= (1LL << 24)) return 0;
+    return (lift_bwd_fused_applies(3, Cm, Co, W, (long long)H * W) && lift_fused_fits(B, H, Hp, Wp, Co) && (Wp & ~3) >= 260 && (Wp & ~3) >= W) ? 1 : 0;
+}
+
+int uno_lift_forward_grid(const float* a, const float* gx, const float* gy, const float* w1, const float* b1, const float* w0, const float* b0,
+                          float* act, int B, int Cm, int Co, int H, int W, int Hp, int Wp, void* stream) {
+    if (int rc = lift_check("uno_lift_forward_grid", B, 3, Cm, Co, H, W, Hp, Wp)) return rc;
+    if (B == 0) return 0;
+    if (!a || !gx || !gy || !w1 || !w0 || !act) { set_error("uno_lift_forward_grid: null pointer"); return -1; }
+    if (!uno_lift_grid_applies(B, Cm, Co, H, W, Hp, Wp)) { set_error("uno_lift_forward_grid: outside the one-kernel lift (query uno_lift_grid_applies)"); return -3; }
+    if (int rc = launch_lift_forward_fused(a, w1, b1, w0, b0, act, B, 3, H, W, Hp, Wp, (hipStream_t)stream, gx, gy)) return rc;
+    return launch_clear_border(act, (long long)B * Co, Hp, Wp, H, Wp, (hipStream_t)stream);
+}
+
+int uno_lift_backward_grid(const float* a, const float* gx, const float* gy, const float* w1, const float* b1, const float* w0, const float* b0_,
+                           const float* g_act, const float* g_act2, float* gw1, float* gb1, float* gw0, float* gb0, void* ws, int B, int Cm, int Co,
+                           int H, int W, int Hp, int Wp, void* stream) {
+    if (int rc = lift_check("uno_lift_backward_grid", B, 3, Cm, Co, H, W, Hp, Wp)) return rc;
+    if (!gw1 || !gw0) { set_error("uno_lift_backward_grid: null pointer"); return -1; }
+    if (B == 0) return uno_lift_backward2(nullptr, nullptr, nullptr, nullptr, nullptr, nullptr, nullptr, gw1, gb1, gw0, gb0, ws, 0, 3, Cm, Co, H, W, Hp, Wp, stream);
+    if (!a || !gx || !gy || !w1 || !w0 || !g_act || !ws) { set_error("uno_lift_backward_grid: null pointer"); return -1; }
+    if (!uno_lift_grid_applies(B, Cm, Co, H, W, Hp, Wp)) { set_error("uno_lift_backward_grid: outside the one-kernel lift (query uno_lift_grid_applies)"); return -3; }
+    hipStream_t s = (hipStream_t)stream;
+    float* part = static_cast<float*>(ws);
+    const long long nparts = lift_bwd_fused_parts(B, H, W);
+    float* part1 = part + (size_t)nparts * Co * (Cm + 1);
+    if (int rc = launch_lift_backward_fused(a, w1, b1, w0, b0_, g_act, part, part1, B, 3, H, W, Hp, Wp, s, g_act2, gx, gy)) return rc;
+    if (int rc = launch_channel_wgrad_finish(part, gw0, gb0, Cm, Co, nparts, 0, s)) return rc;
+    return launch_channel_wgrad_finish(part1, gw1, gb1, 3, Cm, nparts, 0, s);
+}
+
 long long uno_channel_wgrad_ws_bytes(int B, int Ci, int Co, long long P) {
     if (B < 1 || Ci < 1 || Co < 1 || P < 1) return 0;
     return 4LL * channel_wgrad_ws_floats(B, Ci, Co, P, nullptr);
diff --git a/uno_amd/csrc/lift_bwd.hip b/uno_amd/csrc/lift_bwd.hip
--- a/uno_amd/csrc/lift_bwd.hip
+++ b/uno_amd/csrc/lift_bwd.hip
@@ -16,23 +16,25 @@
     int H, W, W4, nslot, npt;
     int skip_d, skip_p;
     int Pd, Pp;
+    int Wt;
     unsigned magic;
 };
 static LiftGeom lift_geom(int H, int W, int Hp, int Wp, int slots_per_row = 0) {
     LiftGeom g;
     g.H = H; g.W = W; g.W4 = slots_per_row ? slots_per_row : ((W + 3) & ~3); g.nslot = H * g.W4; g.npt = (g.nslot + 127) / 128;
-    g.skip_d = W - g.W4; g.skip_p = Wp - g.W4; g.Pd = H * W; g.Pp = Hp * Wp;
+    g.skip_d = W - g.W4; g.skip_p = Wp - g.W4; g.Pd = H * W; g.Pp = Hp * Wp; g.Wt = (W + 3) & ~3;
     g.magic = (unsigned)(((1ULL << 40) + g.W4 - 1) / (unsigned long long)g.W4);
     return g;
 }
 __device__ __forceinline__ int lift_clamped(int off, int plane_len) { return max(min(off, plane_len - 4), 0); }
-struct LiftQuad { int nv, od, op, row_ok, last, shd, shp; };
+struct LiftQuad { int nv, od, op, row_ok, last, shd, shp, og1, og2; };
 __device__ __forceinline__ LiftQuad lift_quad(const LiftGeom& g, int s0, int s) {
     const int r0 = (int)(((unsigned long long)(unsigned)s0 * g.magic) >> 40);
     const int r = r0 + (s >= (r0 + 1) * g.W4 ? 1 : 0);
     const int col = s - r * g.W4;
     const int od = s + r * g.skip_d, op = s + r * g.skip_p, odc = lift_clamped(od, g.Pd), opc = lift_clamped(op, g.Pp);
-    return LiftQuad{r < g.H ? min(max(g.W - col, 0), 4) : 0, odc, opc, r < g.H ? 1 : 0, col == g.W4 - 4 ? 1 : 0, od - odc, op - opc};
+    return LiftQuad{r < g.H ? min(max(g.W - col, 0), 4) : 0, odc, opc, r < g.H ? 1 : 0, col == g.W4 - 4 ? 1 : 0, od - odc, op - opc,
+                    min(r, g.H - 1), min(col, g.Wt - 4)};
 }
 __device__ __forceinline__ float4 lift_fix(const float4& v, int sh) {
     float t0 = v.x, t1 = v.y, t2 = v.z, t3 = v.w;
@@ -46,6 +48,8 @@
 
 struct LiftBwdParams {
     const float* x;
+    const float* gx;
+    const float* gy;
     const float* w1;
     const float* b1;
     const float* w0;
@@ -71,6 +75,7 @@
     d = fmaf(x, 0.39894228040143267794f * __expf(-0.5f * x * x), cdf);
 }
 
+template <bool GRID>
 __global__ __launch_bounds__(256, 2) void lift_backward_kernel(LiftBwdParams p) {
     extern __shared__ __attribute__((aligned(16))) float lb_smem[];
     float* sA = lb_smem;
@@ -95,7 +100,7 @@
         sVH[tid] = make_float4(wr[0], p.Cin > 1 ? wr[1] : 0.f, p.Cin > 2 ? wr[2] : 0.f, p.b1 ? p.b1[tid] : 0.f);
     }
     const float b0v = p.b0 ? p.b0[16 * wave + r16] : 0.f;
-    const float* xb = p.x + (size_t)b * p.Cin * G.Pd;
+    const float* xb = p.x + (size_t)b * (GRID ? 1 : p.Cin) * G.Pd;
     const float* gb = p.g + (size_t)b * LB_CO * G.Pp;
     const float* gb2 = p.g2 ? p.g2 + (size_t)b * LB_CO * G.Pp : nullptr;
 
@@ -120,8 +125,14 @@
     auto load_tile = [&](int tile) {
         const int s0 = tile * LB_PT;
         nxt = lift_quad(G, s0, s0 + (tid & 31) * 4);
-#pragma unroll
-        for (int k = 0; k < 3; ++k) xq[k] = io_ld4(xb + (size_t)min(k, p.Cin - 1) * G.Pd + nxt.od);
+        if (GRID) {
+            xq[0] = io_ld4(xb + nxt.od);
+            xq[1].x = p.gx[nxt.og1];
+            xq[2] = io_ld4(p.gy + nxt.og2);
+        } else {
+#pragma unroll
+            for (int k = 0; k < 3; ++k) xq[k] = io_ld4(xb + (size_t)min(k, p.Cin - 1) * G.Pd + nxt.od);
+        }
 #pragma unroll
         for (int u = 0; u < 8; ++u) gq[u] = io_ld4(gb + (size_t)((tid >> 5) + 8 * u) * G.Pp + nxt.op);
     };
@@ -129,8 +140,15 @@
     __syncthreads();
     for (int tile = t_begin; tile < t_end; ++tile) {
         cur = nxt;
-#pragma unroll
-        for (int k = 0; k < 3; ++k) { xq[k] = lift_fix(xq[k], cur.shd); xc[k] = lift_mask(xq[k], cur.nv); }
+        if (GRID) {
+            xq[0] = lift_fix(xq[0], cur.shd);
+            xq[1] = make_float4(xq[1].x, xq[1].x, xq[1].x, xq[1].x);
+        } else {
+#pragma unroll
+            for (int k = 0; k < 3; ++k) xq[k] = lift_fix(xq[k], cur.shd);
+        }
+#pragma unroll
+        for (int k = 0; k < 3; ++k) xc[k] = lift_mask(xq[k], cur.nv);
         float4 dh[4];
         {
             const int q4 = (tid & 31) * 4;
@@ -284,6 +302,7 @@
 }
 
 struct LiftFwdParams {
+    const float* gx; const float* gy;
     const float* x; const float* w1; const float* b1; const float* w0; const float* b0;
     float* act;
     int B, Cin, tail;
@@ -292,6 +311,7 @@
     int rev;
 };
 
+template <bool GRID>
 __global__ __launch_bounds__(256, 2) void lift_forward_kernel(LiftFwdParams p) {
     extern __shared__ __attribute__((aligned(16))) float lb_smem[];
     float* sA = lb_smem;
@@ -312,15 +332,21 @@
         sVH[tid] = make_float4(wr[0], p.Cin > 1 ? wr[1] : 0.f, p.Cin > 2 ? wr[2] : 0.f, p.b1 ? p.b1[tid] : 0.f);
     }
     const float b0v = p.b0 ? p.b0[16 * wave + r16] : 0.f;
-    const float* xb = p.x + (size_t)b * p.Cin * G.Pd;
+    const float* xb = p.x + (size_t)b * (GRID ? 1 : p.Cin) * G.Pd;
     float* ab = p.act + (size_t)b * LB_CO * G.Pp;
     float4 xqA[3], xqB[3];
     LiftQuad qdA = {0, 0, 0, 0, 0, 0, 0}, qdB = {0, 0, 0, 0, 0, 0, 0};
     auto load_x = [&](int tile, float4* xq, LiftQuad& qd) {
         const int s0 = tile * LB_PT;
         qd = lift_quad(G, s0, s0 + (tid & 31) * 4);
-#pragma unroll
-        for (int k = 0; k < 3; ++k) xq[k] = io_ld4(xb + (size_t)min(k, p.Cin - 1) * G.Pd + qd.od);
+        if (GRID) {
+            xq[0] = io_ld4(xb + qd.od);
+            xq[1].x = p.gx[qd.og1];
+            xq[2] = io_ld4(p.gy + qd.og2);
+        } else {
+#pragma unroll
+            for (int k = 0; k < 3; ++k) xq[k] = io_ld4(xb + (size_t)min(k, p.Cin - 1) * G.Pd + qd.od);
+        }
     };
 #ifdef UNO_LB_DEV
     unsigned long long tph[8] = {0, 0, 0, 0, 0, 0, 0, 0}, t_prev = __builtin_readcyclecounter();
@@ -333,7 +359,9 @@
         const LiftQuad cur = qd;
         {
             const int q4 = (tid & 31) * 4;
-            const float4 q[3] = {lift_mask(lift_fix(xq[0], cur.shd), cur.nv), lift_mask(lift_fix(xq[1], cur.shd), cur.nv), lift_mask(lift_fix(xq[2], cur.shd), cur.nv)};
+            const float4 q[3] = {lift_mask(lift_fix(xq[0], cur.shd), cur.nv),
+                                 lift_mask(GRID ? make_float4(xq[1].x, xq[1].x, xq[1].x, xq[1].x) : lift_fix(xq[1], cur.shd), cur.nv),
+                                 lift_mask(GRID ? xq[2] : lift_fix(xq[2], cur.shd), cur.nv)};
 #pragma unroll
             for (int u = 0; u < 4; ++u) {
                 const int m = (tid >> 5) + 8 * u;
@@ -416,9 +444,12 @@
 }
 
 int launch_lift_forward_fused(const float* x, const float* w1, const float* b1, const float* w0, const float* b0, float* act, int B, int Cin,
-                              int H, int W, int Hp, int Wp, hipStream_t s) {
+                              int H, int W, int Hp, int Wp, hipStream_t s, const float* gx, const float* gy) {
     LiftFwdParams p;
-    p.x = x; p.w1 = w1; p.b1 = b1; p.w0 = w0; p.b0 = b0; p.act = act;
+    const bool grid = gx != nullptr;
+    if (grid != (gy != nullptr)) { set_error("lift_forward: the grid form takes both tables"); return -1; }
+    if (grid) Cin = 3;
+    p.x = x; p.gx = gx; p.gy = gy; p.w1 = w1; p.b1 = b1; p.w0 = w0; p.b0 = b0; p.act = act;
     p.B = B; p.Cin = Cin; p.geo = lift_geom(H, W, Hp, Wp, Wp & ~3); p.tail = Wp & 3;
     p.stamps = nullptr;
     p.rev = next_sweep_reversed(SWEEP_LIFT);
@@ -426,12 +457,15 @@
     if (getenv("UNO_LF_STAMPS")) p.stamps = reinterpret_cast<unsigned long long*>((uintptr_t)strtoull(getenv("UNO_LF_STAMPS"), nullptr, 0));
 #endif
     if ((long long)Hp * Wp * LB_CO >= (1LL << 31) || B > 65535 || (long long)H * Wp >= (1LL << 24)) { set_error("lift_forward: tensor too large"); return -2; }
-    static int lds_slot[64];
+    static int lds_slot[2][64];
     const size_t lds = sizeof(float) * (LB_CM * LB_TS + LB_CO * LB_TS + LB_CM * LB_WS) + sizeof(float4) * LB_CM;
-    if (!ensure_dynamic_lds(reinterpret_cast<const void*>(lift_forward_kernel), lds, lds_slot)) { set_error("lift_forward: cannot raise dynamic LDS to %zu", lds); return -4; }
+    const void* kernel = grid ? reinterpret_cast<const void*>(lift_forward_kernel<true>) : reinterpret_cast<const void*>(lift_forward_kernel<false>);
+    if (!ensure_dynamic_lds(kernel, lds, lds_slot[grid ? 1 : 0])) { set_error("lift_forward: cannot raise dynamic LDS to %zu", lds); return -4; }
     {
-        ProfScope prof("uno::lift_forward_kernel", 4.0 * B * ((double)H * W * Cin + (double)H * Wp * LB_CO), s);
-        hipLaunchKernelGGL(lift_forward_kernel, dim3((unsigned)((p.geo.npt + LB_TPW - 1) / LB_TPW), (unsigned)B), dim3(256), lds, s, p);
+        ProfScope prof("uno::lift_forward_kernel", 4.0 * B * ((double)H * W * (grid ? 1 : Cin) + (double)H * Wp * LB_CO), s);
+        const dim3 blocks((unsigned)((p.geo.npt + LB_TPW - 1) / LB_TPW), (unsigned)B);
+        if (grid) hipLaunchKernelGGL(lift_forward_kernel<true>, blocks, dim3(256), lds, s, p);
+        else hipLaunchKernelGGL(lift_forward_kernel<false>, blocks, dim3(256), lds, s, p);
     }
     const hipError_t e = hipGetLastError();
     if (e != hipSuccess) { set_error("lift_forward launch: %s", hipGetErrorString(e)); return -5; }
@@ -450,9 +484,13 @@
 }
 
 int launch_lift_backward_fused(const float* x, const float* w1, const float* b1, const float* w0, const float* b0, const float* g, float* part,
-                               float* part1, int B, int Cin, int H, int W, int Hp, int Wp, hipStream_t s, const float* g2) {
+                               float* part1, int B, int Cin, int H, int W, int Hp, int Wp, hipStream_t s, const float* g2, const float* gx,
+                               const float* gy) {
     LiftBwdParams p;
-    p.x = x; p.w1 = w1; p.b1 = b1; p.w0 = w0; p.b0 = b0; p.g = g; p.g2 = g2; p.part = part; p.part1 = part1;
+    const bool grid = gx != nullptr;
+    if (grid != (gy != nullptr)) { set_error("lift_backward: the grid form takes both tables"); return -1; }
+    if (grid) Cin = 3;
+    p.x = x; p.gx = gx; p.gy = gy; p.w1 = w1; p.b1 = b1; p.w0 = w0; p.b0 = b0; p.g = g; p.g2 = g2; p.part = part; p.part1 = part1;
     p.B = B; p.Cin = Cin; p.geo = lift_geom(H, W, Hp, Wp);
     p.stamps = nullptr;
     p.rev = next_sweep_reversed(SWEEP_LIFT);
@@ -460,12 +498,15 @@
     if (getenv("UNO_LB_STAMPS")) p.stamps = reinterpret_cast<unsigned long long*>((uintptr_t)strtoull(getenv("UNO_LB_STAMPS"), nullptr, 0));
 #endif
     if ((long long)Hp * Wp * LB_CO >= (1LL << 31) || B > 65535) { set_error("lift_backward: tensor too large"); return -2; }
-    static int lds_slot[64];
+    static int lds_slot[2][64];
     const size_t lds = lift_bwd_lds();
-    if (!ensure_dynamic_lds(reinterpret_cast<const void*>(lift_backward_kernel), lds, lds_slot)) { set_error("lift_backward: cannot raise dynamic LDS to %zu", lds); return -4; }
+    const void* kernel = grid ? reinterpret_cast<const void*>(lift_backward_kernel<true>) : reinterpret_cast<const void*>(lift_backward_kernel<false>);
+    if (!ensure_dynamic_lds(kernel, lds, lds_slot[grid ? 1 : 0])) { set_error("lift_backward: cannot raise dynamic LDS to %zu", lds); return -4; }
     {
-        ProfScope prof("uno::lift_backward_kernel", 4.0 * B * (double)H * W * (Cin + LB_CO * (g2 ? 2 : 1)), s);
-        hipLaunchKernelGGL(lift_backward_kernel, dim3((unsigned)((p.geo.npt + LB_TPW - 1) / LB_TPW), (unsigned)B), dim3(256), lds, s, p);
+        ProfScope prof("uno::lift_backward_kernel", 4.0 * B * (double)H * W * ((grid ? 1 : Cin) + LB_CO * (g2 ? 2 : 1)), s);
+        const dim3 blocks((unsigned)((p.geo.npt + LB_TPW - 1) / LB_TPW), (unsigned)B);
+        if (grid) hipLaunchKernelGGL(lift_backward_kernel<true>, blocks, dim3(256), lds, s, p);
+        else hipLaunchKernelGGL(lift_backward_kernel<false>, blocks, dim3(256), lds, s, p);
     }
     const hipError_t e = hipGetLastError();
     if (e != hipSuccess) { set_error("lift_backward launch: %s", hipGetErrorString(e)); return -5; }
diff --git a/uno_amd/csrc/uno_common.h b/uno_amd/csrc/uno_common.h
--- a/uno_amd/csrc/uno_common.h
+++ b/uno_amd/csrc/uno_common.h
@@ -335,9 +335,11 @@
 bool lift_bwd_fused_applies(int Cin, int Cm, int Co, int W, long long P);
 long long lift_bwd_fused_parts(int B, int H, int W);
 int launch_lift_forward_fused(const float* x, const float* w1, const float* b1, const float* w0, const float* b0, float* act, int B, int Cin,
-                              int H, int W, int Hp, int Wp, hipStream_t s);
+                              int H, int W, int Hp, int Wp, hipStream_t s, const float* gx = nullptr,
+                              const float* gy = nullptr);
 int launch_lift_backward_fused(const float* x, const float* w1, const float* b1, const float* w0, const float* b0, const float* g, float* part,
-                               float* part1, int B, int Cin, int H, int W, int Hp, int Wp, hipStream_t s, const float* g2 = nullptr);
+                               float* part1, int B, int Cin, int H, int W, int Hp, int Wp, hipStream_t s, const float* g2 = nullptr,
+                               const float* gx = nullptr, const float* gy = nullptr);
 int launch_channel_wgrad_finish(const float* parts, float* gw, float* gb, int Ci, int Co, long long nparts, int accumulate, hipStream_t s);
 long long rel_l2_steps_chunks(long long P, int T, long long* chunk_pixels);
 long long rel_l2_steps_ws_floats(int B, long long P, int T);
diff --git a/uno_amd/harness/__init__.py b/uno_amd/harness/__init__.py
--- a/uno_amd/harness/__init__.py
+++ b/uno_amd/harness/__init__.py
@@ -1,6 +1,6 @@
 from .models import UNO, UNO_9, UNO_P, UNO_S256, Uno3D_T9, Uno3D_T10, Uno3D_T20, Uno3D_T40
 from .optim import ComplexAdam
-from .losses import LpLoss, RolloutErrors, StepErrors, lp_loss_rel_sum, rel_l2, step_errors
+from .losses import LpLoss, RolloutErrors, StepErrors, lp_loss_rel_sum, rel_l2, rel_l2_sum, step_errors
 from .mixed import MixedDarcyTrainer
 from .train import DarcyTrainer, GraphedRollout, GraphedStep, ns2d_evaluate, ns2d_rollout_errors, ns2d_rollout_loss, ns3d_evaluate, ns3d_loss, ns3d_step_error, synthetic_darcy_batch
 from .datagen import GaussianRF, generate_ns_dataset, navier_stokes_2d
diff --git a/uno_amd/harness/losses.py b/uno_amd/harness/losses.py
--- a/uno_amd/harness/losses.py
+++ b/uno_amd/harness/losses.py
@@ -53,6 +53,13 @@
         elif not g.is_contiguous():
             g = g.contiguous()
         return _native.rel_l2_backward(x, y, record, g, 1.0 / x.shape[0] if ctx.reduce == 2 else 1.0), None, None
+
+
+def rel_l2_sum(pred: torch.Tensor, target: torch.Tensor) -> torch.Tensor:
+    rows = _native_rows(pred, target)
+    if rows is None:
+        return lp_loss_rel_sum(pred, target)
+    return _RelL2Fn.apply(rows[0], rows[1], 1)
 
 
 def rel_l2(x: torch.Tensor, y: torch.Tensor) -> torch.Tensor:
diff --git a/uno_amd/harness/mixed.py b/uno_amd/harness/mixed.py
--- a/uno_amd/harness/mixed.py
+++ b/uno_amd/harness/mixed.py
@@ -5,7 +5,7 @@
 import torch
 
 from ..integral_operators import enable_mixed_precision
-from .losses import lp_loss_rel_sum
+from .losses import rel_l2_sum
 from .models import UNO_9
 from .train import DarcyTrainer, synthetic_darcy_batch
 
@@ -19,7 +19,7 @@
     def step(self, a, u):
         B = a.shape[0]
         ab = a.to(torch.bfloat16)
-        return self.step_with(lambda: lp_loss_rel_sum(self.model(ab).reshape(B, -1).float(), u.reshape(B, -1)))
+        return self.step_with(lambda: rel_l2_sum(self.model(ab).reshape(B, -1).float(), u.reshape(B, -1)))
 
 
 def c5_mixed_model_bench(dev, B: int = 4, S: int = 1024, steps: int = 4, warmup: int = 2):
diff --git a/uno_amd/harness/models.py b/uno_amd/harness/models.py
--- a/uno_amd/harness/models.py
+++ b/uno_amd/harness/models.py
@@ -9,7 +9,8 @@
 from ..integral_operators import (GradJoin, SpectrumShare, OperatorBlock_2D, OperatorBlock_3D, channel_mix, channel_mix_cat, channel_mix_cat_project,
                                   enable_native_resample3d_any, enable_native_resample3d_wide, enable_one_buffer_any_grid, gelu_channel_mix, gelu_channel_mix_pad, gelu_pad2d, gelu_project, gelu_project2,
                                   lift_gelu_pad)
-from ..pointwise import gelu_channel_mix_pad_last
+from .._native import lift_grid_tables
+from ..pointwise import gelu_channel_mix_pad_last, lift_gelu_pad_grid, lift_grid_applies
 
 NATIVE_ENDS_3D = False
 
@@ -64,6 +65,7 @@
         self.fc1 = nn.Linear(2 * w, w)
         self.fc2 = nn.Linear(w, 1)
         self._grid_cache = {}
+        self._table_cache = {}
 
     def get_grid(self, shape, device):
         def build():
@@ -75,13 +77,17 @@
 
     def forward(self, x):
         S1, S2 = x.shape[1], x.shape[2]
-        x = torch.cat((x, self.get_grid(x.shape, x.device).to(x.dtype)), dim=-1).permute(0, 3, 1, 2).contiguous()
         scale = math.ceil(S2 / 85)
         margin = scale * self.padding
         product = hasattr(self.conv5, "forward_cat")
         fused = product and self.conv5.non_lin and not self.conv5.normalize
         jl = GradJoin() if fused else None
-        lifted = lift_gelu_pad(x, self.fc_n1, self.fc0, margin, margin, grad_join=jl)
+        if product and self.in_width == 3 and lift_grid_applies(x, self.fc_n1, self.fc0, margin, margin):
+            tables = _cached(self._table_cache, (S1, S2, str(x.device)), lambda: lift_grid_tables(S1, S2, x.device))
+            lifted = lift_gelu_pad_grid(x, tables, self.fc_n1, self.fc0, margin, margin, grad_join=jl)
+        else:
+            x = torch.cat((x, self.get_grid(x.shape, x.device).to(x.dtype)), dim=-1).permute(0, 3, 1, 2).contiguous()
+            lifted = lift_gelu_pad(x, self.fc_n1, self.fc0, margin, margin, grad_join=jl)
         d1, d2 = lifted.shape[-2], lifted.shape[-1]
 
         if fused:
diff --git a/uno_amd/harness/train.py b/uno_amd/harness/train.py
--- a/uno_amd/harness/train.py
+++ b/uno_amd/harness/train.py
@@ -6,7 +6,7 @@
 import torch.distributed as dist
 from torch.autograd.function import once_differentiable
 
-from .losses import NATIVE_STEP_ERRORS_MAX_T, RolloutErrors, StepErrors, _step_errors_stock, lp_loss_rel_sum, step_errors
+from .losses import NATIVE_STEP_ERRORS_MAX_T, RolloutErrors, StepErrors, _step_errors_stock, lp_loss_rel_sum, rel_l2_sum, step_errors
 from .optim import ComplexAdam
 
 
@@ -555,12 +555,12 @@
 
     def step(self, a, u):
         B, S = a.shape[0], a.shape[1]
-        return self.step_with(lambda: lp_loss_rel_sum(self.model(a).reshape(B, -1), u.reshape(B, -1)))
+        return self.step_with(lambda: rel_l2_sum(self.model(a).reshape(B, -1), u.reshape(B, -1)))
 
     def step_blocking(self, a, u):
         B = a.shape[0]
         self.grads.zero_()
-        loss = lp_loss_rel_sum(self.model(a).reshape(B, -1), u.reshape(B, -1))
+        loss = rel_l2_sum(self.model(a).reshape(B, -1), u.reshape(B, -1))
         loss.backward()
         self.grads.all_reduce_sum(self.group, self.force_collectives)
         self.opt.step()
diff --git a/uno_amd/pointwise.py b/uno_amd/pointwise.py
--- a/uno_amd/pointwise.py
+++ b/uno_amd/pointwise.py
@@ -587,6 +587,60 @@
     return gelu_channel_mix_pad(channel_mix(x, w1, fc_n1.bias), w0, fc0.bias, pad_h, pad_w)
 
 
+class _LiftGridFn(torch.autograd.Function):
+
+    @staticmethod
+    def forward(ctx, a, gx, gy, w1, b1, w0, b0, Hp, Wp, grad_join=None):
+        a, w1, w0 = _plain(a), _plain(w1), _plain(w0)
+        b1 = None if b1 is None else _plain(b1)
+        b0 = None if b0 is None else _plain(b0)
+        ctx.save_for_backward(a, gx, gy, w1, w0, *[t for t in (b1, b0) if t is not None])
+        ctx.has = (b1 is not None, b0 is not None)
+        ctx.join = None
+        if grad_join is not None:
+            grad_join.accepts_extra = True
+            grad_join.extra = []
+            ctx.join = grad_join
+        return _native.lift_forward_grid(a, gx, gy, w1, b1, w0, b0, Hp, Wp)
+
+    @staticmethod
+    @once_differentiable
+    def backward(ctx, gact):
+        a, gx, gy, w1, w0, *bs = ctx.saved_tensors
+        b1 = bs.pop(0) if ctx.has[0] else None
+        b0 = bs.pop(0) if ctx.has[1] else None
+        gact = _plain(gact)
+        g2 = None
+        if ctx.join is not None:
+            ctx.join.accepts_extra = False
+            H, W = a.shape[-2:]
+            for t, (rows, cols, pitch) in ctx.join.take_extra():
+                t = t.view(gact.shape)
+                if g2 is None and rows >= H and cols >= W and pitch == gact.shape[-1]:
+                    g2 = t
+                else:
+                    gact = gact.clone()
+                    gact[..., :rows, :cols] += t[..., :rows, :cols]
+        gw1, gb1, gw0, gb0 = _native.lift_backward_grid(a, gx, gy, w1, b1, w0, b0, gact, g2)
+        return None, None, None, gw1, gb1, gw0, gb0, None, None, None
+
+
+def lift_grid_applies(a: torch.Tensor, fc_n1: nn.Module, fc0: nn.Module, pad_h: int, pad_w: int) -> bool:
+    w1, w0 = fc_n1.weight, fc0.weight
+    return (a.dim() == 4 and a.shape[-1] == 1 and _dev_act(a) and a.dtype == torch.float32 and not a.requires_grad and w1.dtype == torch.float32
+            and w0.dtype == torch.float32 and pad_h >= 0 and pad_w >= 0
+            and _native.lift_grid_ok(a.reshape(a.shape[:3]), w1, w0, a.shape[1] + int(pad_h), a.shape[2] + int(pad_w)))
+
+
+def lift_gelu_pad_grid(a: torch.Tensor, tables, fc_n1: nn.Module, fc0: nn.Module, pad_h: int, pad_w: int, grad_join=None) -> torch.Tensor:
+    if not lift_grid_applies(a, fc_n1, fc0, pad_h, pad_w):
+        raise RuntimeError(f"uno_amd: lift_gelu_pad_grid does not cover a {tuple(a.shape)} {a.dtype} input on {a.device} "
+                           f"(ask lift_grid_applies; lift_gelu_pad takes the concatenated input)")
+    B, H, W = a.shape[:3]
+    return _LiftGridFn.apply(a.reshape(B, H, W), tables[0], tables[1], fc_n1.weight, fc_n1.bias, fc0.weight, fc0.bias,
+                             H + int(pad_h), W + int(pad_w), grad_join)
+
+
 class _GeluProjectFn(torch.autograd.Function):
 
     @staticmethod
```

New measurement: 1515 samples/s (median of 2 runs). Within noise of the previous version (-0.0%).
